# mauruszach/multimodal_diffusion

Hardware: AMD Instinct MI355X
Metric: denoising steps/sec @256x256 multimodal-cond batch=32 (higher is better)
Workload: dtype f32 via 3xbf16 split operands (6-term products, f32 accumulate; fp32-level error); 1 GPU; C3: 256x256 audio->video CFG denoising step (cond+null MMDiT d512 L8 H8 + noise head + DDIM), 384+37 tokens, batch 32 per GPU, DDIM 50 steps, guidance 3.5; global_batch=32, sampler_steps=50, parallelism=dp1, launch=eager, matmul=bf16x3, attn=default, cfg_halves=one stacked 2B batch, one stream

## Files before the change

include/avdiff_hip.h:

```cpp
#ifndef AVDIFF_HIP_H
#define AVDIFF_HIP_H

#include <stdint.h>

#ifdef __cplusplus
extern "C" {
#endif

#define AVD_ABI_VERSION 7

#define AVD_OK            0
#define AVD_EINVAL       -1
#define AVD_EUNSUPPORTED -2
#define AVD_ELAUNCH      -3
#define AVD_EWORKSPACE   -4

#define AVD_ACT_NONE 0
#define AVD_ACT_GELU 1
#define AVD_ACT_SILU 2
#define AVD_ACT_TANH 3
#define AVD_ACT_RELU 4
#define AVD_ACT_LEAKY_RELU 5

typedef void* avd_stream_t;

int         avd_abi_version(void);
const char* avd_last_error(void);
int         avd_device_arch(char* buf, int buflen);
int         avd_tune_set(const char* key, int64_t value);
int         avd_cfg_dedup_set(int on);

int avd_rmsnorm_f32(const float* x, const float* scale, float* y, int64_t rows, int d, float eps,
                    avd_stream_t stream);

int avd_gemm_bias_act_f32(const float* A, int64_t lda, const float* W, const float* bias,
                          const float* residual, int64_t ldr, float* C, int64_t ldc,
                          int64_t M, int N, int K, int act, avd_stream_t stream);

int avd_gemm_rmsfold_f32(const float* A, const float* W, const float* bias, const float* residual, float* C, int64_t M,
                         int N, int K, int act, const float* ss_in, int ss_in_cols, float eps, float* ss_out,
                         avd_stream_t stream);

int avd_attn_fwd_f32(const float* qkv, float* out, int B, int N, int H, int Dh, float scale,
                     int n_query, const uint8_t* key_padding_mask, avd_stream_t stream);

int avd_layernorm_act_f32(const float* x, const float* gamma, const float* beta, float* y,
                          int64_t rows, int d, float eps, int act, avd_stream_t stream);

int avd_timestep_embedding_f32(const int64_t* t, const float* freqs, float* out, int B, int dim, float max_period,
                               avd_stream_t stream);

int avd_tube_patch_f32(const float* z, float* tok, int B, int C, int T, int H, int W, int t, int h, int w,
                       avd_stream_t stream);
int avd_tube_unpatch_f32(const float* tok, float* z, int B, int C, int T, int H, int W, int t, int h, int w,
                         avd_stream_t stream);

int avd_audio_tokens_f32(const float* z, float* tok, int B, int Ca, int F, int len, int stride,
                         avd_stream_t stream);
int avd_audio_untokens_f32(const float* tok, const float* window, float* z, int B, int Ca, int F, int len, int stride,
                           avd_stream_t stream);

int avd_ddim_step_f32(const float* x_t, const float* eps_hat, const int64_t* t_now, const int64_t* t_prev,
                      const float* alpha_bar, int T_train, float eta, const float* noise,
                      float* x_prev, int B, int64_t per_sample, avd_stream_t stream);

int avd_dpmpp_2m_step_f32(const float* x_t, const float* eps_hat, float* x0_hist, const int64_t* t_last, const int64_t* t_now,
                          const int64_t* t_prev, const float* alpha_bar, int T_train, float* x_out, int B, int64_t per_sample,
                          avd_stream_t stream);

int avd_dpmpp_2m_sde_step_f32(const float* x_t, const float* eps_hat, float* x0_hist, const int64_t* t_last, const int64_t* t_now,
                              const int64_t* t_prev, const float* alpha_bar, int T_train, float eta, const float* noise, float* x_out,
                              int B, int64_t per_sample, avd_stream_t stream);

typedef struct {
    uint64_t seed;
    int64_t sample_offset;
} avd_noise_key;
int avd_gaussian_noise_f32(const avd_noise_key* key, const int64_t* t_now, float* out, int B, int64_t per_sample,
                           avd_stream_t stream);

int avd_canvas_noise_f32(const avd_noise_key* key, const int64_t* t_now, float* out, int N, int64_t outer, int L, int hop,
                         int64_t inner, avd_stream_t stream);

int avd_cfg_unpatch_ddim_slots_f32(const float* eps2, const float* z, const int64_t* t_now, const int64_t* t_prev,
                                   const float* alpha_bar, int T_train, float guidance, int slots, float* z_out,
                                   int B, int C, int T, int H, int W, int t, int h, int w, avd_stream_t stream);
int avd_cfg_untoken_ddim_audio_slots_f32(const float* eps2, const float* z, const int64_t* t_now, const int64_t* t_prev,
                                         const float* alpha_bar, int T_train, float guidance, int slots, float* z_out,
                                         int B, int Ca, int F, int len, int stride, avd_stream_t stream);
int avd_cfg_unpatch_dpmpp_2m_slots_f32(const float* eps2, const float* z, const int64_t* t_last, const int64_t* t_now,
                                       const int64_t* t_prev, const float* alpha_bar, int T_train, float guidance, int slots,
                                       float* x0_hist, float* z_out, int B, int C, int T, int H, int W, int t, int h, int w,
                                       avd_stream_t stream);
int avd_cfg_untoken_dpmpp_2m_audio_slots_f32(const float* eps2, const float* z, const int64_t* t_last, const int64_t* t_now,
                                             const int64_t* t_prev, const float* alpha_bar, int T_train, float guidance, int slots,
                                             float* x0_hist, float* z_out, int B, int Ca, int F, int len, int stride,
                                             avd_stream_t stream);

int avd_fifo_shift_f32(const avd_noise_key* key, int64_t t, int64_t c, const float* z_in, float* z_out, float* popped,
                       int B, int64_t outer, int slots, int slot_len, int64_t inner, avd_stream_t stream);
int avd_fifo_shift_hist_f32(const avd_noise_key* key, int64_t t, int64_t c, const float* z_in, float* z_out, float* popped,
                            const float* hist_in, float* hist_out, int B, int64_t outer, int slots, int slot_len, int64_t inner,
                            avd_stream_t stream);

int avd_fifo_lookahead_f32(const avd_noise_key* key, int64_t t, int64_t c, int shift, const float* z_in, float* z_out, float* popped,
                           int B, int64_t outer, int slots, int ctx, int slot_len, int64_t inner, avd_stream_t stream);
int avd_fifo_lookahead_hist_f32(const avd_noise_key* key, int64_t t, int64_t c, int shift, const float* z_in, float* z_out,
                                float* popped, const float* hist_in, float* hist_out, int B, int64_t outer, int slots, int ctx,
                                int slot_len, int64_t inner, avd_stream_t stream);

int avd_cursor_add(int32_t* cursor, int delta, avd_stream_t stream);
int avd_slot_tables_select(const int64_t* tab0, const int64_t* tab1, const int64_t* tab2, int n_rows, int n, const int32_t* cursor,
                           int64_t* out0, int64_t* out1, int64_t* out2, avd_stream_t stream);
int avd_fifo_prompt_gather_f32(const float* canvas, const int32_t* cursor, float* out, int B, int slots, int prompt_hop, int64_t outer,
                               int64_t P, int64_t prompt_len, int64_t inner, avd_stream_t stream);
int avd_fifo_shift_cursor_f32(const avd_noise_key* key, int64_t t, int64_t c0, const int32_t* cursor, int64_t n_out, const float* z_in,
                              float* z_out, float* clip, int B, int64_t outer, int slots, int slot_len, int64_t inner, avd_stream_t stream);
int avd_fifo_shift_cursor_hist_f32(const avd_noise_key* key, int64_t t, int64_t c0, const int32_t* cursor, int64_t n_out,
                                   const float* z_in, float* z_out, float* clip, const float* hist_in, float* hist_out, int B,
                                   int64_t outer, int slots, int slot_len, int64_t inner, avd_stream_t stream);

typedef struct {
    const float* known;
    const float* mask;
    int64_t mask_batch_stride;
    avd_noise_key key;
} avd_latent_guide;
int avd_latent_guide_f32(const avd_latent_guide* g, const int64_t* tau, const float* alpha_bar, int T_train,
                         const float* z, float* out, int B, int64_t per_sample, avd_stream_t stream);

int avd_latent_guide_canvas_f32(const avd_latent_guide* g, const int64_t* tau, const float* alpha_bar, int T_train,
                                const float* z, float* out, int N, int64_t outer, int L, int hop, int64_t inner, avd_stream_t stream);

int avd_renoise_f32(const avd_noise_key* key, uint32_t visit, const avd_latent_guide* g, const int64_t* t_from, const int64_t* t_to,
                    const float* alpha_bar, int T_train, const float* z, float* out, int B, int64_t per_sample, avd_stream_t stream);
int avd_renoise_canvas_f32(const avd_noise_key* key, uint32_t visit, const avd_latent_guide* g, const int64_t* t_from,
                           const int64_t* t_to, const float* alpha_bar, int T_train, const float* z, float* out, int N, int64_t outer,
                           int L, int hop, int64_t inner, avd_stream_t stream);

typedef struct {
    const float* guidance;
    const float* rescale;
    void* stats;
    int64_t stats_bytes;
} avd_cfg_control;
int64_t avd_cfg_stats_bytes(int B, int64_t per_sample);
int avd_cfg_rescale_f32(const float* e_cond, const float* e_cfg, const float* phi, void* stats, int64_t stats_bytes, float* out,
                        int B, int64_t per_sample, avd_stream_t stream);

typedef struct {
    float norm_threshold;
    float eta_parallel;
    float momentum;
    float* momentum_buf;
    void* stats;
    int64_t stats_bytes;
} avd_apg_control;
int64_t avd_apg_stats_bytes(int B, int64_t per_sample);
int avd_apg_guidance_f32(const float* e_cond, const float* e_null, const float* guidance, float guidance_scalar,
                         const avd_apg_control* apg, float* out, int B, int64_t per_sample, avd_stream_t stream);

int avd_cfg_unpatch_ddim_f32(const float* eps2, const float* z, const int64_t* t_now, const int64_t* t_prev,
                             const float* alpha_bar, int T_train, float guidance, float eta,
                             const float* noise, float* z_out,
                             int B, int C, int T, int H, int W, int t, int h, int w, avd_stream_t stream);

int avd_cfg_untoken_ddim_audio_f32(const float* eps2, const float* z, const int64_t* t_now,
                                   const int64_t* t_prev, const float* alpha_bar, int T_train,
                                   float guidance, float eta, const float* noise, float* z_out,
                                   int B, int Ca, int F, int len, int stride, avd_stream_t stream);

int avd_eps_unpatch_ddim_f32(const float* eps, const float* z, const int64_t* t_now, const int64_t* t_prev,
                             const float* alpha_bar, int T_train, float eta, const float* noise, float* z_out,
                             int B, int C, int T, int H, int W, int t, int h, int w, const avd_noise_key* key,
                             const int64_t* t_last, float* x0_hist, const avd_latent_guide* guide, avd_stream_t stream);
int avd_eps_untoken_ddim_audio_f32(const float* eps, const float* z, const int64_t* t_now, const int64_t* t_prev,
                                   const float* alpha_bar, int T_train, float eta, const float* noise, float* z_out,
                                   int B, int Ca, int F, int len, int stride, const avd_noise_key* key,
                                   const int64_t* t_last, float* x0_hist, const avd_latent_guide* guide, avd_stream_t stream);

typedef struct {
    int target_kind;
    int target_first;
    int B, d, tdim;
    int C, T, H, W;
    int p0, p1, p2;
// ... 244 lines not shown
```

multimodal_diffusion_amd/_lib.py:

```python
from __future__ import annotations

import ctypes as C
import os
from pathlib import Path
from typing import Optional

import torch

_HERE = Path(__file__).resolve().parent
LIB_PATH = Path(os.environ.get("AVDIFF_HIP_LIB", _HERE / "csrc" / "libavdiff_hip.so"))

ACT_NONE, ACT_GELU, ACT_SILU, ACT_TANH, ACT_RELU, ACT_LEAKY_RELU = 0, 1, 2, 3, 4, 5
EINVAL, EUNSUPPORTED, ELAUNCH, EWORKSPACE = -1, -2, -3, -4


class AvdError(RuntimeError):
    """A HIP-side failure (launch error, unsupported shape, workspace)."""


class EmbedDesc(C.Structure):
    _fields_ = [("target_kind", C.c_int), ("target_first", C.c_int), ("B", C.c_int), ("d", C.c_int),
                ("tdim", C.c_int), ("C", C.c_int), ("T", C.c_int), ("H", C.c_int), ("W", C.c_int),
                ("p0", C.c_int), ("p1", C.c_int), ("p2", C.c_int), ("Nt", C.c_int), ("Np", C.c_int),
                ("temb_freqs", C.c_void_p), ("temb_add", C.c_int)]


class BlockWeights(C.Structure):
    _fields_ = [(n, C.c_void_p) for n in (
        "norm1_scale", "in_proj_weight", "in_proj_bias", "out_proj_weight", "out_proj_bias",
        "norm2_scale", "fc1_weight", "fc1_bias", "fc2_weight", "fc2_bias",
        "in_proj_weight_n", "fc1_weight_n",
        "in_proj_weight3", "out_proj_weight3", "fc1_weight3", "fc2_weight3",
        "norm1_bias", "norm2_bias")] + [("f16x2_scale", C.c_float * 8), ("in_proj_weight3n", C.c_void_p), ("fc1_weight3n", C.c_void_p)]


class CoreWeights(C.Structure):
    _fields_ = [("d", C.c_int), ("n_layers", C.c_int), ("n_heads", C.c_int), ("mlp_hidden", C.c_int),
                ("norm_eps", C.c_float), ("blocks", C.POINTER(BlockWeights)), ("final_norm_scale", C.c_void_p),
                ("norm_kind", C.c_int), ("final_norm_bias", C.c_void_p), ("split_terms", C.c_int), ("attn_mode", C.c_int)]


class HeadWeights(C.Structure):
    _fields_ = [("d_in", C.c_int), ("hidden", C.c_int), ("d_out", C.c_int), ("n_shared", C.c_int),
                ("ln_eps", C.c_float), ("act", C.c_int),
                ("input_proj_weight", C.c_void_p), ("input_proj_bias", C.c_void_p),
                ("shared_lin_weight", C.POINTER(C.c_void_p)), ("shared_lin_bias", C.POINTER(C.c_void_p)),
                ("shared_ln_weight", C.POINTER(C.c_void_p)), ("shared_ln_bias", C.POINTER(C.c_void_p)),
                ("out_proj_weight", C.c_void_p), ("out_proj_bias", C.c_void_p),
                ("split_terms", C.c_int), ("input_proj_weight3", C.c_void_p), ("shared_lin_weight3", C.POINTER(C.c_void_p)),
                ("out_proj_weight3", C.c_void_p), ("f16x2_scale", C.POINTER(C.c_float))]


class StepDesc(C.Structure):
    _fields_ = [("embed", EmbedDesc), ("core", C.POINTER(CoreWeights)), ("head", C.POINTER(HeadWeights)),
                ("adapt_w", C.c_void_p), ("adapt_b", C.c_void_p), ("alpha_bar", C.c_void_p), ("T_train", C.c_int),
                ("guidance", C.c_float), ("eta", C.c_float), ("split_streams", C.c_int)]


class NoiseKey(C.Structure):
    _fields_ = [("seed", C.c_uint64), ("sample_offset", C.c_int64)]


class LatentGuide(C.Structure):
    _fields_ = [("known", C.c_void_p), ("mask", C.c_void_p), ("mask_batch_stride", C.c_int64), ("key", NoiseKey)]


class CfgControl(C.Structure):
    _fields_ = [("guidance", C.c_void_p), ("rescale", C.c_void_p), ("stats", C.c_void_p), ("stats_bytes", C.c_int64)]


class ApgControl(C.Structure):
    _fields_ = [("norm_threshold", C.c_float), ("eta_parallel", C.c_float), ("momentum", C.c_float), ("momentum_buf", C.c_void_p),
                ("stats", C.c_void_p), ("stats_bytes", C.c_int64)]


class VaeDecodeDesc(C.Structure):
    _fields_ = [("B", C.c_int), ("Cv", C.c_int), ("Tp", C.c_int), ("Hp", C.c_int), ("Wp", C.c_int),
                ("T", C.c_int), ("H", C.c_int), ("W", C.c_int),
                ("base", C.c_int), ("n_blocks", C.c_int), ("out_ch", C.c_int), ("out_tanh", C.c_int),
                ("gn_eps", C.c_float),
                ("from_lat_w", C.c_void_p), ("from_lat_b", C.c_void_p),
                ("conv_w", C.POINTER(C.c_void_p)), ("conv_b", C.POINTER(C.c_void_p)),
                ("gn_w", C.POINTER(C.c_void_p)), ("gn_b", C.POINTER(C.c_void_p)),
                ("to_img_w", C.c_void_p), ("to_img_b", C.c_void_p),
                ("conv_w3", C.POINTER(C.c_void_p)), ("conv_terms", C.c_int),
                ("conv_w_scale", C.POINTER(C.c_float)), ("conv_a_scale", C.POINTER(C.c_float)),
                ("conv0_lat_w3", C.c_void_p), ("conv0_lat_btab", C.c_void_p), ("conv0_lat_w_scale", C.c_float),
                ("conv0_lat_packed", C.c_int)]


class VaeEncodeDesc(C.Structure):
    _fields_ = [("B", C.c_int), ("in_ch", C.c_int), ("T", C.c_int), ("H", C.c_int), ("W", C.c_int),
                ("t_down", C.c_int), ("s_down", C.c_int),
                ("base", C.c_int), ("n_blocks", C.c_int), ("lat_ch", C.c_int), ("gn_eps", C.c_float),
                ("conv_w", C.POINTER(C.c_void_p)), ("conv_b", C.POINTER(C.c_void_p)),
                ("gn_w", C.POINTER(C.c_void_p)), ("gn_b", C.POINTER(C.c_void_p)),
                ("to_lat_w", C.c_void_p), ("to_lat_b", C.c_void_p),
                ("conv_w3", C.POINTER(C.c_void_p)), ("conv_terms", C.c_int),
                ("conv_w_scale", C.POINTER(C.c_float)), ("conv_a_scale", C.POINTER(C.c_float)),
                ("conv0_pk_w3", C.c_void_p)]


ABI_VERSION = 7
_P, _I, _L, _F = C.c_void_p, C.c_int, C.c_int64, C.c_float

SIGNATURES = {
    "avd_abi_version": (_I, []),
    "avd_last_error": (C.c_char_p, []),
    "avd_device_arch": (_I, [C.c_char_p, _I]),
    "avd_rmsnorm_f32": (_I, [_P, _P, _P, _L, _I, _F, _P]),
    "avd_gemm_bias_act_f32": (_I, [_P, _L, _P, _P, _P, _L, _P, _L, _L, _I, _I, _I, _P]),
    "avd_gemm_rmsfold_f32": (_I, [_P, _P, _P, _P, _P, _L, _I, _I, _I, _P, _I, _F, _P, _P]),
    "avd_tune_set": (_I, [C.c_char_p, _L]),
    "avd_cfg_dedup_set": (_I, [_I]),
    "avd_attn_fwd_f32": (_I, [_P, _P, _I, _I, _I, _I, _F, _I, _P, _P]),
    "avd_layernorm_act_f32": (_I, [_P, _P, _P, _P, _L, _I, _F, _I, _P]),
    "avd_timestep_embedding_f32": (_I, [_P, _P, _P, _I, _I, _F, _P]),
    "avd_tube_patch_f32": (_I, [_P, _P] + [_I] * 8 + [_P]),
    "avd_tube_unpatch_f32": (_I, [_P, _P] + [_I] * 8 + [_P]),
    "avd_audio_tokens_f32": (_I, [_P, _P] + [_I] * 5 + [_P]),
    "avd_audio_untokens_f32": (_I, [_P, _P, _P] + [_I] * 5 + [_P]),
    "avd_ddim_step_f32": (_I, [_P, _P, _P, _P, _P, _I, _F, _P, _P, _I, _L, _P]),
    "avd_cfg_unpatch_ddim_f32": (_I, [_P, _P, _P, _P, _P, _I, _F, _F, _P, _P] + [_I] * 8 + [_P]),
    "avd_cfg_untoken_ddim_audio_f32": (_I, [_P, _P, _P, _P, _P, _I, _F, _F, _P, _P] + [_I] * 5 + [_P]),
    "avd_embed_workspace_floats": (_L, [C.POINTER(EmbedDesc)]),
    "avd_embed_cfg_pair_f32": (_I, [C.POINTER(EmbedDesc), _P, _P, _P, _P, _P, _P, _P, _P]),
    "avd_core_workspace_bytes": (_L, [C.POINTER(CoreWeights), _I, _I]),
    "avd_core_forward_f32": (_I, [C.POINTER(CoreWeights), _P, _P, _I, _I, _I, _I, _P, _P, _L, _P]),
    "avd_head_workspace_bytes": (_L, [C.POINTER(HeadWeights), _L]),
    "avd_head_forward_f32": (_I, [C.POINTER(HeadWeights), _P, _L, _L, _L, _L, _P, _P, _L, _P]),
    "avd_step_workspace_bytes": (_L, [C.POINTER(StepDesc)]),
    "avd_denoise_step_f32": (_I, [C.POINTER(StepDesc), _P, _P, _P, _P, _P, _P, _P, _L, _P]),
    "avd_denoise_step_seeded_f32": (_I, [C.POINTER(StepDesc), C.POINTER(NoiseKey), _P, _P, _P, _P, _P, _P, _L, _P]),
    "avd_gaussian_noise_f32": (_I, [C.POINTER(NoiseKey), _P, _P, _I, _L, _P]),
    "avd_canvas_noise_f32": (_I, [C.POINTER(NoiseKey), _P, _P, _I, _L, _I, _I, _L, _P]),
    "avd_denoise_step_canvas_f32": (_I, [C.POINTER(StepDesc), C.POINTER(NoiseKey), _I, C.POINTER(CfgControl), C.POINTER(LatentGuide), _I,
                                         _P, _P, _P, _P, _P, _P, _L, _P]),
    "avd_cfg_unpatch_ddim_slots_f32": (_I, [_P, _P, _P, _P, _P, _I, _F, _I, _P] + [_I] * 8 + [_P]),
    "avd_cfg_untoken_ddim_audio_slots_f32": (_I, [_P, _P, _P, _P, _P, _I, _F, _I, _P] + [_I] * 5 + [_P]),
    "avd_embed_cfg_pair_slots_f32": (_I, [C.POINTER(EmbedDesc), _P, _P, _P, _P, _I, _P, _P, _P, _P]),
    "avd_denoise_step_slots_f32": (_I, [C.POINTER(StepDesc), _P, _P, _P, _P, _I, _P, _P, _L, _P]),
    "avd_fifo_shift_f32": (_I, [C.POINTER(NoiseKey), _L, _L, _P, _P, _P, _I, _L, _I, _I, _L, _P]),
    "avd_cfg_unpatch_dpmpp_2m_slots_f32": (_I, [_P, _P, _P, _P, _P, _P, _I, _F, _I, _P, _P] + [_I] * 8 + [_P]),
    "avd_cfg_untoken_dpmpp_2m_audio_slots_f32": (_I, [_P, _P, _P, _P, _P, _P, _I, _F, _I, _P, _P] + [_I] * 5 + [_P]),
    "avd_denoise_step_slots_dpmpp_2m_f32": (_I, [C.POINTER(StepDesc), _P, _P, _P, _P, _P, _I, _P, _P, _P, _L, _P]),
    "avd_fifo_shift_hist_f32": (_I, [C.POINTER(NoiseKey), _L, _L, _P, _P, _P, _P, _P, _I, _L, _I, _I, _L, _P]),
    "avd_fifo_lookahead_f32": (_I, [C.POINTER(NoiseKey), _L, _L, _I, _P, _P, _P, _I, _L, _I, _I, _I, _L, _P]),
    "avd_fifo_lookahead_hist_f32": (_I, [C.POINTER(NoiseKey), _L, _L, _I, _P, _P, _P, _P, _P, _I, _L, _I, _I, _I, _L, _P]),
    "avd_cursor_add": (_I, [_P, _I, _P]),
    "avd_slot_tables_select": (_I, [_P, _P, _P, _I, _I, _P, _P, _P, _P, _P]),
    "avd_fifo_prompt_gather_f32": (_I, [_P, _P, _P, _I, _I, _I, _L, _L, _L, _L, _P]),
    "avd_fifo_shift_cursor_f32": (_I, [C.POINTER(NoiseKey), _L, _L, _P, _L, _P, _P, _P, _I, _L, _I, _I, _L, _P]),
    "avd_fifo_shift_cursor_hist_f32": (_I, [C.POINTER(NoiseKey), _L, _L, _P, _L, _P, _P, _P, _P, _P, _I, _L, _I, _I, _L, _P]),
    "avd_sched_advance": (_I, [_P, _I, _P, _P, _P, _I, _P]),
    "avd_sched_advance_ms": (_I, [_P, _I, _P, _P, _P, _P, _I, _P]),
    "avd_dpmpp_2m_step_f32": (_I, [_P, _P, _P, _P, _P, _P, _P, _I, _P, _I, _L, _P]),
    "avd_denoise_step_dpmpp_2m_f32": (_I, [C.POINTER(StepDesc), _P, _P, _P, _P, _P, _P, _P, _P, _L, _P]),
    "avd_dpmpp_2m_sde_step_f32": (_I, [_P, _P, _P, _P, _P, _P, _P, _I, _F, _P, _P, _I, _L, _P]),
    "avd_denoise_step_dpmpp_2m_sde_f32": (_I, [C.POINTER(StepDesc), C.POINTER(NoiseKey), _I, C.POINTER(CfgControl), C.POINTER(LatentGuide),
                                               _I, _P, _P, _P, _P, _P, _P, _P, _P, _L, _P]),
    "avd_latent_guide_f32": (_I, [C.POINTER(LatentGuide), _P, _P, _I, _P, _P, _I, _L, _P]),
    "avd_latent_guide_canvas_f32": (_I, [C.POINTER(LatentGuide), _P, _P, _I, _P, _P, _I, _L, _I, _I, _L, _P]),
    "avd_renoise_f32": (_I, [C.POINTER(NoiseKey), C.c_uint32, C.POINTER(LatentGuide), _P, _P, _P, _I, _P, _P, _I, _L, _P]),
    "avd_renoise_canvas_f32": (_I, [C.POINTER(NoiseKey), C.c_uint32, C.POINTER(LatentGuide), _P, _P, _P, _I, _P, _P, _I, _L, _I, _I, _L,
                                    _P]),
    "avd_denoise_step_canvas_guided_f32": (_I, [C.POINTER(StepDesc), C.POINTER(LatentGuide), _I, C.POINTER(NoiseKey), C.POINTER(CfgControl),
                                                _I, _P, _P, _P, _P, _P, _P, _P, _P, _L, _P]),
    "avd_denoise_step_guided_f32": (_I, [C.POINTER(StepDesc), C.POINTER(LatentGuide), C.POINTER(NoiseKey), _P, _P, _P, _P, _P, _P, _P,
                                         _P, _L, _P]),
    "avd_cfg_stats_bytes": (_L, [_I, _L]),
    "avd_cfg_rescale_f32": (_I, [_P, _P, _P, _P, _L, _P, _I, _L, _P]),
    "avd_denoise_step_cfg_f32": (_I, [C.POINTER(StepDesc), C.POINTER(CfgControl), C.POINTER(LatentGuide), C.POINTER(NoiseKey), _P, _P, _P,
                                      _P, _P, _P, _P, _P, _L, _P]),
    "avd_apg_stats_bytes": (_L, [_I, _L]),
    "avd_apg_guidance_f32": (_I, [_P, _P, _P, _F, C.POINTER(ApgControl), _P, _I, _L, _P]),
    "avd_denoise_step_apg_f32": (_I, [C.POINTER(StepDesc), C.POINTER(ApgControl), C.POINTER(CfgControl), C.POINTER(LatentGuide),
                                      C.POINTER(NoiseKey), _I, _I, _P, _P, _P, _P, _P, _P, _P, _P, _L, _P]),
    "avd_eps_unpatch_ddim_f32": (_I, [_P, _P, _P, _P, _P, _I, _F, _P, _P] + [_I] * 8 + [C.POINTER(NoiseKey), _P, _P, C.POINTER(LatentGuide), _P]),
    "avd_eps_untoken_ddim_audio_f32": (_I, [_P, _P, _P, _P, _P, _I, _F, _P, _P] + [_I] * 5 + [C.POINTER(NoiseKey), _P, _P,
                                                                                               C.POINTER(LatentGuide), _P]),
    "avd_embed_cond_f32": (_I, [C.POINTER(EmbedDesc), _P, _P, _P, _P, _P, _P, _P, _P, _P]),
    "avd_denoise_step_cond_f32": (_I, [C.POINTER(StepDesc), C.POINTER(LatentGuide), C.POINTER(NoiseKey), _P, _P, _P, _P, _P, _P, _P, _P,
                                       _P, _L, _P]),
    "avd_split3_bytes": (_L, [_L, _I]),
    "avd_split3_f32": (_I, [_P, _P, _L, _I, _P]),
    "avd_rmsnorm_split3_f32": (_I, [_P, _P, _P, _L, _I, _F, _P]),
    "avd_attn_fwd_split3_f32": (_I, [_P, _P, _I, _I, _I, _I, _F, _I, _P]),
    "avd_qkv3_bytes": (_L, [_I, _I, _I]),
    "avd_gemm_bf16x3_qkv3_f32": (_I, [_P, _P, _P, _P, _L, _I, _I, _I, _F, _I, _P]),
    "avd_attn_fwd_qkv3_f32": (_I, [_P, _P, _P, _I, _I, _I, _I, _I, _P]),
    "avd_attn_fp8_workspace_bytes": (_L, [_I, _I, _I]),
    "avd_attn_fwd_fp8_f32": (_I, [_P, _P, _L, _P, _P, _I, _I, _I, _I, _P]),
    "avd_attn_fwd_fp8_f16x2_f32": (_I, [_P, _P, _L, _P, _P, _I, _I, _I, _I, _F, _F, _P]),
    "avd_gemm_bf16x3_f32": (_I, [_P, _P, _P, _P, _P, _P, _L, _I, _I, _I, _I, _P]),
    "avd_weight_bounds_f32": (_I, [_P, _L, _I, _P, _P]),
    "avd_split_f16x2_f32": (_I, [_P, _P, _L, _I, _F, _P]),
    "avd_rmsnorm_split_f16x2_f32": (_I, [_P, _P, _P, _L, _I, _F, _F, _P]),
    "avd_gemm_f16x2_f32": (_I, [_P, _P, _P, _P, _P, _P, _L, _I, _I, _I, _F, _F, _P]),
    "avd_gemm_f16x2_qkv_f32": (_I, [_P, _P, _P, _P, _L, _I, _I, _I, _F, _F, _F, _P]),
    "avd_attn_fwd_qkv_f16x2_f32": (_I, [_P, _P, _P, _I, _I, _I, _I, _F, _F, _P]),
    "avd_conv3_weight_bytes": (_L, []),
    "avd_conv3_weight_f32": (_I, [_P, _P, _P]),
    "avd_conv3_weight_f16x2_f32": (_I, [_P, _P, _F, _P]),
    "avd_vae_decode_workspace_bytes": (_L, [C.POINTER(VaeDecodeDesc)]),
    "avd_vae_decode_f32": (_I, [C.POINTER(VaeDecodeDesc), _P, _P, _P, _L, _P]),
    "avd_vae_encode_workspace_bytes": (_L, [C.POINTER(VaeEncodeDesc)]),
    "avd_vae_encode_f32": (_I, [C.POINTER(VaeEncodeDesc), _P, _P, _P, _L, _P]),
    "avd_conv1d_act_f32": (_I, [_P, _P, _P, _P, _I, _I, _I, _I, _I, _I, _I, _P]),
    "avd_avgpool_frames_f32": (_I, [_P, _P, _I, _I, _I, _I, _P]),
    "avd_crossfade_f32": (_I, [_P, _P, _P, _I, _I, _I, _L, _P]),
    "avd_crossfade_u8": (_I, [_P, _P, _P, _I, _I, _I, _L, _P]),
    "avd_window_consensus_f32": (_I, [_P, _P, _I, _L, _I, _I, _L, _P]),
    "avd_prof_enable": (_I, [_I]),
    "avd_prof_num_tags": (_I, []),
    "avd_prof_tag_name": (C.c_char_p, [_I]),
    "avd_prof_report": (_I, [C.POINTER(C.c_int64), C.POINTER(C.c_double), C.POINTER(C.c_double), _I]),
}

def prof_enable(on: bool) -> None:
    check(lib().avd_prof_enable(1 if on else 0))


def prof_report():
    n = lib().avd_prof_num_tags()
    cnt, ms, work = (C.c_int64 * max(n, 1))(), (C.c_double * max(n, 1))(), (C.c_double * max(n, 1))()
    check(lib().avd_prof_report(cnt, ms, work, n))
    return {lib().avd_prof_tag_name(i).decode(): (int(cnt[i]), float(ms[i]), float(work[i])) for i in range(n)}


_lib: Optional[C.CDLL] = None


def lib() -> C.CDLL:
    global _lib
    if _lib is None:
        if not LIB_PATH.exists():
            raise AvdError(
                f"{LIB_PATH} not found: build it with `make -C multimodal_diffusion_amd/csrc` "
                "(or __graft_entry__.build()); this package has no CPU/PyTorch fallback")
        handle = C.CDLL(str(LIB_PATH))
        for name, (res, args) in SIGNATURES.items():
            fn = getattr(handle, name)
            fn.restype, fn.argtypes = res, args
        if handle.avd_abi_version() != ABI_VERSION:
            raise AvdError(f"ABI version mismatch: library {handle.avd_abi_version()}, binding {ABI_VERSION}")
        _lib = handle
    return _lib


def check(rc: int) -> None:
    if rc == 0:
        return
    msg = lib().avd_last_error().decode("utf-8", "replace")
    if rc == EINVAL:
        raise ValueError(msg)
    raise AvdError(f"[avd {rc}] {msg}")


def stream_ptr(device: torch.device) -> int:
    idx = device.index if device.index is not None else torch.cuda.current_device()
    if idx != torch.cuda.current_device():
        raise AvdError(f"tensors are on cuda:{idx} but the current device is cuda:{torch.cuda.current_device()}: "
                       "call torch.cuda.set_device / use torch.cuda.device(...) around the call")
    return torch.cuda.current_stream(device).cuda_stream


MATMUL_TERMS = {"auto": 6, "f32": 0, "bf16x3": 6, "bf16x3_strict": 9, "bf16": 1, "f16x2": 3}
# ... 21 lines not shown
```

multimodal_diffusion_amd/csrc/avd_common.h:

```cpp
#pragma once
#include <hip/hip_runtime.h>
#include <stdint.h>
#include <stdio.h>
#include <stdarg.h>
#include <atomic>

#include "../../include/avdiff_hip.h"

namespace avd {

int set_error(int code, const char* fmt, ...);

#define AVD_REQUIRE(cond, code, ...)                       \
    do {                                                   \
        if (!(cond)) return avd::set_error((code), __VA_ARGS__); \
    } while (0)

#define AVD_CHECK_LAUNCH(name)                                                          \
    do {                                                                                \
        hipError_t e__ = hipGetLastError();                                             \
        if (e__ != hipSuccess)                                                          \
            return avd::set_error(AVD_ELAUNCH, "%s: %s", (name), hipGetErrorString(e__)); \
    } while (0)

// ... 66 lines not shown
    }
};

struct TubeGather {
    int T, H, W, t, h, w, Ht, Wt, Nt;
    int64_t per;
    __host__ __device__ __forceinline__ int64_t row_off(int64_t row) const {
        const int64_t b = row / Nt;
        const int n = (int)(row - b * Nt);
        const int nx = n % Wt, ny = (n / Wt) % Ht, nt = n / (Wt * Ht);
        return b * per + ((int64_t)(nt * t) * H + ny * h) * W + nx * w;
    }
    __host__ __device__ __forceinline__ int64_t k_off(int k) const {
        const int dx = k % w, dy = (k / w) % h, dt = (k / (w * h)) % t, c = k / (w * h * t);
        return (((int64_t)c * T + dt) * H + dy) * W + dx;
    }
};

typedef __bf16 bf16x8 __attribute__((ext_vector_type(8)));
typedef unsigned int u32x4 __attribute__((ext_vector_type(4)));

constexpr int S3_CHUNK = 128 * 96;
constexpr int S3_PLANE = 128 * 32;

typedef __bf16 bf16x2 __attribute__((ext_vector_type(2)));
typedef float f32x2 __attribute__((ext_vector_type(2)));

__device__ __forceinline__ unsigned int pk_bf16(float a, float b) {
    const f32x2 v = {a, b};
    return __builtin_bit_cast(unsigned int, __builtin_convertvector(v, bf16x2));
}
__device__ __forceinline__ float bf16_lo(unsigned int p) { return __uint_as_float(p << 16); }
__device__ __forceinline__ float bf16_hi(unsigned int p) { return __uint_as_float(p & 0xffff0000u); }

template <bool RANGE_CHECK = true>
__device__ __forceinline__ void split8(const float* v, u32x4& H, u32x4& Mi, u32x4& Lo) {
#pragma clang fp contract(off)
    bool edge = false;
    if constexpr (RANGE_CHECK) {
        float amax = fabsf(v[0]);
#pragma unroll
        for (int e = 1; e < 8; ++e) amax = fmaxf(amax, fabsf(v[e]));
        edge = __any(amax > 3.3895313892515355e38f);
    }
#pragma unroll
    for (int e = 0; e < 4; ++e) {
        const float a = v[2 * e], b = v[2 * e + 1];
        unsigned int h = pk_bf16(a, b);
        float ra = a - bf16_lo(h), rb = b - bf16_hi(h);
        if (edge) {
            if ((h & 0x7fffu) == 0x7f80u) {
                if (fabsf(a) < __builtin_inff()) { h = (h & 0xffff8000u) | 0x7f7fu; ra = a - bf16_lo(h); } else ra = 0.f;
            }
            if ((h & 0x7fff0000u) == 0x7f800000u) {
                if (fabsf(b) < __builtin_inff()) { h = (h & 0x8000ffffu) | 0x7f7f0000u; rb = b - bf16_hi(h); } else rb = 0.f;
            }
        }
        const unsigned int m = pk_bf16(ra, rb);
        const float sa = ra - bf16_lo(m), sb = rb - bf16_hi(m);
        H[e] = h;
        Mi[e] = m;
        Lo[e] = pk_bf16(sa, sb);
    }
}

template <bool RANGE_CHECK = true>
__device__ __forceinline__ void store_split8(unsigned char* img, int64_t r, int k, int K, const float* v) {
    u32x4 H, Mi, Lo;
    split8<RANGE_CHECK>(v, H, Mi, Lo);
    const int rr = (int)(r & 127), half = (k >> 3) & 1;
    unsigned char* dst = img + ((r >> 7) * (K >> 4) + (k >> 4)) * (int64_t)S3_CHUNK + rr * 32 + ((half ^ ((rr >> 4) & 1)) << 4);
    *reinterpret_cast<u32x4*>(dst) = H;
    *reinterpret_cast<u32x4*>(dst + S3_PLANE) = Mi;
    *reinterpret_cast<u32x4*>(dst + 2 * S3_PLANE) = Lo;
}

typedef _Float16 f16x8 __attribute__((ext_vector_type(8)));
typedef _Float16 f16x2 __attribute__((ext_vector_type(2)));

__device__ __forceinline__ unsigned int pk_f16(float a, float b) {
    const f32x2 v = {a, b};
    return __builtin_bit_cast(unsigned int, __builtin_convertvector(v, f16x2));
}
__device__ __forceinline__ f32x2 unpk_f16(unsigned int p) { return __builtin_convertvector(__builtin_bit_cast(f16x2, p), f32x2); }

__device__ __forceinline__ void split8_h2(const float* v, float s, u32x4& H, u32x4& L) {
#pragma unroll
    for (int e = 0; e < 4; ++e) {
        const float a = v[2 * e] * s, b = v[2 * e + 1] * s;
        const unsigned int h = pk_f16(a, b);
        const f32x2 u = unpk_f16(h);
        H[e] = h;
        L[e] = pk_f16(a - u[0], b - u[1]);
    }
}
__device__ __forceinline__ void store_split8_h2(unsigned char* img, int64_t r, int k, int K, const float* v, float s) {
    u32x4 H, L;
    split8_h2(v, s, H, L);
    const int rr = (int)(r & 127), half = (k >> 3) & 1;
    unsigned char* dst = img + ((r >> 7) * (K >> 4) + (k >> 4)) * (int64_t)S3_CHUNK + rr * 32 + ((half ^ ((rr >> 4) & 1)) << 4);
    *reinterpret_cast<u32x4*>(dst) = H;
    *reinterpret_cast<u32x4*>(dst + S3_PLANE) = L;
}

template <bool F16>
__device__ __forceinline__ f32x16 mma16(bf16x8 a, bf16x8 b, f32x16 c) {
    if constexpr (F16)
        return __builtin_amdgcn_mfma_f32_32x32x16_f16(__builtin_bit_cast(f16x8, a), __builtin_bit_cast(f16x8, b), c, 0, 0, 0);
    else
        return __builtin_amdgcn_mfma_f32_32x32x16_bf16(a, b, c, 0, 0, 0);
}
__host__ __device__ constexpr int s3_planes(int terms) { return terms == 1 ? 1 : terms == 3 ? 2 : 3; }

constexpr int QKV3_ROWB = 384;
__host__ __device__ __forceinline__ int qkv3_npad(int n) { return (n + 63) / 64 * 64; }
__host__ __device__ __forceinline__ int qkv3_swizzle(int part, int n) {
    return part == 0 ? 0 : part == 1 ? (n >> 1) & 7 : (((n >> 1) & 1) << 2) | (((n >> 2) & 1) << 1);
}

extern bool g_prof_on;
void prof_mark(int tag, double work, hipStream_t st, bool begin);
int prof_tag_id(const char* fmt, ...);
struct ProfScope {
    int tag; hipStream_t st; bool on;
    ProfScope(int t, double work, hipStream_t s) : tag(t), st(s), on(g_prof_on) { if (on) prof_mark(tag, work, st, true); }
    ~ProfScope() { if (on) prof_mark(tag, 0.0, st, false); }
};

int gemm_f32(const float* A, RowMap am, const float* W, const float* bias, const float* R, RowMap rm,
             float* C, RowMap cm, int64_t M, int N, int K, int act, hipStream_t st);
int gemm_f32_tube(const float* z, const TubeGather& tg, const float* W, const float* bias, float* C, RowMap cm, int64_t M, int N, int K,
                  hipStream_t st);

extern int g_gemm_stages;
extern int g_gemm_force_tile;
bool gemm_f32_fold_supported(int N, int K);
int gemm_f32_fold(const float* A, RowMap am, const float* W, const float* bias, const float* R, RowMap rm, float* C, RowMap cm,
                  int64_t M, int N, int K, int act, const float* ss_in, int ss_in_cols, float sqrt_d, float eps, float* ss_out,
                  hipStream_t st);
int rowss_f32(const float* x, float* ss, int64_t rows, int d, hipStream_t st);
constexpr int kGemmSplitKMax = 4;
extern int g_gemm_splitk;
int gemm_f32_splitk_slices(int64_t M, int N, int K);
int64_t gemm_f32_splitk_ws_max_floats(int64_t M, int N, int K);
int gemm_f32_splitk(const float* A, RowMap am, const float* W, const float* bias, const float* R, RowMap rm, float* C, RowMap cm, int64_t M,
                    int N, int K, int ns, float* part, float* ss_out, hipStream_t st);

int attn_f32(const float* qkv, float* out, int B, int N, int H, int Dh, float scale, int n_query, const unsigned char* key_padding_mask,
             hipStream_t st);
int rmsnorm_f32(const float* x, RowMap xm, const float* scale, float* y, RowMap ym, int64_t rows, int d, float eps,
                hipStream_t st);
int layernorm_act_f32(const float* x, const float* gamma, const float* beta, float* y, int64_t rows, int d, float eps,
                      int act, hipStream_t st);
int weight_bounds_f32(const float* x, int64_t rows, int d, float* out2, hipStream_t st);

int64_t split3_bytes(int64_t rows, int K);
int split3_f32(const float* x, int64_t ld, void* out, int64_t rows, int K, hipStream_t st, float h2_scale = 0.f);
int split3_rows_f32(const float* x, RowMap xm, void* out, int64_t rows, int K, hipStream_t st, float h2_scale = 0.f, float* ss = nullptr);
int rmsnorm_split3_f32(const float* x, const float* scale, void* out, int64_t rows, int d, float eps, hipStream_t st, float h2_scale = 0.f);
int layernorm_act_split3_f32(const float* x, const float* gamma, const float* beta, void* out, int64_t rows, int d, float eps, int act,
                             hipStream_t st, float h2_scale = 0.f);
bool gemm_bf16x3_supported(int64_t M, int N, int K);
int attn_f32_split3(const float* qkv, void* out3, int B, int N, int H, int Dh, float scale, int n_query, hipStream_t st);
extern int g_s3_stagger;
extern int g_mlp_fused;
bool mlp_bf16x3_supported(int d, int hidden, int terms);
int mlp_bf16x3(const void* X3, const void* W1n3, const float* b1, const void* W23, const float* b2, const float* ss_in, float eps,
               const float* R, float* C, void* C3, float* ss_out, int64_t M, int d, int hidden, hipStream_t st);
extern int g_attn_m16;
extern int g_attn_pipe;
extern int g_s3_m16;
extern int g_s3_w128;
extern int g_s3_rt4;
extern int g_s3_deep4;
extern int g_s3_rt;
extern int g_vae_lat;
extern int g_vae_fold;
extern int g_codec_mfma;
extern int g_cfg_rows;
extern int g_s3_sn, g_s3_super4, g_s3_super8;
extern int g_s3_tile;
extern thread_local bool t_s3_two_streams;
int gemm_bf16x3_qkv3(const void* A3, const void* W3, const float* bias, void* img, const RowSegs& seg, int heads, int K, float qscale,
                     int terms, hipStream_t st, float ab_scale = 1.f, float c_scale = 1.f, const float* ss_in = nullptr, float eps = 0.f,
                     int64_t plan_rows = 0);
int64_t qkv3_bytes(int B, int N, int H);
int64_t attn_fp8_ws_bytes(int B, int N, int H);
int attn_fp8(const void* qkv3, void* ws, int64_t ws_bytes, float* out, void* out3, int B, int N, int H, int n_query, hipStream_t st,
             int img_terms = 6, float img_scale = 1.f, float out_scale = 1.f);
int attn_bf16x3(const void* qkv3, float* out, void* out3, int B, int N, int H, int n_query, int terms, hipStream_t st,
                float img_scale = 1.f, float out_scale = 1.f, int out_tokens = 0, const RowSegs* out_rows = nullptr);
int gemm_bf16x3(const void* A3, const void* W3, const float* bias, const float* R, float* C, void* C3, int64_t M, int N, int K,
                int act, int terms, hipStream_t st, float ab_scale = 1.f, float c_scale = 1.f, const float* ss_in = nullptr, float eps = 0.f,
                float* ss_out = nullptr, const float* gamma = nullptr, int r_seg = 0, const RowSegs* r_map = nullptr, int64_t plan_rows = 0);
bool gemm_bf16x3_resmap_supported(int terms);
bool gemm_bf16x3_rownorm_supported(int N, int terms);
extern int g_s3_splitk;
int gemm_bf16x3_splitk_slices(int64_t M, int N, int K, int terms);
int64_t gemm_bf16x3_splitk_ws_floats(int64_t M, int N, int ns);
constexpr int kS3SplitKMax = 4;
int64_t gemm_bf16x3_splitk_ws_max_floats(int64_t M, int N, int K);
int gemm_bf16x3_splitk(const void* A3, const void* W3, const float* bias, const float* R, float* C, void* C3, float* ss, int64_t M, int N,
                       int K, int terms, int ns, float* part, hipStream_t st);

}
```

multimodal_diffusion_amd/csrc/composite.hip:

```cpp
#include "avd_common.h"

#include <limits.h>
#include <stdlib.h>

#include <string.h>
#include <map>
#include <mutex>
#include <string>
#include <utility>
#include <vector>

namespace avd {

static thread_local char g_err[512] = "";

int set_error(int code, const char* fmt, ...) {
    va_list ap;
    va_start(ap, fmt);
    vsnprintf(g_err, sizeof(g_err), fmt, ap);
    va_end(ap);
    return code;
}

int LdsAttr::ensure(const void* kern, int lds_bytes, const char* what) {
// ... 4 lines not shown
    if (bit && (done.load(std::memory_order_acquire) & bit)) return AVD_OK;
    e = hipFuncSetAttribute(kern, hipFuncAttributeMaxDynamicSharedMemorySize, lds_bytes);
    if (e != hipSuccess) return set_error(AVD_ELAUNCH, "%s: hipFuncSetAttribute: %s", what, hipGetErrorString(e));
    done.fetch_or(bit, std::memory_order_release);
    return AVD_OK;
}

bool g_prof_on = false;
namespace {
struct ProfRec { hipEvent_t a, b; int tag; double work; };
std::vector<ProfRec> g_recs;
std::vector<hipEvent_t> g_pool;
std::vector<std::string> g_tags;
hipEvent_t take_event() {
    if (!g_pool.empty()) { hipEvent_t e = g_pool.back(); g_pool.pop_back(); return e; }
    hipEvent_t e; (void)hipEventCreate(&e); return e;
}
}
int prof_tag_id(const char* fmt, ...) {
    char buf[160];
    va_list ap;
    va_start(ap, fmt);
    vsnprintf(buf, sizeof(buf), fmt, ap);
    va_end(ap);
    for (size_t i = 0; i < g_tags.size(); ++i)
        if (g_tags[i] == buf) return (int)i;
    g_tags.emplace_back(buf);
    return (int)g_tags.size() - 1;
}
void prof_mark(int tag, double work, hipStream_t st, bool begin) {
    if (begin) {
        ProfRec r{take_event(), take_event(), tag, work};
        (void)hipEventRecord(r.a, st);
        g_recs.push_back(r);
    } else if (!g_recs.empty()) {
        (void)hipEventRecord(g_recs.back().b, st);
    }
}

int temb_f32(const int64_t* t, const float* freqs, float* out, int B, int dim, float max_period, hipStream_t st);
int tube_patch_f32(const float* z, float* tok, int B, int C, int T, int H, int W, int t, int h, int w, hipStream_t st);
int audio_tokens_f32(const float* z, float* tok, int B, int Ca, int F, int len, int stride, hipStream_t st);
int assemble_f32(float* X2, const float* temb, const float* Xp, int B, int N, int d, int tdim, int Nt, int Np,
                 int target_first, hipStream_t st);
int assemble_rows_f32(float* X2, const int64_t* t_now, const float* freqs, const float* Xp, float* ss, int B, int N, int d, int tdim,
                      int Nt, int Np, int target_first, float max_period, hipStream_t st, const RowSegs* short_null = nullptr, int slots = 0,
                      int slot_tok = 0);
int qkv3_replicate(void* img, int img_samples, int H, int n_keys, int first_sample, int n_samples, int src, hipStream_t st);
int cfg_unpatch_ddim_f32(const float* eps2, const float* z, const int64_t* t_now, const int64_t* t_prev,
                         const float* abar, int T_train, float guidance, float eta, const float* noise, float* z_out,
                         int B, int C, int T, int H, int W, int t, int h, int w, hipStream_t st, const avd_noise_key* key = nullptr,
                         const int64_t* t_last = nullptr, float* x0_hist = nullptr, const avd_latent_guide* guide = nullptr,
                         const avd_cfg_control* ctl = nullptr, int canvas_hop = 0, int guide_hop = 0, int slots = 0,
                         const avd_apg_control* apg = nullptr);
int cfg_untoken_ddim_audio_f32(const float* eps2, const float* z, const int64_t* t_now, const int64_t* t_prev,
                               const float* abar, int T_train, float guidance, float eta, const float* noise,
                               float* z_out, int B, int Ca, int F, int len, int stride, hipStream_t st,
                               const avd_noise_key* key = nullptr, const int64_t* t_last = nullptr, float* x0_hist = nullptr,
                               const avd_latent_guide* guide = nullptr, const avd_cfg_control* ctl = nullptr, int canvas_hop = 0, int guide_hop = 0,
                               int slots = 0, const avd_apg_control* apg = nullptr);
int assemble_cond_f32(float* X1, const float* temb, const float* Xp, int B, int N, int d, int tdim, int Nt, int Np, int target_first,
                      hipStream_t st);
int assemble_rows_cond_f32(float* X1, const int64_t* t_now, const float* freqs, const float* Xp, float* ss, int B, int N, int d,
                           int tdim, int Nt, int Np, int target_first, float max_period, hipStream_t st);
int eps_unpatch_ddim_f32(const float* eps1, const float* z, const int64_t* t_now, const int64_t* t_prev, const float* abar, int T_train,
                         float eta, const float* noise, float* z_out, int B, int C, int T, int H, int W, int t, int h, int w,
                         hipStream_t st, const avd_noise_key* key, const int64_t* t_last, float* x0_hist, const avd_latent_guide* guide,
                         int canvas_hop = 0, int guide_hop = 0);
int eps_untoken_ddim_audio_f32(const float* eps1, const float* z, const int64_t* t_now, const int64_t* t_prev, const float* abar,
                               int T_train, float eta, const float* noise, float* z_out, int B, int Ca, int F, int len, int stride,
                               hipStream_t st, const avd_noise_key* key, const int64_t* t_last, float* x0_hist,
                               const avd_latent_guide* guide, int canvas_hop = 0, int guide_hop = 0);
int check_canvas_key(const avd_noise_key* key, int N, int64_t outer, int L, int hop, int64_t inner);
int check_canvas_guide(const avd_latent_guide* g, int N, int64_t outer, int L, int hop, int64_t inner, const float* out,
                       const float* x0_hist);
int check_latent_guide(const avd_latent_guide* g, int B, int64_t per, const float* out, const float* x0_hist);
int check_cfg_control(const avd_cfg_control* ctl, int B, int64_t per, const float* out, const float* x0_hist);
int check_apg_control(const avd_apg_control* apg, const avd_cfg_control* ctl, int B, int64_t per, const float* z, const float* out,
                      const float* x0_hist, const void* eps, int64_t eps_bytes);
bool overlaps(const float* a, const float* b, int64_t n);

static inline int64_t align_up(int64_t x) { return (x + 255) & ~(int64_t)255; }

struct Carver {
    char* base;
    int64_t used, cap;
    bool ok = true;
    float* take(int64_t floats) {
        float* p = reinterpret_cast<float*>(base + used);
        used += align_up(floats * (int64_t)sizeof(float));
        if (used > cap) ok = false;
        return p;
    }
};

constexpr int64_t kSplitMinRows = 6144;
constexpr int64_t kSplitMinRowsM16 = 2048;
static int g_s3_min_rows = -1;
static int g_no_fold = 0;
static int64_t split_min_rows(int terms = 3) {
    if (g_s3_min_rows >= 0) return g_s3_min_rows;
    return (terms == 0 || terms == 6) && g_s3_m16 ? kSplitMinRowsM16 : kSplitMinRows;
}
static bool core_split_capable(const avd_core_weights* w, int64_t M) {
    if (w->norm_kind != 0) return false;
    if (!gemm_bf16x3_supported(M, 3 * w->d, w->d) || !gemm_bf16x3_supported(M, w->d, w->d) ||
        !gemm_bf16x3_supported(M, w->mlp_hidden, w->d) || !gemm_bf16x3_supported(M, w->d, w->mlp_hidden))
        return false;
    for (int l = 0; l < w->n_layers; ++l) {
        const avd_block_weights& b = w->blocks[l];
        if (!b.in_proj_weight3 || !b.out_proj_weight3 || !b.fc1_weight3 || !b.fc2_weight3) return false;
    }
    return true;
}
static thread_local int64_t t_step_rows = 0;
static bool core_use_split(const avd_core_weights* w, int64_t M) {
    const int64_t Mt = t_step_rows > M ? t_step_rows : M;
    if (Mt < split_min_rows(w->split_terms) && w->split_terms != 1 && w->attn_mode != 1) return false;
    return core_split_capable(w, M);
}

static bool core_split_fold_capable(const avd_core_weights* w) {
    if (w->norm_kind != 0 || w->split_terms == 3 || w->d % 64 != 0) return false;
    for (int l = 0; l < w->n_layers; ++l)
        if (!w->blocks[l].in_proj_weight3n || !w->blocks[l].fc1_weight3n) return false;
    return true;
}
static bool core_use_split_fold(const avd_core_weights* w) { return !g_no_fold && core_split_fold_capable(w); }

static bool core_split_rownorm_capable(const avd_core_weights* w) {
    return w->norm_kind == 0 && w->split_terms == 3 && gemm_bf16x3_rownorm_supported(w->d, 3);
}
static bool core_use_split_rownorm(const avd_core_weights* w) { return !g_no_fold && core_split_rownorm_capable(w); }

static bool core_use_fold(const avd_core_weights* w) {
    if (g_no_fold || w->norm_kind != 0) return false;
    if (!gemm_f32_fold_supported(3 * w->d, w->d) || !gemm_f32_fold_supported(w->d, w->d) ||
        !gemm_f32_fold_supported(w->mlp_hidden, w->d) || !gemm_f32_fold_supported(w->d, w->mlp_hidden))
        return false;
    for (int l = 0; l < w->n_layers; ++l)
        if (!w->blocks[l].in_proj_weight_n || !w->blocks[l].fc1_weight_n) return false;
    return true;
}

static int g_core_trim = 1;
static int64_t core_trim_floats(const avd_core_weights* w, int B, int N) { return (int64_t)B * N * w->d; }

static int g_cfg_dedup = 1;
[[maybe_unused]] static const bool g_cfg_dedup_env_applied = [] {
    if (const char* e = getenv("AVD_CFG_DEDUP")) g_cfg_dedup = atoll(e) != 0;
    return true;
}();

static int64_t core_split_wide_bytes(const avd_core_weights* w, int B, int N) {
    const int64_t qkv3 = qkv3_bytes(B, N, w->n_heads), fc1 = split3_bytes((int64_t)B * N, w->mlp_hidden);
    return qkv3 > fc1 ? qkv3 : fc1;
}

static int64_t core_ws_bytes(const avd_core_weights* w, int B, int N) {
    const int64_t M = (int64_t)B * N;
    const int wide = 3 * w->d > w->mlp_hidden ? 3 * w->d : w->mlp_hidden;
    int64_t fp32_path = align_up(M * w->d * 4) + align_up(M * wide * 4) + 2 * align_up(M * (w->d / 32 + 1) * 4) +
                        align_up(gemm_f32_splitk_ws_max_floats(M, w->d, w->mlp_hidden) * 4);
    if (!core_split_capable(w, M)) return fp32_path;
    const int64_t wide_b = core_split_wide_bytes(w, B, N);
    const int64_t f8_b = w->attn_mode == 1 ? attn_fp8_ws_bytes(B, N, w->n_heads) : 0;
    const int64_t fold_b = core_split_fold_capable(w) ? align_up(split3_bytes(M, w->d)) + align_up(M * (w->d / 64) * 4)
                         : core_split_rownorm_capable(w) ? align_up(split3_bytes(M, w->d)) : 0;
    const int64_t sk_b = core_split_fold_capable(w) ? align_up(gemm_bf16x3_splitk_ws_max_floats(M, w->d, w->mlp_hidden) * 4) : 0;
    const int64_t trim_b = core_split_fold_capable(w) ? align_up(core_trim_floats(w, B, N) * 4) : 0;
    const int64_t split_path = align_up(wide_b) + align_up(split3_bytes(M, w->d)) + align_up(f8_b) + fold_b + sk_b + trim_b;
    return split_path > fp32_path ? split_path : fp32_path;
}

static int check_core(const avd_core_weights* w) {
    AVD_REQUIRE(w && w->blocks && w->final_norm_scale, AVD_EINVAL, "core: null weight table");
    AVD_REQUIRE(w->d > 0 && w->n_layers > 0 && w->n_heads > 0 && w->mlp_hidden > 0, AVD_EINVAL, "core: bad dims");
    AVD_REQUIRE(w->d % w->n_heads == 0, AVD_EINVAL, "core: d_model %d not divisible by n_heads %d", w->d, w->n_heads);
    AVD_REQUIRE(w->attn_mode == 0 || w->attn_mode == 1, AVD_EINVAL, "core: attn_mode must be 0 (follow the matmul mode) or 1 (fp8)");
    AVD_REQUIRE(w->norm_kind == 0 || w->norm_kind == 1, AVD_EINVAL, "core: norm_kind must be 0 (RMSNorm) or 1 (LayerNorm)");
    AVD_REQUIRE(w->d / w->n_heads == 64, AVD_EUNSUPPORTED, "core: head_dim %d unsupported (64 only)", w->d / w->n_heads);
    AVD_REQUIRE(w->d % 4 == 0 && w->mlp_hidden % 4 == 0, AVD_EUNSUPPORTED, "core: widths must be multiples of 4");
    AVD_REQUIRE(w->split_terms == 0 || w->split_terms == 6 || w->split_terms == 9 || w->split_terms == 1 || w->split_terms == 3, AVD_EINVAL,
                "core: split_terms must be 0/6 (default), 9 (strict), 1 (plain bf16) or 3 (f16x2), got %d", w->split_terms);
    if (w->split_terms == 3) {
        for (int l = 0; l < w->n_layers; ++l)
            for (int i = 0; i < 8; ++i) {
                const float s = w->blocks[l].f16x2_scale[i];
                AVD_REQUIRE(s > 0.f && s < __builtin_inff(), AVD_EINVAL, "core: blocks[%d].f16x2_scale[%d] must be positive and finite", l, i);
            }
    }
    return AVD_OK;
}

static int core_norm(const avd_core_weights* w, const float* x, const float* scale, const float* bias, float* y, int64_t M, hipStream_t st) {
    const RowMap rd{w->d, 0, 0};
    if (w->norm_kind == 0) return rmsnorm_f32(x, rd, scale, y, rd, M, w->d, w->norm_eps, st);
    AVD_REQUIRE(bias, AVD_EINVAL, "core: norm_kind 1 (LayerNorm) needs the bias vectors");
    return layernorm_act_f32(x, scale, bias, y, M, w->d, w->norm_eps, AVD_ACT_NONE, st);
}

static bool core_dedup_ok(const avd_core_weights* w, int B2, int N, int n_out) {
    const int terms = w->split_terms;
    return B2 % 2 == 0 && n_out > 0 && n_out + 2 <= N && w->attn_mode == 0 && (terms == 0 || terms == 6 || terms == 9) && g_core_trim &&
           !g_mlp_fused && gemm_bf16x3_resmap_supported(terms) && core_use_split(w, (int64_t)B2 * N) && core_use_split_fold(w);
}

static int core_forward(const avd_core_weights* w, const float* x, float* y, int B, int N, int out_row0,
                        int n_out_rows, const unsigned char* kpm, void* ws, int64_t ws_bytes, hipStream_t st,
                        const float* ss_first = nullptr, const RowSegs* segs = nullptr) {
    if (int rc = check_core(w)) return rc;
    AVD_REQUIRE(x && y && B > 0 && N > 0, AVD_EINVAL, "core: bad input");
    AVD_REQUIRE(out_row0 >= 0 && n_out_rows > 0 && out_row0 + n_out_rows <= N, AVD_EINVAL, "core: bad output row window");
    const int64_t M = (int64_t)B * N;
    AVD_REQUIRE(ws && ws_bytes >= core_ws_bytes(w, B, N), AVD_EWORKSPACE, "core: workspace %lld < %lld bytes",
                (long long)ws_bytes, (long long)core_ws_bytes(w, B, N));
    const int d = w->d, hid = w->mlp_hidden, H = w->n_heads;
    Carver cv{static_cast<char*>(ws), 0, ws_bytes};
    float* hbuf = cv.take(M * d);
    float* wide = cv.take(M * (3 * d > hid ? 3 * d : hid));
    const RowMap rd{d, 0, 0}, r3{3 * d, 0, 0}, rh{hid, 0, 0};
    const float scale = 1.0f / sqrtf((float)(d / H));
    const float* cur = x;
    AVD_REQUIRE(!(w->attn_mode == 1 && (kpm || w->norm_kind != 0)), AVD_EUNSUPPORTED,
                "core: attn_mode 1 (fp8 attention) cannot be combined with a key_padding_mask or norm_kind 1 (LayerNorm)");
    const int null_from = segs ? segs->samples[0] : 0;
    AVD_REQUIRE(!segs || (null_from > 0 && segs->n_samples() == B && segs->tok[0] == N && segs->tok[1] == n_out_rows + 1 &&
                          segs->m0 == (int64_t)null_from * N && out_row0 == 0 && !kpm && core_dedup_ok(w, B, N, n_out_rows)), AVD_EUNSUPPORTED,
                "core: the two-segment row layout needs the folded six-term split path with the trimmed last block");
    AVD_REQUIRE(!(w->attn_mode == 1 && !core_use_split(w, M)), AVD_EUNSUPPORTED,
                "core: attn_mode 1 (fp8 attention) reads the q|k|v image of the split-operand projections, which these weights / shapes "
                "do not take (every block needs its *_weight3 images; 3 d, d and mlp_hidden must be multiples of 256, d of 16)");
    if (!kpm && core_use_split(w, M)) {
        const int terms = w->split_terms;
        Carver cs{static_cast<char*>(ws), 0, ws_bytes};
        const int64_t wide_b = core_split_wide_bytes(w, B, N);
        float* qkv = cs.take((wide_b + 3) / 4);
        void* wide3 = qkv;
        void* hs = cs.take((split3_bytes(M, d) + 3) / 4);
        const int64_t f8_b = w->attn_mode == 1 ? attn_fp8_ws_bytes(B, N, H) : 0;
        float* f8w = cs.take((f8_b + 3) / 4);
        if (core_use_split_fold(w)) {
            void* hx = cs.take((split3_bytes(M, d) + 3) / 4);
            float* ss = cs.take(M * (d / 64));
            const int ns = gemm_bf16x3_splitk_slices(M, d, hid, terms);
            float* part = ns ? cs.take(gemm_bf16x3_splitk_ws_floats(M, d, ns)) : nullptr;
            const bool trim = g_core_trim && out_row0 == 0 && n_out_rows < N && w->attn_mode == 0 && gemm_bf16x3_resmap_supported(terms);
            float* yc = cs.take(core_trim_floats(w, B, N));
            const bool fused = g_mlp_fused && !ns && mlp_bf16x3_supported(d, hid, terms) && gemm_bf16x3_resmap_supported(terms);
            AVD_REQUIRE(cs.ok, AVD_EWORKSPACE, "core: workspace carve %lld > %lld bytes", (long long)cs.used, (long long)cs.cap);
            const RowSegs seg = segs ? *segs : RowSegs::uniform(B, N);
            const int64_t Mr = seg.rows();
            const float qscale = scale * 1.4426950408889634f;
            auto in_proj = [&](const avd_block_weights& b) {
                if (int rc = gemm_bf16x3_qkv3(hx, b.in_proj_weight3n, b.in_proj_bias, qkv, seg, H, d, qscale, terms, st, 1.f, 1.f, ss, w->norm_eps, M))
                    return rc;
                return null_from ? qkv3_replicate(qkv, B, H, N, null_from, B - null_from, n_out_rows, st) : (int)AVD_OK;
            };
            if (int rc = split3_rows_f32(cur, rd, hx, Mr, d, st, 0.f, ss)) return rc;
            for (int l = 0; l < w->n_layers; ++l) {
                const avd_block_weights& b = w->blocks[l];
                const bool last = l == w->n_layers - 1;
                const int nq = (last && out_row0 == 0) ? n_out_rows : N;
                if (last && trim) {
                    const int64_t Mc = (int64_t)B * nq;
                    if (int rc = in_proj(b)) return rc;
                    if (int rc = attn_bf16x3(qkv, nullptr, hs, B, N, H, nq, terms, st, 1.f, 1.f, nq)) return rc;
                    if (int rc = gemm_bf16x3(hs, b.out_proj_weight3, b.out_proj_bias, cur, yc, hx, Mc, d, d, AVD_ACT_NONE, terms, st, 1.f, 1.f,
                                             nullptr, 0.f, ss, nullptr, nq, &seg)) return rc;
                    if (fused) {
                        if (int rc = mlp_bf16x3(hx, b.fc1_weight3n, b.fc1_bias, b.fc2_weight3, b.fc2_bias, ss, w->norm_eps, yc, yc, nullptr, nullptr, Mc,
                                                d, hid, st)) return rc;
                    } else {
                        if (int rc = gemm_bf16x3(hx, b.fc1_weight3n, b.fc1_bias, nullptr, nullptr, wide3, Mc, hid, d, AVD_ACT_GELU, terms, st, 1.f, 1.f,
                                                 ss, w->norm_eps)) return rc;
                        if (ns) {
                            if (int rc = gemm_bf16x3_splitk(wide3, b.fc2_weight3, b.fc2_bias, yc, yc, nullptr, nullptr, Mc, d, hid, terms, ns, part,
                                                            st)) return rc;
                        } else {
                            if (int rc = gemm_bf16x3(wide3, b.fc2_weight3, b.fc2_bias, yc, yc, nullptr, Mc, d, hid, AVD_ACT_NONE, terms, st)) return rc;
                        }
                    }
                    return rmsnorm_f32(yc, rd, w->final_norm_scale, y, null_from ? rd : RowMap{d, nq, (int64_t)N * d}, Mc, d, w->norm_eps, st);
                }
                if (int rc = in_proj(b)) return rc;
                if (w->attn_mode == 1) {
                    if (int rc = attn_fp8(qkv, f8w, f8_b, nullptr, hs, B, N, H, nq, st, terms, 1.f, 1.f)) return rc;
                } else if (null_from) {
                    if (int rc = attn_bf16x3(qkv, nullptr, hs, B, N, H, N, terms, st, 1.f, 1.f, 0, &seg)) return rc;
                } else {
                    if (int rc = attn_bf16x3(qkv, nullptr, hs, B, N, H, nq, terms, st, 1.f, 1.f)) return rc;
                }
                if (int rc = gemm_bf16x3(hs, b.out_proj_weight3, b.out_proj_bias, cur, y, hx, Mr, d, d, AVD_ACT_NONE, terms, st, 1.f, 1.f, nullptr,
                                         0.f, ss, nullptr, 0, nullptr, M)) return rc;
                cur = y;
                if (fused) {
                    if (int rc = mlp_bf16x3(hx, b.fc1_weight3n, b.fc1_bias, b.fc2_weight3, b.fc2_bias, ss, w->norm_eps, y, y, last ? nullptr : hx,
                                            last ? nullptr : ss, Mr, d, hid, st)) return rc;
                    continue;
                }
                if (int rc = gemm_bf16x3(hx, b.fc1_weight3n, b.fc1_bias, nullptr, nullptr, wide3, Mr, hid, d, AVD_ACT_GELU, terms, st, 1.f, 1.f, ss,
                                         w->norm_eps, nullptr, nullptr, 0, nullptr, M)) return rc;
                if (ns) {
                    if (int rc = gemm_bf16x3_splitk(wide3, b.fc2_weight3, b.fc2_bias, y, y, last ? nullptr : hx, last ? nullptr : ss, Mr, d, hid,
                                                    terms, ns, part, st)) return rc;
                } else if (last) {
                    if (int rc = gemm_bf16x3(wide3, b.fc2_weight3, b.fc2_bias, y, y, nullptr, Mr, d, hid, AVD_ACT_NONE, terms, st)) return rc;
                } else {
                    if (int rc = gemm_bf16x3(wide3, b.fc2_weight3, b.fc2_bias, y, y, hx, Mr, d, hid, AVD_ACT_NONE, terms, st, 1.f, 1.f, nullptr, 0.f,
                                             ss, nullptr, 0, nullptr, M)) return rc;
                }
            }
            return rmsnorm_f32(y, rd, w->final_norm_scale, y, rd, Mr, d, w->norm_eps, st);
        }
        const bool rown = core_use_split_rownorm(w);
        void* hn = rown ? cs.take((split3_bytes(M, d) + 3) / 4) : hs;
        AVD_REQUIRE(cs.ok, AVD_EWORKSPACE, "core: workspace carve %lld > %lld bytes", (long long)cs.used, (long long)cs.cap);
        for (int l = 0; l < w->n_layers; ++l) {
            const avd_block_weights& b = w->blocks[l];
            const bool last = l == w->n_layers - 1;
            const int nq = (last && out_row0 == 0) ? n_out_rows : N;
            const bool h2 = terms == 3;
            const float* fs = b.f16x2_scale;
            const float s_n1 = h2 ? fs[4] : 0.f, s_qkv = h2 ? fs[5] : 1.f, s_n2 = h2 ? fs[6] : 0.f, s_fc1 = h2 ? fs[7] : 1.f;
            const float w_in = h2 ? fs[0] : 1.f, w_out = h2 ? fs[1] : 1.f, w_fc1 = h2 ? fs[2] : 1.f, w_fc2 = h2 ? fs[3] : 1.f;
            if (!rown || l == 0)
                if (int rc = rmsnorm_split3_f32(cur, b.norm1_scale, hn, M, d, w->norm_eps, st, s_n1)) return rc;
            if (int rc = gemm_bf16x3_qkv3(hn, b.in_proj_weight3, b.in_proj_bias, qkv, RowSegs::uniform(B, N), H, d, scale * 1.4426950408889634f, terms, st,
                                          h2 ? s_n1 * w_in : 1.f, s_qkv)) return rc;
            if (w->attn_mode == 1) {
                if (int rc = attn_fp8(qkv, f8w, f8_b, nullptr, hs, B, N, H, nq, st, terms, s_qkv, s_qkv)) return rc;
            } else {
                if (int rc = attn_bf16x3(qkv, nullptr, hs, B, N, H, nq, terms, st, s_qkv, s_qkv)) return rc;
            }
            if (rown) {
                if (int rc = gemm_bf16x3(hs, b.out_proj_weight3, b.out_proj_bias, cur, y, hn, M, d, d, AVD_ACT_NONE, terms, st, s_qkv * w_out, s_n2,
                                         nullptr, w->norm_eps, nullptr, b.norm2_scale)) return rc;
                cur = y;
            } else {
                if (int rc = gemm_bf16x3(hs, b.out_proj_weight3, b.out_proj_bias, cur, y, nullptr, M, d, d, AVD_ACT_NONE, terms, st,
                                         h2 ? s_qkv * w_out : 1.f, 1.f)) return rc;
                cur = y;
                if (int rc = rmsnorm_split3_f32(y, b.norm2_scale, hn, M, d, w->norm_eps, st, s_n2)) return rc;
            }
            if (int rc = gemm_bf16x3(hn, b.fc1_weight3, b.fc1_bias, nullptr, nullptr, wide3, M, hid, d, AVD_ACT_GELU, terms, st,
                                     h2 ? s_n2 * w_fc1 : 1.f, s_fc1)) return rc;
            if (rown && !last) {
                const avd_block_weights& nb = w->blocks[l + 1];
                if (int rc = gemm_bf16x3(wide3, b.fc2_weight3, b.fc2_bias, y, y, hn, M, d, hid, AVD_ACT_NONE, terms, st, s_fc1 * w_fc2,
                                         nb.f16x2_scale[4], nullptr, w->norm_eps, nullptr, nb.norm1_scale)) return rc;
            } else {
                if (int rc = gemm_bf16x3(wide3, b.fc2_weight3, b.fc2_bias, y, y, nullptr, M, d, hid, AVD_ACT_NONE, terms, st,
                                         h2 ? s_fc1 * w_fc2 : 1.f, 1.f)) return rc;
            }
        }
        return rmsnorm_f32(y, rd, w->final_norm_scale, y, rd, M, d, w->norm_eps, st);
    }
    if (core_use_fold(w)) {
        float* ssA = cv.take(M * (d / 32 + 1));
        float* ssB = cv.take(M * (d / 32 + 1));
        const int nsf = gemm_f32_splitk_slices(M, d, hid);
        float* partf = nsf ? cv.take((int64_t)nsf * M * d) : nullptr;
        AVD_REQUIRE(cv.ok, AVD_EWORKSPACE, "core: workspace carve %lld > %lld bytes", (long long)cv.used, (long long)cv.cap);
        const float sqrt_d = (float)sqrt((double)d);
        const float* ssA_in = ss_first;
        if (!ssA_in) {
            if (int rc = rowss_f32(cur, ssA, M, d, st)) return rc;
            ssA_in = ssA;
        }
        int colsA = 1;
        for (int l = 0; l < w->n_layers; ++l) {
            const avd_block_weights& b = w->blocks[l];
            const bool last = l == w->n_layers - 1;
            const int nq = (last && out_row0 == 0) ? n_out_rows : N;
            if (int rc = gemm_f32_fold(cur, rd, b.in_proj_weight_n, b.in_proj_bias, nullptr, rd, wide, r3, M, 3 * d, d, AVD_ACT_NONE,
                                       l == 0 ? ssA_in : ssA, colsA, sqrt_d, w->norm_eps, nullptr, st)) return rc;
            if (int rc = attn_f32(wide, hbuf, B, N, H, d / H, scale, nq, kpm, st)) return rc;
            if (int rc = gemm_f32_fold(hbuf, rd, b.out_proj_weight, b.out_proj_bias, cur, rd, y, rd, M, d, d, AVD_ACT_NONE, nullptr, 0,
                                       1.f, 0.f, ssB, st)) return rc;
            cur = y;
            if (int rc = gemm_f32_fold(y, rd, b.fc1_weight_n, b.fc1_bias, nullptr, rd, wide, rh, M, hid, d, AVD_ACT_GELU, ssB, d / 32,
                                       sqrt_d, w->norm_eps, nullptr, st)) return rc;
            if (nsf) {
                if (int rc = gemm_f32_splitk(wide, rh, b.fc2_weight, b.fc2_bias, y, rd, y, rd, M, d, hid, nsf, partf, ssA, st)) return rc;
            } else {
                if (int rc = gemm_f32_fold(wide, rh, b.fc2_weight, b.fc2_bias, y, rd, y, rd, M, d, hid, AVD_ACT_NONE, nullptr, 0, 1.f, 0.f,
                                           ssA, st)) return rc;
            }
            colsA = d / 32;
        }
        return rmsnorm_f32(y, rd, w->final_norm_scale, y, rd, M, d, w->norm_eps, st);
    }
    for (int l = 0; l < w->n_layers; ++l) {
        const avd_block_weights& b = w->blocks[l];
        const bool last = l == w->n_layers - 1;
        const int nq = (last && out_row0 == 0) ? n_out_rows : N;
        if (int rc = core_norm(w, cur, b.norm1_scale, b.norm1_bias, hbuf, M, st)) return rc;
        if (int rc = gemm_f32(hbuf, rd, b.in_proj_weight, b.in_proj_bias, nullptr, rd, wide, r3, M, 3 * d, d, AVD_ACT_NONE, st)) return rc;
        if (int rc = attn_f32(wide, hbuf, B, N, H, d / H, scale, nq, kpm, st)) return rc;
        if (int rc = gemm_f32(hbuf, rd, b.out_proj_weight, b.out_proj_bias, cur, rd, y, rd, M, d, d, AVD_ACT_NONE, st)) return rc;
        cur = y;
        if (int rc = core_norm(w, y, b.norm2_scale, b.norm2_bias, hbuf, M, st)) return rc;
        if (int rc = gemm_f32(hbuf, rd, b.fc1_weight, b.fc1_bias, nullptr, rd, wide, rh, M, hid, d, AVD_ACT_GELU, st)) return rc;
        if (int rc = gemm_f32(wide, rh, b.fc2_weight, b.fc2_bias, y, rd, y, rd, M, d, hid, AVD_ACT_NONE, st)) return rc;
    }
    return core_norm(w, y, w->final_norm_scale, w->final_norm_bias, y, M, st);
}

static bool head_split_capable(const avd_head_weights* w, int64_t rows) {
    if (w->split_terms == 0) return false;
    if (!w->input_proj_weight3 || !w->out_proj_weight3 || (w->n_shared > 0 && !w->shared_lin_weight3)) return false;
    for (int j = 0; j < w->n_shared; ++j)
        if (!w->shared_lin_weight3[j]) return false;
    if (w->split_terms == 3 && !w->f16x2_scale) return false;
    return gemm_bf16x3_supported(rows, w->hidden, w->d_in) && gemm_bf16x3_supported(rows, w->hidden, w->hidden) &&
           gemm_bf16x3_supported(rows, w->d_out, w->hidden);
}
static thread_local int64_t t_step_head_rows = 0;
static bool head_use_split(const avd_head_weights* w, int64_t rows) {
    return (t_step_head_rows > rows ? t_step_head_rows : rows) >= split_min_rows() && head_split_capable(w, rows);
}

static int64_t head_ws_bytes(const avd_head_weights* w, int64_t rows) {
    const int64_t fp32_path = 2 * align_up(rows * w->hidden * 4);
    if (!head_split_capable(w, rows)) return fp32_path;
    const int wide = w->d_in > w->hidden ? w->d_in : w->hidden;
    const int64_t split_path = 2 * align_up(split3_bytes(rows, wide)) + align_up(rows * w->hidden * 4);
    return split_path > fp32_path ? split_path : fp32_path;
}

static int head_forward(const avd_head_weights* w, const float* h, RowMap hm, int64_t rows, float* out, void* ws,
                        int64_t ws_bytes, hipStream_t st) {
    AVD_REQUIRE(w && h && out, AVD_EINVAL, "head: null pointer");
    AVD_REQUIRE(w->d_in > 0 && w->hidden > 0 && w->d_out > 0 && w->n_shared >= 0, AVD_EINVAL, "head: bad dims");
    AVD_REQUIRE(w->input_proj_weight && w->out_proj_weight, AVD_EINVAL, "head: null weights");
    AVD_REQUIRE(w->n_shared == 0 || (w->shared_lin_weight && w->shared_lin_bias && w->shared_ln_weight && w->shared_ln_bias),
                AVD_EINVAL, "head: null shared-trunk tables");
    AVD_REQUIRE(w->split_terms == 0 || w->split_terms == 6 || w->split_terms == 9 || w->split_terms == 1 || w->split_terms == 3, AVD_EINVAL,
                "head: split_terms must be 0 (fp32), 6, 9, 1 or 3, got %d", w->split_terms);
    AVD_REQUIRE(ws && ws_bytes >= head_ws_bytes(w, rows), AVD_EWORKSPACE, "head: workspace too small");
    Carver cv{static_cast<char*>(ws), 0, ws_bytes};
    const RowMap rh{w->hidden, 0, 0}, ro{w->d_out, 0, 0};
    if (head_use_split(w, rows)) {
        const int terms = w->split_terms, n = w->n_shared;
        const bool h2 = terms == 3;
        const float* fs = w->f16x2_scale;
        if (h2)
            for (int i = 0; i < 2 * (n + 2); ++i)
                AVD_REQUIRE(fs[i] > 0.f && fs[i] < __builtin_inff(), AVD_EINVAL, "head: f16x2_scale[%d] must be positive and finite", i);
        auto wsc = [&](int i) { return h2 ? fs[i] : 1.f; };
        auto asc = [&](int i) { return h2 ? fs[n + 2 + i] : 0.f; };
        const int wide = w->d_in > w->hidden ? w->d_in : w->hidden;
        void* imgA = cv.take((split3_bytes(rows, wide) + 3) / 4);
        void* imgB = cv.take((split3_bytes(rows, wide) + 3) / 4);
        float* t2 = cv.take(rows * w->hidden);
        if (int rc = split3_rows_f32(h, hm, imgA, rows, w->d_in, st, asc(0))) return rc;
        if (int rc = gemm_bf16x3(imgA, w->input_proj_weight3, w->input_proj_bias, nullptr, nullptr, imgB, rows, w->hidden, w->d_in, AVD_ACT_NONE,
                                 terms, st, h2 ? asc(0) * wsc(0) : 1.f, h2 ? asc(1) : 1.f)) return rc;
        void* cur = imgB;
        void* nxt = imgA;
        for (int j = 0; j < n; ++j) {
            if (int rc = gemm_bf16x3(cur, w->shared_lin_weight3[j], w->shared_lin_bias[j], nullptr, t2, nullptr, rows, w->hidden, w->hidden,
                                     AVD_ACT_NONE, terms, st, h2 ? asc(1 + j) * wsc(1 + j) : 1.f, 1.f)) return rc;
            if (int rc = layernorm_act_split3_f32(t2, w->shared_ln_weight[j], w->shared_ln_bias[j], nxt, rows, w->hidden, w->ln_eps, w->act, st,
                                                  asc(2 + j))) return rc;
            void* t = cur; cur = nxt; nxt = t;
        }
        return gemm_bf16x3(cur, w->out_proj_weight3, w->out_proj_bias, nullptr, out, nullptr, rows, w->d_out, w->hidden, AVD_ACT_NONE, terms, st,
                           h2 ? asc(1 + n) * wsc(1 + n) : 1.f, 1.f);
    }
    float* t1 = cv.take(rows * w->hidden);
    float* t2 = cv.take(rows * w->hidden);
    if (int rc = gemm_f32(h, hm, w->input_proj_weight, w->input_proj_bias, nullptr, rh, t1, rh, rows, w->hidden, w->d_in, AVD_ACT_NONE, st)) return rc;
    for (int j = 0; j < w->n_shared; ++j) {
        if (int rc = gemm_f32(t1, rh, w->shared_lin_weight[j], w->shared_lin_bias[j], nullptr, rh, t2, rh, rows, w->hidden, w->hidden, AVD_ACT_NONE, st)) return rc;
        if (int rc = layernorm_act_f32(t2, w->shared_ln_weight[j], w->shared_ln_bias[j], t1, rows, w->hidden, w->ln_eps, w->act, st)) return rc;
    }
    return gemm_f32(t1, rh, w->out_proj_weight, w->out_proj_bias, nullptr, ro, out, ro, rows, w->d_out, w->hidden, AVD_ACT_NONE, st);
}

static int check_embed(const avd_embed_desc* e) {
    AVD_REQUIRE(e, AVD_EINVAL, "embed: null descriptor");
    AVD_REQUIRE(e->B > 0 && e->d > 0 && e->tdim >= 0, AVD_EINVAL, "embed: bad widths");
    AVD_REQUIRE(e->temb_add ? e->tdim == e->d : e->tdim < e->d, AVD_EINVAL,
                "embed: timestep width %d does not fit token width %d in %s mode", e->tdim, e->d, e->temb_add ? "add" : "concat");
    AVD_REQUIRE(e->d % 4 == 0 && e->tdim % 4 == 0, AVD_EUNSUPPORTED, "embed: d and tdim must be multiples of 4");
    AVD_REQUIRE(e->Nt > 0 && e->Np >= 0, AVD_EINVAL, "embed: bad token counts");
    if (e->target_kind == 0) {
        AVD_REQUIRE(e->p0 > 0 && e->p1 > 0 && e->p2 > 0 && e->T % e->p0 == 0 && e->H % e->p1 == 0 && e->W % e->p2 == 0,
                    AVD_EINVAL, "tube sizes must divide latent dims");
        AVD_REQUIRE(e->Nt == (e->T / e->p0) * (e->H / e->p1) * (e->W / e->p2), AVD_EINVAL, "embed: token count mismatch");
    } else if (e->target_kind == 1) {
        AVD_REQUIRE(e->p0 > 0 && e->p1 > 0 && e->T >= e->p0, AVD_EINVAL, "embed: bad audio chunking");
        AVD_REQUIRE(e->Nt == (e->T - e->p0) / e->p1 + 1, AVD_EINVAL, "embed: token count mismatch");
    } else {
        return set_error(AVD_EINVAL, "embed: unknown target_kind %d", e->target_kind);
    }
    return AVD_OK;
}
static int embed_tok_dim(const avd_embed_desc* e) {
    return e->target_kind == 0 ? e->C * e->p0 * e->p1 * e->p2 : e->C * e->p0;
}
static int64_t embed_ws_floats(const avd_embed_desc* e) {
    return align_up((int64_t)e->B * e->Nt * embed_tok_dim(e) * 4) / 4 + align_up((int64_t)e->B * (e->tdim > 0 ? e->tdim : 1) * 4) / 4;
}

static int embed_slots(const avd_embed_desc* e, int& S, int& tok) {
    if (e->target_kind == 0) {
        S = e->T / e->p0;
        tok = (e->H / e->p1) * (e->W / e->p2);
    } else {
        AVD_REQUIRE(e->p1 == e->p0, AVD_EUNSUPPORTED, "slot timesteps need non-overlapping audio chunks (stride %d == len %d)", e->p1, e->p0);
        S = e->Nt;
        tok = 1;
    }
    return AVD_OK;
}

static int embed_cfg_pair(const avd_embed_desc* e, const float* z, const float* Wt, const float* bt,
                          const int64_t* t_now, const float* Xp, float* tok_ws, float* X2, hipStream_t st, float* ss_out = nullptr,
                          bool cond_only = false, const RowSegs* short_null = nullptr, int slots = 0) {
    if (int rc = check_embed(e)) return rc;
    int slot_tok = 0;
    if (slots) {
        int S = 0;
        if (int rc = embed_slots(e, S, slot_tok)) return rc;
        AVD_REQUIRE(slots == S, AVD_EINVAL, "embed: slots %d must equal the geometry's %d slots along the sliding axis", slots, S);
        AVD_REQUIRE(!e->temb_add && !cond_only, AVD_EINVAL, "embed: slot timesteps take the concat embedding of the CFG pair (temb_add == 0)");
    }
    AVD_REQUIRE(z && Wt && t_now && tok_ws && X2 && (e->Np == 0 || Xp), AVD_EINVAL, "embed: null pointer");
    AVD_REQUIRE(!short_null || (!cond_only && !e->temb_add && e->target_first && e->Np >= 1), AVD_EINVAL,
                "embed: the short null half is the concat-mode CFG pair with the target rows first");
    const int B = e->B, d = e->d, N = e->Nt + e->Np, D = embed_tok_dim(e);
    float* tok = tok_ws;
    float* temb = tok_ws + align_up((int64_t)B * e->Nt * D * 4) / 4;
    const bool fuse_patch = e->target_kind == 0 && !e->temb_add && e->p2 % 4 == 0 && e->W % 4 == 0 && D % 4 == 0 && aligned16(z);
    if (e->target_kind == 0) {
        if (!fuse_patch)
            if (int rc = tube_patch_f32(z, tok, B, e->C, e->T, e->H, e->W, e->p0, e->p1, e->p2, st)) return rc;
    } else {
        if (int rc = audio_tokens_f32(z, tok, B, e->C, e->T, e->p0, e->p1, st)) return rc;
    }
    if (e->tdim > 0 && e->temb_add)
        if (int rc = temb_f32(t_now, e->temb_freqs, temb, B, e->tdim, 10000.f, st)) return rc;
    float* c0 = X2 + (e->target_first ? 0 : (int64_t)e->Np * d);
    const RowMap cm{d, e->Nt, (int64_t)N * d};
    if (e->temb_add) {
        const RowMap rm{0, e->Nt, (int64_t)e->tdim};
        if (int rc = gemm_f32(tok, RowMap{D, 0, 0}, Wt, bt, temb, rm, c0, cm, (int64_t)B * e->Nt, d, D, AVD_ACT_NONE, st)) return rc;
        if (cond_only) return assemble_cond_f32(X2, temb, Xp, B, N, d, 0, e->Nt, e->Np, e->target_first, st);
        return assemble_f32(X2, temb, Xp, B, N, d, 0, e->Nt, e->Np, e->target_first, st);
    }
    if (fuse_patch) {
        const TubeGather tg{e->T, e->H, e->W, e->p0, e->p1, e->p2, e->H / e->p1, e->W / e->p2, e->Nt, (int64_t)e->C * e->T * e->H * e->W};
        if (int rc = gemm_f32_tube(z, tg, Wt, bt, c0, cm, (int64_t)B * e->Nt, d - e->tdim, D, st)) return rc;
    } else {
        if (int rc = gemm_f32(tok, RowMap{D, 0, 0}, Wt, bt, nullptr, cm, c0, cm, (int64_t)B * e->Nt, d - e->tdim, D, AVD_ACT_NONE, st)) return rc;
    }
    if (cond_only)
        return assemble_rows_cond_f32(X2, t_now, e->temb_freqs, Xp, ss_out, B, N, d, e->tdim, e->Nt, e->Np, e->target_first, 10000.f, st);
    return assemble_rows_f32(X2, t_now, e->temb_freqs, Xp, ss_out, B, N, d, e->tdim, e->Nt, e->Np, e->target_first, 10000.f, st,
                             short_null, slots, slot_tok);
}

#define AVD_HIP(call)                                                                        \
    do {                                                                                     \
        hipError_t e__ = (call);                                                             \
        if (e__ != hipSuccess) return set_error(AVD_ELAUNCH, "%s: %s", #call, hipGetErrorString(e__)); \
    } while (0)

struct AuxState { hipStream_t aux = nullptr; hipEvent_t fork = nullptr, join = nullptr; };
static std::mutex g_aux_mu;
static std::map<std::pair<int, hipStream_t>, AuxState> g_aux_map;
static int ensure_aux(hipStream_t st, AuxState& out) {
    int dev = 0;
    AVD_HIP(hipGetDevice(&dev));
    std::lock_guard<std::mutex> lk(g_aux_mu);
    AuxState& a = g_aux_map[{dev, st}];
    if (!a.aux) {
        AVD_HIP(hipStreamCreateWithFlags(&a.aux, hipStreamNonBlocking));
        AVD_HIP(hipEventCreateWithFlags(&a.fork, hipEventDisableTiming));
        AVD_HIP(hipEventCreateWithFlags(&a.join, hipEventDisableTiming));
    }
    out = a;
    return AVD_OK;
}

struct StepPlan {
    int64_t x2, tok, core, head, eps, ss, total;
    int N, D;
    int64_t rows;
};
static int plan_step(const avd_step_desc* s, StepPlan& p) {
    AVD_REQUIRE(s && s->core && s->head, AVD_EINVAL, "step: null descriptor");
    if (int rc = check_embed(&s->embed)) return rc;
    if (int rc = check_core(s->core)) return rc;
    const avd_embed_desc& e = s->embed;
    AVD_REQUIRE(e.d == s->core->d && s->head->d_in == e.d, AVD_EINVAL, "step: width mismatch between embed/core/head");
    p.N = e.Nt + e.Np;
    p.D = embed_tok_dim(&e);
    AVD_REQUIRE(s->head->d_out == p.D, AVD_EINVAL, "step: head d_out %d != token dim %d", s->head->d_out, p.D);
    p.rows = (int64_t)2 * e.B * e.Nt;
    p.x2 = align_up((int64_t)2 * e.B * p.N * e.d * 4);
    p.tok = align_up(embed_ws_floats(&e) * 4);
    const int64_t halves = 2 * core_ws_bytes(s->core, e.B, p.N), whole = core_ws_bytes(s->core, 2 * e.B, p.N);
    p.core = halves > whole ? halves : whole;
    const int64_t head_halves = 2 * head_ws_bytes(s->head, p.rows / 2), head_whole = head_ws_bytes(s->head, p.rows);
    p.head = head_halves > head_whole ? head_halves : head_whole;
    p.eps = align_up(p.rows * p.D * 4);
    p.ss = align_up((int64_t)2 * e.B * p.N * 4);
    p.total = p.x2 + p.tok + p.core + p.head + p.ss + p.eps;
    return AVD_OK;
}

struct StepWs {
    StepPlan p;
    float *X, *tok;
    void *core_ws, *head_ws;
    float *ssx, *eps;
};
static int open_step(const avd_step_desc* s, const float* z, const float* z_out, const int64_t* t_now, const int64_t* t_prev,
                     void* workspace, int64_t workspace_bytes, StepWs& ws) {
    StepPlan& p = ws.p;
    if (int rc = plan_step(s, p)) return rc;
    AVD_REQUIRE(z && z_out && t_now && t_prev && s->alpha_bar && s->adapt_w, AVD_EINVAL, "step: null pointer");
    AVD_REQUIRE(z != z_out, AVD_EINVAL, "step: z_out must not alias z");
    AVD_REQUIRE(workspace && workspace_bytes >= p.total, AVD_EWORKSPACE, "step: workspace %lld < %lld bytes",
                (long long)workspace_bytes, (long long)p.total);
    char* w = static_cast<char*>(workspace);
    ws.X = reinterpret_cast<float*>(w);
    ws.tok = reinterpret_cast<float*>(w + p.x2);
    ws.core_ws = w + p.x2 + p.tok;
    ws.head_ws = w + p.x2 + p.tok + p.core;
    ws.ssx = reinterpret_cast<float*>(w + p.x2 + p.tok + p.core + p.head);
    ws.eps = reinterpret_cast<float*>(w + p.x2 + p.tok + p.core + p.head + p.ss);
    return AVD_OK;
}

}

using namespace avd;

extern "C" int avd_abi_version(void) { return AVD_ABI_VERSION; }
extern "C" const char* avd_last_error(void) { return g_err; }

constexpr int kNoExcept = INT_MIN;
struct TuneKey { const char* key; const char* env; int* var; int lo, hi; bool boolean; int except = kNoExcept; };
static const TuneKey kTuneKeys[] = {
    {"s3_tile", "AVD_S3_TILE", &g_s3_tile, INT_MIN, INT_MAX, false},
    {"s3_m16", "AVD_S3_M16", &g_s3_m16, INT_MIN, INT_MAX, false},
    {"s3_rt", "AVD_S3_RT", &g_s3_rt, INT_MIN, INT_MAX, false},
    {"s3_rt4", "AVD_S3_RT4", &g_s3_rt4, 0, 8, false, 1},
    {"s3_deep4", "AVD_S3_DEEP4", &g_s3_deep4, INT_MIN, INT_MAX, true},
    {"s3_w128", "AVD_S3_W128", &g_s3_w128, INT_MIN, INT_MAX, false},
    {"s3_splitk", "AVD_S3_SPLITK", &g_s3_splitk, 0, kS3SplitKMax, false},
    {"s3_stagger", "AVD_S3_STAGGER", &g_s3_stagger, INT_MIN, INT_MAX, false},
    {"cfg_rows", "AVD_CFG_ROWS", &g_cfg_rows, INT_MIN, INT_MAX, true},
    {"vae_lat", "AVD_VAE_LAT", &g_vae_lat, INT_MIN, INT_MAX, true},
    {"vae_fold", "AVD_VAE_FOLD", &g_vae_fold, INT_MIN, INT_MAX, true},
    {"codec_mfma", "AVD_CODEC_MFMA", &g_codec_mfma, INT_MIN, INT_MAX, true},
    {"s3_sn", "AVD_S3_SN", &g_s3_sn, INT_MIN, INT_MAX, false},
    {"s3_super4", "AVD_S3_SUPER4", &g_s3_super4, INT_MIN, INT_MAX, false},
    {"s3_super8", "AVD_S3_SUPER8", &g_s3_super8, INT_MIN, INT_MAX, false},
    {"attn_pipe", "AVD_ATTN_PIPE", &g_attn_pipe, INT_MIN, INT_MAX, false},
    {"attn_m16", "AVD_ATTN_M16", &g_attn_m16, INT_MIN, INT_MAX, false},
    {"core_trim", "AVD_CORE_TRIM", &g_core_trim, INT_MIN, INT_MAX, true},
    {"mlp_fused", "AVD_MLP_FUSED", &g_mlp_fused, INT_MIN, INT_MAX, false},
    {"gemm_tile", "AVD_GEMM_TILE", &g_gemm_force_tile, INT_MIN, INT_MAX, false},
    {"gemm_stages", "AVD_GEMM_STAGES", &g_gemm_stages, INT_MIN, INT_MAX, false},
    {"gemm_splitk", "AVD_GEMM_SPLITK", &g_gemm_splitk, 0, kGemmSplitKMax, false},
    {"s3_min_rows", "AVD_S3_MIN_ROWS", &g_s3_min_rows, INT_MIN, INT_MAX, false},
    {"no_fold", "AVD_NO_FOLD", &g_no_fold, INT_MIN, INT_MAX, true},
};
static void tune_store(const TuneKey& t, int64_t value) { *t.var = t.boolean ? value != 0 : (int)value; }
[[maybe_unused]] static const bool g_tune_env_applied = [] {
    for (const TuneKey& t : kTuneKeys)
        if (const char* e = getenv(t.env)) {
            const long long v = atoll(e);
            tune_store(t, v < t.lo ? t.lo : v > t.hi ? t.hi : v);
        }
    return true;
}();

extern "C" int avd_tune_set(const char* key, int64_t value) {
    AVD_REQUIRE(key, AVD_EINVAL, "tune_set: null key");
    for (const TuneKey& t : kTuneKeys) {
        if (strcmp(key, t.key)) continue;
        AVD_REQUIRE(value >= t.lo && value <= t.hi && value != t.except, AVD_EINVAL, "tune_set: %s does not take %lld", key, (long long)value);
        tune_store(t, value);
        return AVD_OK;
    }
    return set_error(AVD_EINVAL, "tune_set: unknown key '%s'", key);
}

extern "C" int avd_cfg_dedup_set(int on) {
    const int prev = g_cfg_dedup;
    g_cfg_dedup = on != 0;
    return prev;
}

extern "C" int avd_device_arch(char* buf, int buflen) {
    AVD_REQUIRE(buf && buflen > 0, AVD_EINVAL, "device_arch: bad buffer");
    hipDeviceProp_t prop;
    int dev = 0;
    hipError_t e = hipGetDevice(&dev);
    if (e != hipSuccess) return set_error(AVD_ELAUNCH, "hipGetDevice: %s", hipGetErrorString(e));
    e = hipGetDeviceProperties(&prop, dev);
    if (e != hipSuccess) return set_error(AVD_ELAUNCH, "hipGetDeviceProperties: %s", hipGetErrorString(e));
    strncpy(buf, prop.gcnArchName, buflen - 1);
    buf[buflen - 1] = 0;
    return AVD_OK;
}

extern "C" int64_t avd_core_workspace_bytes(const avd_core_weights* w, int B, int N) {
    if (!w || B <= 0 || N <= 0) return -1;
    return core_ws_bytes(w, B, N);
}
extern "C" int avd_core_forward_f32(const avd_core_weights* w, const float* x, float* y, int B, int N, int out_row0,
                                    int n_out_rows, const uint8_t* key_padding_mask, void* workspace, int64_t workspace_bytes,
                                    avd_stream_t stream) {
    return core_forward(w, x, y, B, N, out_row0, n_out_rows, key_padding_mask, workspace, workspace_bytes,
                        static_cast<hipStream_t>(stream));
}

extern "C" int64_t avd_head_workspace_bytes(const avd_head_weights* w, int64_t rows) {
    if (!w || rows < 0) return -1;
    return head_ws_bytes(w, rows);
}
extern "C" int avd_head_forward_f32(const avd_head_weights* w, const float* h, int64_t ldh, int64_t seg_rows,
                                    int64_t seg_stride, int64_t rows, float* out, void* workspace,
                                    int64_t workspace_bytes, avd_stream_t stream) {
    return head_forward(w, h, RowMap{ldh, seg_rows, seg_stride}, rows, out, workspace, workspace_bytes,
                        static_cast<hipStream_t>(stream));
}

extern "C" int64_t avd_embed_workspace_floats(const avd_embed_desc* e) {
    if (check_embed(e)) return -1;
    return embed_ws_floats(e);
}
extern "C" int avd_embed_cfg_pair_f32(const avd_embed_desc* desc, const float* z_target, const float* Wt,
                                      const float* bt, const int64_t* t_now, const float* Xp, float* tok_ws, float* X2,
                                      avd_stream_t stream) {
    return embed_cfg_pair(desc, z_target, Wt, bt, t_now, Xp, tok_ws, X2, static_cast<hipStream_t>(stream));
}

extern "C" int avd_embed_cfg_pair_slots_f32(const avd_embed_desc* desc, const float* z_target, const float* Wt, const float* bt,
                                            const int64_t* t_now, int slots, const float* Xp, float* tok_ws, float* X2,
                                            avd_stream_t stream) {
    AVD_REQUIRE(slots > 0, AVD_EINVAL, "embed_cfg_pair_slots: slots must be > 0 (got %d)", slots);
    return embed_cfg_pair(desc, z_target, Wt, bt, t_now, Xp, tok_ws, X2, static_cast<hipStream_t>(stream), nullptr, false, nullptr, slots);
}

extern "C" int avd_embed_cond_f32(const avd_embed_desc* desc, const float* z_target, const float* Wt, const float* bt,
                                  const int64_t* t_now, const float* Xp, float* tok_ws, float* X1, float* ss, avd_stream_t stream) {
    return embed_cfg_pair(desc, z_target, Wt, bt, t_now, Xp, tok_ws, X1, static_cast<hipStream_t>(stream), ss, true);
}

extern "C" int64_t avd_step_workspace_bytes(const avd_step_desc* s) {
    StepPlan p;
    if (plan_step(s, p)) return -1;
    return p.total;
}

static int denoise_step(const avd_step_desc* s, const avd_noise_key* key, const float* z, const float* Xp, const int64_t* t_now,
                        const int64_t* t_prev, const float* noise, float* z_out, void* workspace, int64_t workspace_bytes,
                        avd_stream_t stream, const int64_t* t_last = nullptr, float* x0_hist = nullptr,
                        const avd_latent_guide* guide = nullptr, const avd_cfg_control* ctl = nullptr, int canvas_hop = 0,
                        int guide_hop = 0, int slots = 0, const avd_apg_control* apg = nullptr) {
    StepWs ws;
    if (int rc = open_step(s, z, z_out, t_now, t_prev, workspace, workspace_bytes, ws)) return rc;
    auto& [p, X2, tok, core_ws, head_ws, ssx, eps2] = ws;
    hipStream_t st = static_cast<hipStream_t>(stream);
    const avd_embed_desc& e = s->embed;
    const bool have_ss = !e.temb_add;

    const bool dedup = g_cfg_dedup && !s->split_streams && !e.temb_add && e.target_first && e.Np >= 2 && core_dedup_ok(s->core, 2 * e.B, p.N, e.Nt);
    const RowSegs seg{(int64_t)e.B * p.N, {p.N, e.Nt + 1}, {e.B, e.B}};
    if (int rc = embed_cfg_pair(&e, z, s->adapt_w, s->adapt_b, t_now, Xp, tok, X2, st, ssx, false, dedup ? &seg : nullptr, slots)) return rc;
    const int row0 = e.target_first ? 0 : e.Np;
    const RowMap hm{e.d, e.Nt, (int64_t)p.N * e.d};
    if (dedup) {
        if (int rc = core_forward(s->core, X2, X2, 2 * e.B, p.N, 0, e.Nt, nullptr, core_ws, p.core, st, nullptr, &seg)) return rc;
        if (int rc = head_forward(s->head, X2, RowMap{e.d, 0, 0}, p.rows, eps2, head_ws, p.head, st)) return rc;
    } else if (!s->split_streams) {
        if (int rc = core_forward(s->core, X2, X2, 2 * e.B, p.N, row0, e.Nt, nullptr, core_ws, p.core, st, have_ss ? ssx : nullptr)) return rc;
        if (int rc = head_forward(s->head, X2 + (int64_t)row0 * e.d, hm, p.rows, eps2, head_ws, p.head, st)) return rc;
    } else {
        AuxState ax;
        if (int rc = ensure_aux(st, ax)) return rc;
        hipStream_t g_aux = ax.aux;
        hipEvent_t g_fork = ax.fork, g_join = ax.join;
        const int64_t half_rows = (int64_t)e.B * p.N * e.d;
        const int64_t hc = p.core / 2, hh = p.head / 2;
        AVD_HIP(hipEventRecord(g_fork, st));
        AVD_HIP(hipStreamWaitEvent(g_aux, g_fork, 0));
        struct TwoStreams {
            TwoStreams(int64_t rows, int64_t head_rows) { t_s3_two_streams = true; t_step_rows = rows; t_step_head_rows = head_rows; }
            ~TwoStreams() { t_s3_two_streams = false; t_step_rows = 0; t_step_head_rows = 0; }
        } two_streams_scope((int64_t)2 * e.B * p.N, p.rows);
        for (int half = 0; half < 2; ++half) {
            hipStream_t hs = half ? g_aux : st;
            float* xh = X2 + half * half_rows;
            if (int rc = core_forward(s->core, xh, xh, e.B, p.N, row0, e.Nt, nullptr, static_cast<char*>(core_ws) + half * hc, hc, hs,
                                      have_ss ? ssx + (int64_t)half * e.B * p.N : nullptr)) return rc;
            if (int rc = head_forward(s->head, xh + (int64_t)row0 * e.d, hm, p.rows / 2, eps2 + half * (p.rows / 2) * p.D,
                                      static_cast<char*>(head_ws) + half * hh, hh, hs)) return rc;
        }
        AVD_HIP(hipEventRecord(g_join, g_aux));
        AVD_HIP(hipStreamWaitEvent(st, g_join, 0));
    }
    if (e.target_kind == 0)
        return cfg_unpatch_ddim_f32(eps2, z, t_now, t_prev, s->alpha_bar, s->T_train, s->guidance, s->eta, noise, z_out,
                                    e.B, e.C, e.T, e.H, e.W, e.p0, e.p1, e.p2, st, key, t_last, x0_hist, guide, ctl, canvas_hop,
                                    guide_hop, slots, apg);
    return cfg_untoken_ddim_audio_f32(eps2, z, t_now, t_prev, s->alpha_bar, s->T_train, s->guidance, s->eta, noise, z_out,
                                      e.B, e.C, e.T, e.p0, e.p1, st, key, t_last, x0_hist, guide, ctl, canvas_hop, guide_hop, slots, apg);
}

static int denoise_step_cond(const avd_step_desc* s, const avd_noise_key* key, const float* z, const float* Xp, const int64_t* t_now,
                             const int64_t* t_prev, const float* noise, float* z_out, void* workspace, int64_t workspace_bytes,
                             avd_stream_t stream, const int64_t* t_last, float* x0_hist, const avd_latent_guide* guide,
                             int canvas_hop = 0, int guide_hop = 0) {
    StepWs ws;
    if (int rc = open_step(s, z, z_out, t_now, t_prev, workspace, workspace_bytes, ws)) return rc;
    auto& [p, X1, tok, core_ws, head_ws, ssx, eps1] = ws;
    hipStream_t st = static_cast<hipStream_t>(stream);
    const avd_embed_desc& e = s->embed;
    const bool have_ss = !e.temb_add;

    if (int rc = embed_cfg_pair(&e, z, s->adapt_w, s->adapt_b, t_now, Xp, tok, X1, st, ssx, true)) return rc;
    const int row0 = e.target_first ? 0 : e.Np;
    const RowMap hm{e.d, e.Nt, (int64_t)p.N * e.d};
    if (int rc = core_forward(s->core, X1, X1, e.B, p.N, row0, e.Nt, nullptr, core_ws, p.core / 2, st, have_ss ? ssx : nullptr)) return rc;
    if (int rc = head_forward(s->head, X1 + (int64_t)row0 * e.d, hm, p.rows / 2, eps1, head_ws, p.head / 2, st)) return rc;
    if (e.target_kind == 0)
        return eps_unpatch_ddim_f32(eps1, z, t_now, t_prev, s->alpha_bar, s->T_train, s->eta, noise, z_out, e.B, e.C, e.T, e.H, e.W, e.p0,
                                    e.p1, e.p2, st, key, t_last, x0_hist, guide, canvas_hop, guide_hop);
    return eps_untoken_ddim_audio_f32(eps1, z, t_now, t_prev, s->alpha_bar, s->T_train, s->eta, noise, z_out, e.B, e.C, e.T, e.p0, e.p1, st,
                                      key, t_last, x0_hist, guide, canvas_hop, guide_hop);
}

enum { NEED_KEY = 1, NEED_HIST = 2, NEED_GUIDE = 4, NEED_CTL = 8, TAKES_SDE = 16 };
static int check_step_options(const char* what, int need, const avd_step_desc* s, const avd_noise_key* key, const int64_t* t_last,
                              const float* x0_hist, const float* z, const float* z_out, const avd_latent_guide* g,
                              const avd_cfg_control* ctl, const float* noise, bool takes_noise = false) {
    AVD_REQUIRE(s, AVD_EINVAL, "step: null descriptor");
    const int B = s->embed.B;
    const int64_t n = (int64_t)B * s->embed.C * s->embed.T * s->embed.H * s->embed.W, per = B > 0 ? n / B : 0;
    if (ctl || (need & NEED_CTL))
        if (int rc = check_cfg_control(ctl, B, per, z_out, x0_hist)) return rc;
    if (g || (need & NEED_GUIDE))
        if (int rc = check_latent_guide(g, B, per, z_out, x0_hist)) return rc;
    AVD_REQUIRE(!(need & NEED_HIST) || (t_last && x0_hist), AVD_EINVAL, "%s: null t_last or x0_hist", what);
    AVD_REQUIRE(!t_last == !x0_hist, AVD_EINVAL, "%s: t_last and x0_hist go together (the DPM-Solver++(2M) update)", what);
    if (x0_hist) {
        AVD_REQUIRE(s->eta == 0.f || (need & TAKES_SDE), AVD_EINVAL,
                    "%s: DPM-Solver++(2M) needs eta == 0 here (eta > 0 is avd_denoise_step_dpmpp_2m_sde_f32)", what);
        AVD_REQUIRE(!(z && overlaps(x0_hist, z, n)) && !(z_out && overlaps(x0_hist, z_out, n)), AVD_EINVAL,
                    "%s: x0_hist must not alias z or z_out", what);
    }
    AVD_REQUIRE(key || !(need & NEED_KEY), AVD_EINVAL, "%s: null noise key", what);
    AVD_REQUIRE(!(noise && key), AVD_EINVAL, "%s: pass a noise tensor or a noise key, not both", what);
    AVD_REQUIRE(!(noise && g), AVD_EINVAL, "%s: unseeded noise is not supported with a latent guide (pass a noise key)", what);
    AVD_REQUIRE(s->eta == 0.f || key || noise, AVD_EINVAL, "%s: eta > 0 needs a noise key%s", what,
                takes_noise && !g ? " or a noise tensor" : " (unseeded noise is not supported here)");
    if (key)
        AVD_REQUIRE(key->sample_offset >= 0 && key->sample_offset + (int64_t)B <= ((int64_t)1 << 32), AVD_EINVAL,
                    "%s: sample_offset %lld + B %d must lie in [0, 2^32]", what, (long long)key->sample_offset, B);
    return AVD_OK;
}

extern "C" int avd_denoise_step_cond_f32(const avd_step_desc* s, const avd_latent_guide* g, const avd_noise_key* key,
                                         const int64_t* t_last, float* x0_hist, const float* z, const float* Xp, const int64_t* t_now,
                                         const int64_t* t_prev, const float* noise, float* z_out, void* workspace,
                                         int64_t workspace_bytes, avd_stream_t stream) {
    if (int rc = check_step_options("denoise_step_cond", 0, s, key, t_last, x0_hist, z, z_out, g, nullptr, noise, true)) return rc;
    return denoise_step_cond(s, key, z, Xp, t_now, t_prev, noise, z_out, workspace, workspace_bytes, stream, t_last, x0_hist, g);
}

extern "C" int avd_denoise_step_f32(const avd_step_desc* s, const float* z, const float* Xp, const int64_t* t_now,
                                    const int64_t* t_prev, const float* noise, float* z_out, void* workspace,
                                    int64_t workspace_bytes, avd_stream_t stream) {
    return denoise_step(s, nullptr, z, Xp, t_now, t_prev, noise, z_out, workspace, workspace_bytes, stream);
}

extern "C" int avd_denoise_step_slots_f32(const avd_step_desc* s, const float* z, const float* Xp, const int64_t* t_now,
                                          const int64_t* t_prev, int slots, float* z_out, void* workspace, int64_t workspace_bytes,
                                          avd_stream_t stream) {
    AVD_REQUIRE(s, AVD_EINVAL, "denoise_step_slots: null descriptor");
    AVD_REQUIRE(s->eta == 0.f, AVD_EINVAL, "denoise_step_slots: slot timesteps take the DDIM update at eta == 0 (eta is %g)", (double)s->eta);
    AVD_REQUIRE(!s->embed.temb_add, AVD_EINVAL, "denoise_step_slots: slot timesteps take the concat embedding (temb_add == 0)");
    if (int rc = check_embed(&s->embed)) return rc;
    int S = 0, tok = 0;
    if (int rc = embed_slots(&s->embed, S, tok)) return rc;
    AVD_REQUIRE(slots == S, AVD_EINVAL, "denoise_step_slots: slots %d must equal the geometry's %d slots along the sliding axis", slots, S);
    return denoise_step(s, nullptr, z, Xp, t_now, t_prev, nullptr, z_out, workspace, workspace_bytes, stream, nullptr, nullptr, nullptr,
                        nullptr, 0, 0, slots);
}

extern "C" int avd_denoise_step_slots_dpmpp_2m_f32(const avd_step_desc* s, const float* z, const float* Xp, const int64_t* t_last,
                                                   const int64_t* t_now, const int64_t* t_prev, int slots, float* x0_hist, float* z_out,
                                                   void* workspace, int64_t workspace_bytes, avd_stream_t stream) {
    AVD_REQUIRE(s, AVD_EINVAL, "denoise_step_slots_dpmpp_2m: null descriptor");
    AVD_REQUIRE(s->eta == 0.f, AVD_EINVAL, "denoise_step_slots_dpmpp_2m: slot timesteps take the ODE update at eta == 0 (eta is %g)",
                (double)s->eta);
    AVD_REQUIRE(!s->embed.temb_add, AVD_EINVAL, "denoise_step_slots_dpmpp_2m: slot timesteps take the concat embedding (temb_add == 0)");
    if (int rc = check_embed(&s->embed)) return rc;
    int S = 0, tok = 0;
    if (int rc = embed_slots(&s->embed, S, tok)) return rc;
    AVD_REQUIRE(slots == S, AVD_EINVAL, "denoise_step_slots_dpmpp_2m: slots %d must equal the geometry's %d slots along the sliding axis",
                slots, S);
    if (int rc = check_step_options("denoise_step_slots_dpmpp_2m", NEED_HIST, s, nullptr, t_last, x0_hist, z, z_out, nullptr, nullptr, nullptr))
        return rc;
    AVD_REQUIRE(aligned16(x0_hist), AVD_EUNSUPPORTED, "denoise_step_slots_dpmpp_2m: x0_hist must be 16-byte aligned");
    return denoise_step(s, nullptr, z, Xp, t_now, t_prev, nullptr, z_out, workspace, workspace_bytes, stream, t_last, x0_hist, nullptr,
                        nullptr, 0, 0, slots);
}

extern "C" int avd_denoise_step_seeded_f32(const avd_step_desc* s, const avd_noise_key* key, const float* z, const float* Xp,
                                           const int64_t* t_now, const int64_t* t_prev, float* z_out, void* workspace,
                                           int64_t workspace_bytes, avd_stream_t stream) {
    if (int rc = check_step_options("denoise_step_seeded", NEED_KEY, s, key, nullptr, nullptr, z, z_out, nullptr, nullptr, nullptr)) return rc;
    return denoise_step(s, key, z, Xp, t_now, t_prev, nullptr, z_out, workspace, workspace_bytes, stream);
}

extern "C" int avd_denoise_step_dpmpp_2m_f32(const avd_step_desc* s, const float* z, const float* Xp, const int64_t* t_last,
                                             const int64_t* t_now, const int64_t* t_prev, float* x0_hist, float* z_out, void* workspace,
                                             int64_t workspace_bytes, avd_stream_t stream) {
    if (int rc = check_step_options("denoise_step_dpmpp_2m", NEED_HIST, s, nullptr, t_last, x0_hist, z, z_out, nullptr, nullptr, nullptr))
        return rc;
    return denoise_step(s, nullptr, z, Xp, t_now, t_prev, nullptr, z_out, workspace, workspace_bytes, stream, t_last, x0_hist);
}

extern "C" int avd_denoise_step_guided_f32(const avd_step_desc* s, const avd_latent_guide* g, const avd_noise_key* key,
                                           const int64_t* t_last, float* x0_hist, const float* z, const float* Xp, const int64_t* t_now,
                                           const int64_t* t_prev, float* z_out, void* workspace, int64_t workspace_bytes,
                                           avd_stream_t stream) {
    if (int rc = check_step_options("denoise_step_guided", NEED_GUIDE, s, key, t_last, x0_hist, z, z_out, g, nullptr, nullptr)) return rc;
    return denoise_step(s, key, z, Xp, t_now, t_prev, nullptr, z_out, workspace, workspace_bytes, stream, t_last, x0_hist, g);
}

extern "C" int avd_denoise_step_cfg_f32(const avd_step_desc* s, const avd_cfg_control* ctl, const avd_latent_guide* g,
                                        const avd_noise_key* key, const int64_t* t_last, float* x0_hist, const float* z, const float* Xp,
                                        const int64_t* t_now, const int64_t* t_prev, float* z_out, void* workspace,
                                        int64_t workspace_bytes, avd_stream_t stream) {
    if (int rc = check_step_options("denoise_step_cfg", NEED_CTL, s, key, t_last, x0_hist, z, z_out, g, ctl, nullptr)) return rc;
    return denoise_step(s, key, z, Xp, t_now, t_prev, nullptr, z_out, workspace, workspace_bytes, stream, t_last, x0_hist, g, ctl);
}

extern "C" int avd_denoise_step_canvas_f32(const avd_step_desc* s, const avd_noise_key* key, int hop, const avd_cfg_control* ctl,
                                           const avd_latent_guide* g, int cond_only, const float* z, const float* Xp,
                                           const int64_t* t_now, const int64_t* t_prev, float* z_out, void* workspace,
                                           int64_t workspace_bytes, avd_stream_t stream) {
    AVD_REQUIRE(s, AVD_EINVAL, "denoise_step_canvas: null descriptor");
    AVD_REQUIRE(key, AVD_EINVAL, "denoise_step_canvas: null noise key");
    AVD_REQUIRE(s->eta > 0.f, AVD_EINVAL, "denoise_step_canvas: canvas keying is the seeded eta > 0 DDIM step (eta is %g)", (double)s->eta);
    AVD_REQUIRE(!(cond_only && ctl), AVD_EINVAL, "denoise_step_canvas: a cond-only step takes no CFG control");
    const avd_embed_desc& e = s->embed;
    if (int rc = check_canvas_key(key, e.B, e.C, e.T, hop, (int64_t)e.H * e.W)) return rc;
    if (int rc = check_step_options("denoise_step_canvas", NEED_KEY, s, key, nullptr, nullptr, z, z_out, g, ctl, nullptr)) return rc;
    if (cond_only)
        return denoise_step_cond(s, key, z, Xp, t_now, t_prev, nullptr, z_out, workspace, workspace_bytes, stream, nullptr, nullptr, g, hop);
    return denoise_step(s, key, z, Xp, t_now, t_prev, nullptr, z_out, workspace, workspace_bytes, stream, nullptr, nullptr, g, ctl, hop);
}

extern "C" int avd_denoise_step_dpmpp_2m_sde_f32(const avd_step_desc* s, const avd_noise_key* key, int canvas_hop,
                                                 const avd_cfg_control* ctl, const avd_latent_guide* g, int cond_only,
                                                 const int64_t* t_last, float* x0_hist, const float* z, const float* Xp,
                                                 const int64_t* t_now, const int64_t* t_prev, float* z_out, void* workspace,
                                                 int64_t workspace_bytes, avd_stream_t stream) {
    AVD_REQUIRE(s, AVD_EINVAL, "denoise_step_dpmpp_2m_sde: null descriptor");
    AVD_REQUIRE(s->eta > 0.f, AVD_EINVAL, "denoise_step_dpmpp_2m_sde: the SDE form needs eta > 0 (eta is %g: avd_denoise_step_dpmpp_2m_f32)",
                (double)s->eta);
    AVD_REQUIRE(key, AVD_EINVAL, "denoise_step_dpmpp_2m_sde: null noise key (the SDE form draws seeded noise only)");
    AVD_REQUIRE(t_last && x0_hist, AVD_EINVAL, "denoise_step_dpmpp_2m_sde: null t_last or x0_hist");
    AVD_REQUIRE(!(cond_only && ctl), AVD_EINVAL, "denoise_step_dpmpp_2m_sde: a cond-only step takes no CFG control");
    AVD_REQUIRE(canvas_hop >= 0, AVD_EINVAL, "denoise_step_dpmpp_2m_sde: canvas_hop must be >= 0 (0: per-sample keying), got %d", canvas_hop);
    const avd_embed_desc& e = s->embed;
    if (canvas_hop)
        if (int rc = check_canvas_key(key, e.B, e.C, e.T, canvas_hop, (int64_t)e.H * e.W)) return rc;
    if (int rc = check_step_options("denoise_step_dpmpp_2m_sde", NEED_KEY | NEED_HIST | TAKES_SDE, s, key, t_last, x0_hist, z, z_out, g, ctl,
                                    nullptr)) return rc;
    if (cond_only)
        return denoise_step_cond(s, key, z, Xp, t_now, t_prev, nullptr, z_out, workspace, workspace_bytes, stream, t_last, x0_hist, g,
                                 canvas_hop);
    return denoise_step(s, key, z, Xp, t_now, t_prev, nullptr, z_out, workspace, workspace_bytes, stream, t_last, x0_hist, g, ctl, canvas_hop);
}
// ... 84 lines not shown
```

multimodal_diffusion_amd/csrc/rowops.hip:

```cpp
#include "avd_common.h"

namespace avd {

constexpr int ROW_MAXV = 8;

template <int NV>
__global__ __launch_bounds__(256) void rmsnorm_kernel(const float* x, RowMap xm,
                                                      const float* __restrict__ scale, float* y,
                                                      RowMap ym, int64_t rows, int d, float eps, float sqrt_d) {
    const int lane = threadIdx.x & 63;
    const int64_t row = (int64_t)blockIdx.x * 4 + (threadIdx.x >> 6);
    if (row >= rows) return;
    const float* xr = x + xm.off(row);
    f32x4 v[NV];
    float ss = 0.f;
#pragma unroll
    for (int i = 0; i < NV; ++i) {
        const int c = (lane + 64 * i) * 4;
        if (c < d) {
            v[i] = *reinterpret_cast<const f32x4*>(xr + c);
            ss += v[i][0] * v[i][0] + v[i][1] * v[i][1] + v[i][2] * v[i][2] + v[i][3] * v[i][3];
        }
    }
    ss = wave_sum(ss);
    const float den = sqrtf(ss) / sqrt_d + eps;
    float* yr = y + ym.off(row);
#pragma unroll
    for (int i = 0; i < NV; ++i) {
        const int c = (lane + 64 * i) * 4;
        if (c < d) {
            const f32x4 s = *reinterpret_cast<const f32x4*>(scale + c);
            f32x4 o = {s[0] * v[i][0] / den, s[1] * v[i][1] / den, s[2] * v[i][2] / den, s[3] * v[i][3] / den};
            *reinterpret_cast<f32x4*>(yr + c) = o;
        }
    }
}

template <int NV>
__global__ __launch_bounds__(256) void layernorm_act_kernel(const float* x,
                                                            const float* __restrict__ gamma,
                                                            const float* __restrict__ beta, float* y,
                                                            int64_t rows, int d, float eps, int act) {
    const int lane = threadIdx.x & 63;
    const int64_t row = (int64_t)blockIdx.x * 4 + (threadIdx.x >> 6);
    if (row >= rows) return;
    const float* xr = x + row * d;
    f32x4 v[NV];
    float s = 0.f;
#pragma unroll
    for (int i = 0; i < NV; ++i) {
        const int c = (lane + 64 * i) * 4;
        if (c < d) {
            v[i] = *reinterpret_cast<const f32x4*>(xr + c);
            s += v[i][0] + v[i][1] + v[i][2] + v[i][3];
        }
    }
    const float mean = wave_sum(s) / (float)d;
    float q = 0.f;
#pragma unroll
    for (int i = 0; i < NV; ++i) {
        const int c = (lane + 64 * i) * 4;
        if (c < d) {
#pragma unroll
            for (int e = 0; e < 4; ++e) {
                const float t = v[i][e] - mean;
                q += t * t;
            }
        }
    }
    const float var = wave_sum(q) / (float)d;
    const float rstd = 1.0f / sqrtf(var + eps);
    float* yr = y + row * d;
#pragma unroll
    for (int i = 0; i < NV; ++i) {
        const int c = (lane + 64 * i) * 4;
        if (c < d) {
            const f32x4 gm = *reinterpret_cast<const f32x4*>(gamma + c);
            const f32x4 bt = *reinterpret_cast<const f32x4*>(beta + c);
            f32x4 o;
#pragma unroll
            for (int e = 0; e < 4; ++e) {
                float t = (v[i][e] - mean) * rstd * gm[e] + bt[e];
                if (act == AVD_ACT_GELU) t = gelu_erf(t);
                else if (act == AVD_ACT_SILU) t = silu(t);
                else if (act == AVD_ACT_RELU) t = fmaxf(t, 0.f);
                else if (act == AVD_ACT_LEAKY_RELU) t = t > 0.f ? t : 0.1f * t;
                o[e] = t;
            }
            *reinterpret_cast<f32x4*>(yr + c) = o;
        }
    }
}

static int nv_for(int d) { return (d + 255) / 256; }

int rmsnorm_f32(const float* x, RowMap xm, const float* scale, float* y, RowMap ym, int64_t rows, int d, float eps,
                hipStream_t st) {
    AVD_REQUIRE(x && scale && y, AVD_EINVAL, "rmsnorm: null pointer");
    AVD_REQUIRE(rows >= 0 && d > 0, AVD_EINVAL, "rmsnorm: bad dims");
    AVD_REQUIRE(d % 4 == 0 && d <= 256 * ROW_MAXV, AVD_EUNSUPPORTED, "rmsnorm: d=%d must be a multiple of 4, <= %d", d,
                256 * ROW_MAXV);
    AVD_REQUIRE(xm.ld % 4 == 0 && ym.ld % 4 == 0 && aligned16(x) && aligned16(y) && aligned16(scale), AVD_EUNSUPPORTED,
                "rmsnorm: rows must be 16-byte aligned");
    if (rows == 0) return AVD_OK;
    const int tag = prof_tag_id("rmsnorm_kernel<%d>", nv_for(d));
    ProfScope prof(tag, 8.0 * (double)rows * d, st);
    const unsigned grid = (unsigned)((rows + 3) / 4);
    const float isd = (float)sqrt((double)d);
    switch (nv_for(d)) {
#define AVD_CASE(NV) case NV: hipLaunchKernelGGL(rmsnorm_kernel<NV>, dim3(grid), dim3(256), 0, st, x, xm, scale, y, ym, rows, d, eps, isd); break;
        AVD_CASE(1) AVD_CASE(2) AVD_CASE(3) AVD_CASE(4) AVD_CASE(5) AVD_CASE(6) AVD_CASE(7) AVD_CASE(8)
#undef AVD_CASE
    }
    AVD_CHECK_LAUNCH("rmsnorm");
    return AVD_OK;
}

__global__ __launch_bounds__(256) void rowss_kernel(const float* __restrict__ x, float* __restrict__ ss, int64_t rows, int d) {
    const int lane = threadIdx.x & 63;
    const int64_t row = (int64_t)blockIdx.x * 4 + (threadIdx.x >> 6);
    if (row >= rows) return;
    const float* xr = x + row * d;
    float s = 0.f;
    for (int c = lane * 4; c < d; c += 256) {
        const f32x4 v = *reinterpret_cast<const f32x4*>(xr + c);
        s += v[0] * v[0] + v[1] * v[1] + v[2] * v[2] + v[3] * v[3];
    }
    s = wave_sum(s);
    if (lane == 0) ss[row] = s;
}

int rowss_f32(const float* x, float* ss, int64_t rows, int d, hipStream_t st) {
    AVD_REQUIRE(x && ss && rows > 0 && d > 0 && d % 4 == 0 && aligned16(x), AVD_EINVAL, "rowss: bad arguments");
    static const int tag = prof_tag_id("rowss_kernel");
    ProfScope prof(tag, 4.0 * (double)rows * d, st);
    hipLaunchKernelGGL(rowss_kernel, dim3((unsigned)((rows + 3) / 4)), dim3(256), 0, st, x, ss, rows, d);
    AVD_CHECK_LAUNCH("rowss");
    return AVD_OK;
}

__global__ __launch_bounds__(256) void bounds_kernel(const float* __restrict__ x, float* __restrict__ out, int64_t rows, int d) {
    const int lane = threadIdx.x & 63;
    const int64_t row = (int64_t)blockIdx.x * 4 + (threadIdx.x >> 6);
    if (row >= rows) return;
    const float* xr = x + row * d;
    float s = 0.f, m = 0.f;
    bool bad = false;
    for (int c = lane; c < d; c += 64) {
        const float v = xr[c];
        s += v * v;
        m = fmaxf(m, fabsf(v));
        bad = bad || v != v;
    }
    s = wave_sum(s);
#pragma unroll
    for (int o = 32; o > 0; o >>= 1) m = fmaxf(m, __shfl_xor(m, o, 64));
    bad = __any(bad);
    if (lane == 0) {
        const float nrm = bad ? __builtin_nanf("") : sqrtf(s);
        const float mx = bad ? __builtin_nanf("") : m;
        atomicMax(reinterpret_cast<unsigned int*>(out), __float_as_uint(mx));
        atomicMax(reinterpret_cast<unsigned int*>(out) + 1, __float_as_uint(nrm));
    }
}
__global__ void bounds_init_kernel(float* out) { out[threadIdx.x] = 0.f; }

int weight_bounds_f32(const float* x, int64_t rows, int d, float* out2, hipStream_t st) {
    AVD_REQUIRE(x && out2 && rows > 0 && d > 0, AVD_EINVAL, "weight_bounds: bad arguments");
    hipLaunchKernelGGL(bounds_init_kernel, dim3(1), dim3(2), 0, st, out2);
    hipLaunchKernelGGL(bounds_kernel, dim3((unsigned)((rows + 3) / 4)), dim3(256), 0, st, x, out2, rows, d);
    AVD_CHECK_LAUNCH("weight_bounds");
    return AVD_OK;
}

int layernorm_act_f32(const float* x, const float* gamma, const float* beta, float* y, int64_t rows, int d, float eps,
                      int act, hipStream_t st) {
    AVD_REQUIRE(x && gamma && beta && y, AVD_EINVAL, "layernorm: null pointer");
    AVD_REQUIRE(rows >= 0 && d > 0, AVD_EINVAL, "layernorm: bad dims");
    AVD_REQUIRE(d % 4 == 0 && d <= 256 * ROW_MAXV, AVD_EUNSUPPORTED, "layernorm: d=%d must be a multiple of 4, <= %d",
                d, 256 * ROW_MAXV);
    AVD_REQUIRE(aligned16(x) && aligned16(y) && aligned16(gamma) && aligned16(beta), AVD_EUNSUPPORTED,
                "layernorm: pointers must be 16-byte aligned");
    if (rows == 0) return AVD_OK;
    const int tag = prof_tag_id("layernorm_act_kernel<%d>", nv_for(d));
    ProfScope prof(tag, 8.0 * (double)rows * d, st);
    const unsigned grid = (unsigned)((rows + 3) / 4);
    switch (nv_for(d)) {
#define AVD_CASE(NV) case NV: hipLaunchKernelGGL(layernorm_act_kernel<NV>, dim3(grid), dim3(256), 0, st, x, gamma, beta, y, rows, d, eps, act); break;
        AVD_CASE(1) AVD_CASE(2) AVD_CASE(3) AVD_CASE(4) AVD_CASE(5) AVD_CASE(6) AVD_CASE(7) AVD_CASE(8)
#undef AVD_CASE
    }
    AVD_CHECK_LAUNCH("layernorm_act");
    return AVD_OK;
}

}

extern "C" int avd_rmsnorm_f32(const float* x, const float* scale, float* y, int64_t rows, int d, float eps,
                               avd_stream_t stream) {
    return avd::rmsnorm_f32(x, avd::RowMap{d, 0, 0}, scale, y, avd::RowMap{d, 0, 0}, rows, d, eps,
                            static_cast<hipStream_t>(stream));
}

extern "C" int avd_weight_bounds_f32(const float* w, int64_t rows, int cols, float* out2, avd_stream_t stream) {
    return avd::weight_bounds_f32(w, rows, cols, out2, static_cast<hipStream_t>(stream));
}

extern "C" int avd_layernorm_act_f32(const float* x, const float* gamma, const float* beta, float* y, int64_t rows,
                                     int d, float eps, int act, avd_stream_t stream) {
    return avd::layernorm_act_f32(x, gamma, beta, y, rows, d, eps, act, static_cast<hipStream_t>(stream));
}
```

multimodal_diffusion_amd/functional.py:

```python
from __future__ import annotations

import ctypes as C
import math
import numbers
from typing import Optional

import torch

from . import _lib as L

Tensor = torch.Tensor


def _st(t: Tensor) -> int:
    return L.stream_ptr(t.device)


def rmsnorm(x: Tensor, scale: Tensor, eps: float = 1e-6) -> Tensor:
    x = L.dev_f32(x, "x")
    scale = L.dev_f32(scale, "scale")
    d = x.shape[-1]
    y = torch.empty_like(x)
    L.check(L.lib().avd_rmsnorm_f32(x.data_ptr(), scale.data_ptr(), y.data_ptr(), x.numel() // d, d, eps, _st(x)))
    return y


def linear(x: Tensor, weight: Tensor, bias: Optional[Tensor] = None, act: int = L.ACT_NONE,
           residual: Optional[Tensor] = None) -> Tensor:
    x = L.dev_f32(x, "x")
    weight = L.dev_f32(weight, "weight")
    n, k = weight.shape
    if x.shape[-1] != k:
        raise RuntimeError(f"mat1 and mat2 shapes cannot be multiplied ({tuple(x.shape)} x {k}->{n})")
    m = x.numel() // k
    out = torch.empty(*x.shape[:-1], n, device=x.device, dtype=torch.float32)
    b = None if bias is None else L.dev_f32(bias, "bias")
    r = None
    if residual is not None:
        r = L.dev_f32(residual, "residual")
        if r.shape != out.shape:
            raise RuntimeError("residual shape mismatch")
    L.check(L.lib().avd_gemm_bias_act_f32(x.data_ptr(), k, weight.data_ptr(), L.ptr(b), L.ptr(r), n, out.data_ptr(), n,
                                          m, n, k, act, _st(x)))
    return out


def linear_rmsfold(x: Tensor, weight_n: Tensor, bias: Optional[Tensor] = None, act: int = L.ACT_NONE,
                   residual: Optional[Tensor] = None, ss_in: Optional[Tensor] = None, eps: float = 1e-6, want_ss: bool = False):
    x = L.dev_f32(x, "x")
    weight_n = L.dev_f32(weight_n, "weight")
    n, k = weight_n.shape
    m = x.numel() // k
    y = torch.empty(*x.shape[:-1], n, device=x.device, dtype=torch.float32)
    ss_out = torch.empty(m, n // 32, device=x.device, dtype=torch.float32) if want_ss else None
    cols = 0 if ss_in is None else ss_in.shape[-1]
    L.check(L.lib().avd_gemm_rmsfold_f32(x.data_ptr(), weight_n.data_ptr(), L.ptr(bias), L.ptr(residual), y.data_ptr(), m, n, k,
                                         act, L.ptr(ss_in), cols, eps, L.ptr(ss_out), _st(x)))
    return y, ss_out


def key_padding_bytes(mask: Optional[Tensor], B: int, N: int, device: torch.device) -> Optional[Tensor]:
    if mask is None:
        return None
    if mask.is_floating_point():
        raise NotImplementedError("key_padding_mask must be boolean / integer (True = padding), as MMDiT.forward documents")
    if tuple(mask.shape) != (B, N):
        raise RuntimeError(f"key_padding_mask shape {tuple(mask.shape)} != {(B, N)}")
    if not mask.is_cuda:
        raise L.AvdError("key_padding_mask must be on the ROCm device (no CPU fallback)")
    return (mask != 0).to(torch.uint8).contiguous()


def attention(qkv: Tensor, n_heads: int, n_query: Optional[int] = None, key_padding_mask: Optional[Tensor] = None) -> Tensor:
    qkv = L.dev_f32(qkv, "qkv")
    B, N, d3 = qkv.shape
    kpm = key_padding_bytes(key_padding_mask, B, N, qkv.device)
    d = d3 // 3
    dh = d // n_heads
    out = torch.empty(B, N, d, device=qkv.device, dtype=torch.float32) if n_query in (None, N) else \
        torch.zeros(B, N, d, device=qkv.device, dtype=torch.float32)
    L.check(L.lib().avd_attn_fwd_f32(qkv.data_ptr(), out.data_ptr(), B, N, n_heads, dh, 1.0 / math.sqrt(dh),
                                     N if n_query is None else n_query, L.ptr(kpm), _st(qkv)))
    return out


def layernorm_act(x: Tensor, weight: Tensor, bias: Tensor, eps: float = 1e-5, act: int = L.ACT_NONE) -> Tensor:
    x = L.dev_f32(x, "x")
    d = x.shape[-1]
    y = torch.empty_like(x)
    L.check(L.lib().avd_layernorm_act_f32(x.data_ptr(), L.dev_f32(weight).data_ptr(), L.dev_f32(bias).data_ptr(),
                                          y.data_ptr(), x.numel() // d, d, eps, act, _st(x)))
    return y


_FREQS = {}


def temb_freqs(dim: int, max_period: int, device: torch.device) -> Tensor:
    key = (dim, max_period, str(device))
    if key not in _FREQS:
        half = dim // 2
        f = torch.exp(-math.log(max_period) * torch.arange(0, half, dtype=torch.float32) / half)
        _FREQS[key] = f.to(device)
    return _FREQS[key]


def timestep_embedding(t: Tensor, dim: int, max_period: int = 10000) -> Tensor:
    if not t.is_cuda:
        raise L.AvdError("timesteps must be on the ROCm device (no CPU fallback)")
    if t.is_floating_point():
        if not torch.equal(t, t.round()):
            raise L.AvdError("fractional timesteps are not supported by the HIP path")
    t = L.dev_i64(t, t.device)
    out = torch.empty(t.shape[0], dim, device=t.device, dtype=torch.float32)
    fr = temb_freqs(dim, max_period, t.device) if dim >= 2 else None
    L.check(L.lib().avd_timestep_embedding_f32(t.data_ptr(), L.ptr(fr), out.data_ptr(), t.shape[0], dim,
                                               float(max_period), _st(out)))
    return out


def tube_patch(z: Tensor, t: int, h: int, w: int) -> Tensor:
    z = L.dev_f32(z, "z")
    B, C_, T, H, W = z.shape
    assert T % t == 0 and H % h == 0 and W % w == 0, "tube sizes must divide latent dims"
    n = (T // t) * (H // h) * (W // w)
    tok = torch.empty(B, n, C_ * t * h * w, device=z.device, dtype=torch.float32)
    L.check(L.lib().avd_tube_patch_f32(z.data_ptr(), tok.data_ptr(), B, C_, T, H, W, t, h, w, _st(z)))
    return tok


def tube_unpatch(tokens: Tensor, C_: int, T: int, H: int, W: int, t: int, h: int, w: int) -> Tensor:
    tokens = L.dev_f32(tokens, "tokens")
    B, N, D = tokens.shape
    assert D == C_ * t * h * w, "token width mismatch"
    assert N == (T // t) * (H // h) * (W // w), "token count mismatch"
    z = torch.empty(B, C_, T, H, W, device=tokens.device, dtype=torch.float32)
    L.check(L.lib().avd_tube_unpatch_f32(tokens.data_ptr(), z.data_ptr(), B, C_, T, H, W, t, h, w, _st(z)))
    return z


def audio_tokens(z_a: Tensor, length: int, stride: int) -> Tensor:
    z_a = L.dev_f32(z_a, "z_a")
    B, Ca, F = z_a.shape
    if length <= 0 or stride <= 0 or F < length:
        raise L.AvdError(f"audio_tokens: need 0 < len <= F and stride > 0 (got F={F} len={length} stride={stride})")
    na = (F - length) // stride + 1
    tok = torch.empty(B, na, Ca * length, device=z_a.device, dtype=torch.float32)
    L.check(L.lib().avd_audio_tokens_f32(z_a.data_ptr(), tok.data_ptr(), B, Ca, F, length, stride, _st(z_a)))
    return tok


def audio_untokens(tokens: Tensor, Ca: int, length: int, frames: int, stride: int, window: Optional[Tensor] = None) -> Tensor:
    tokens = L.dev_f32(tokens, "tokens")
    if window is not None:
        window = L.dev_f32(window, "window")
        assert window.numel() == length
    B, na, D = tokens.shape
    assert D == Ca * length
# ... 438 lines not shown
    elif not (hist_out.is_cuda and hist_out.dtype == torch.float32 and hist_out.is_contiguous() and hist_out.shape == hist.shape and
              hist_out.device == hist.device):
        raise ValueError(f"hist_out must be a contiguous float32 tensor of hist's shape {tuple(hist.shape)} on its device")
    L.check(L.lib().avd_fifo_shift_hist_f32(C.byref(key), t, c, z.data_ptr(), out.data_ptr(), popped.data_ptr(), hist.data_ptr(),
                                            hist_out.data_ptr(), z.shape[0], outer, L_ // slot_len, slot_len, inner, _st(z)))
    return out, popped, hist_out


def fifo_lookahead(z: Tensor, ctx: int, shift: int, slot_len: int, c: Optional[int] = None, seed: Optional[int] = None,
                   t: Optional[int] = None, hist: Optional[Tensor] = None, hist_out: Optional[Tensor] = None):
    z = L.dev_f32(z, "z")
    if hist is None and hist_out is not None:
        raise ValueError("hist_out goes with hist")
    if hist is not None and not (hist.is_cuda and hist.dtype == torch.float32 and hist.is_contiguous() and hist.shape == z.shape and
                                 hist.device == z.device):
        raise ValueError(f"hist must be a contiguous float32 tensor of z's shape {tuple(z.shape)} on z's device")
    outer, L_, inner = window_dims(z.shape)
    if isinstance(slot_len, bool) or not isinstance(slot_len, int) or slot_len < 1 or L_ % slot_len:
        raise ValueError(f"slot_len must be an int >= 1 that divides the sliding length {L_}, got {slot_len!r}")
    S = L_ // slot_len
    if isinstance(ctx, bool) or not isinstance(ctx, int) or not 0 <= ctx < S:
        raise ValueError(f"the lookahead ctx must be an int in [0, S = {S}), got {ctx!r}")
    if isinstance(shift, bool) or shift not in (0, 1):
        raise ValueError(f"shift must be 0 or 1, got {shift!r}")
    popped, key = None, None
    if shift:
        for name, v in (("c", c), ("t", t)):
            if isinstance(v, bool) or not isinstance(v, int) or v < 0:
                raise ValueError(f"{name} must be an int >= 0 at shift=1, got {v!r}")
        if (c + 1) * slot_len > 2 ** 32:
            raise ValueError(f"(c {c} + 1) * slot_len {slot_len} exceeds the stream's 2**32 canvas positions")
        if seed is None:
            raise ValueError("shift=1 draws the entering slot's noise from a seed: pass one")
        key = C.byref(noise_key(seed, 0))
        popped = torch.empty((z.shape[1], slot_len) + tuple(z.shape[3:]), device=z.device, dtype=torch.float32)
    elif c is not None or seed is not None or t is not None:
        raise ValueError("shift=0 draws nothing: leave c, seed and t None")
    out = torch.empty_like(z)
    head = (key, t or 0, c or 0, shift, z.data_ptr(), out.data_ptr(), L.ptr(popped))
    tail = (z.shape[0], outer, S, ctx, slot_len, inner, _st(z))
    if hist is None:
        L.check(L.lib().avd_fifo_lookahead_f32(*head, *tail))
        return out, popped
    if hist_out is None:
        hist_out = torch.empty_like(hist)
    elif not (hist_out.is_cuda and hist_out.dtype == torch.float32 and hist_out.is_contiguous() and hist_out.shape == hist.shape and
              hist_out.device == hist.device):
        raise ValueError(f"hist_out must be a contiguous float32 tensor of hist's shape {tuple(hist.shape)} on its device")
    L.check(L.lib().avd_fifo_lookahead_hist_f32(*head, hist.data_ptr(), hist_out.data_ptr(), *tail))
    return out, popped, hist_out


def _cursor(cursor: Tensor, device: torch.device) -> Tensor:
    if not (isinstance(cursor, Tensor) and cursor.is_cuda and cursor.dtype == torch.int32 and cursor.numel() == 1 and
            cursor.device == device):
        raise ValueError("a cursor is one int32 in device memory (a 1-element int32 tensor on the buffers' device)")
    return cursor


def cursor_add(cursor: Tensor, delta: int = 1) -> None:
    L.check(L.lib().avd_cursor_add(_cursor(cursor, cursor.device).data_ptr(), int(delta), _st(cursor)))


def stack_slot_tables(rows: Tensor) -> Tensor:
    rows = torch.as_tensor(rows)
    if rows.dim() != 3 or rows.is_floating_point() or rows.dtype == torch.bool:
        raise ValueError(f"slot tables are integer [n_rows, B, S], got {rows.dtype} {tuple(rows.shape)}")
    return rows.to(torch.long).reshape(rows.shape[0], rows.shape[1] * rows.shape[2]).contiguous()


def slot_tables_select(tables, cursor: Tensor, outs) -> None:
    tables, outs = list(tables), list(outs)
    if len(tables) not in (2, 3) or len(outs) != len(tables):
        raise ValueError("slot_tables_select takes two or three tables and as many buffers")
    dev = tables[0].device
    n_rows, n = (int(v) for v in tables[0].shape) if tables[0].dim() == 2 else (0, 0)
    for t in tables:
        if not (t.is_cuda and t.dtype == torch.long and t.is_contiguous() and t.dim() == 2 and tuple(t.shape) == (n_rows, n) and t.device == dev):
            raise ValueError("tables must be contiguous int64 [n_rows, n] device tensors of one shape")
    for o in outs:
        if not (o.is_cuda and o.dtype == torch.long and o.is_contiguous() and o.numel() == n and o.device == dev):
            raise ValueError(f"every buffer must be a contiguous int64 device tensor of {n} elements")
    p = [t.data_ptr() for t in tables] + [None] * (3 - len(tables))
    q = [o.data_ptr() for o in outs] + [None] * (3 - len(outs))
    L.check(L.lib().avd_slot_tables_select(*p, n_rows, n, _cursor(cursor, dev).data_ptr(), *q, L.stream_ptr(dev)))


def fifo_prompt_gather(prompt_canvas: Tensor, cursor: Tensor, B: int, S: int, prompt_hop: int, prompt_len: int,
                       out: Optional[Tensor] = None) -> Tensor:
    pc = prompt_canvas
    if not (isinstance(pc, Tensor) and pc.is_cuda and pc.dtype == torch.float32 and pc.is_contiguous() and pc.dim() in (2, 4)):
        raise ValueError("a prompt canvas is a contiguous float32 device tensor [C, P, H, W] (video) or [Ca, P] (audio)")
    for name, v in (("B", B), ("S", S), ("prompt_hop", prompt_hop), ("prompt_len", prompt_len)):
        if isinstance(v, bool) or not isinstance(v, int) or not 1 <= v < 2 ** 31:
            raise ValueError(f"{name} must be an int in [1, 2**31), got {v!r}")
    shape = (B, pc.shape[0], prompt_len) + tuple(pc.shape[2:])
    if out is None:
        out = torch.empty(shape, device=pc.device, dtype=torch.float32)
    elif not (out.is_cuda and out.dtype == torch.float32 and out.is_contiguous() and tuple(out.shape) == shape and out.device == pc.device):
        raise ValueError(f"out must be a contiguous float32 tensor of shape {shape} on the canvas's device")
    inner = pc.shape[2] * pc.shape[3] if pc.dim() == 4 else 1
    L.check(L.lib().avd_fifo_prompt_gather_f32(pc.data_ptr(), _cursor(cursor, pc.device).data_ptr(), out.data_ptr(), B, S, prompt_hop,
                                               pc.shape[0], pc.shape[1], prompt_len, inner, _st(pc)))
    return out


def fifo_shift_cursor(z: Tensor, c0: int, cursor: Tensor, clip: Tensor, seed: int, t: int, slot_len: int, out: Optional[Tensor] = None,
                      hist: Optional[Tensor] = None, hist_out: Optional[Tensor] = None):
    z = L.dev_f32(z, "z")
    outer, L_, inner = window_dims(z.shape)
    if isinstance(slot_len, bool) or not isinstance(slot_len, int) or slot_len < 1 or L_ % slot_len:
        raise ValueError(f"slot_len must be an int >= 1 that divides the sliding length {L_}, got {slot_len!r}")
    for name, v in (("c0", c0), ("t", t)):
        if isinstance(v, bool) or not isinstance(v, int) or v < 0:
            raise ValueError(f"{name} must be an int >= 0, got {v!r}")
    if not (isinstance(clip, Tensor) and clip.is_cuda and clip.dtype == torch.float32 and clip.is_contiguous() and clip.device == z.device and
            clip.dim() == z.dim() - 1 and clip.shape[0] == z.shape[1] and tuple(clip.shape[2:]) == tuple(z.shape[3:]) and
            clip.shape[1] >= slot_len and clip.shape[1] % slot_len == 0):
        raise ValueError(f"clip must be a contiguous float32 canvas [{z.shape[1]}, n_out * {slot_len}, ...] of z's slice shape on z's device")
    n_out = clip.shape[1] // slot_len
    if (c0 + n_out) * slot_len > 2 ** 32:
        raise ValueError(f"(c0 {c0} + n_out {n_out}) * slot_len {slot_len} exceeds the stream's 2**32 canvas positions")
    if hist is None and hist_out is not None:
        raise ValueError("hist_out goes with hist")
    bufs = [("out", out)] + ([("hist", hist), ("hist_out", hist_out)] if hist is not None else [])
    for name, b in bufs:
        if b is not None and not (b.is_cuda and b.dtype == torch.float32 and b.is_contiguous() and b.shape == z.shape and b.device == z.device):
            raise ValueError(f"{name} must be a contiguous float32 tensor of z's shape {tuple(z.shape)} on z's device")
    key = noise_key(seed, 0)
    out = torch.empty_like(z) if out is None else out
    head = (C.byref(key), t, c0, _cursor(cursor, z.device).data_ptr(), n_out, z.data_ptr(), out.data_ptr(), clip.data_ptr())
    tail = (z.shape[0], outer, L_ // slot_len, slot_len, inner, _st(z))
    if hist is None:
        L.check(L.lib().avd_fifo_shift_cursor_f32(*head, *tail))
        return out
    hist_out = torch.empty_like(hist) if hist_out is None else hist_out
    L.check(L.lib().avd_fifo_shift_cursor_hist_f32(*head, hist.data_ptr(), hist_out.data_ptr(), *tail))
    return out, hist_out


def split3(x: Tensor, out: Optional[Tensor] = None) -> Tensor:
    x = L.dev_f32(x, "x")
    k = x.shape[-1]
    rows = x.numel() // k
    nbytes = L.lib().avd_split3_bytes(rows, k)
    if nbytes < 0:
        raise L.AvdError(f"split3: K={k} must be a multiple of 16")
    if out is None or out.numel() != nbytes or out.device != x.device:
        out = torch.empty(nbytes, dtype=torch.uint8, device=x.device)
    L.check(L.lib().avd_split3_f32(x.data_ptr(), out.data_ptr(), rows, k, _st(x)))
    return out


def rmsnorm_split3(x: Tensor, scale: Tensor, eps: float = 1e-6) -> Tensor:
    x = L.dev_f32(x, "x")
    scale = L.dev_f32(scale, "scale")
    d = x.shape[-1]
    rows = x.numel() // d
    out = torch.empty(L.lib().avd_split3_bytes(rows, d), dtype=torch.uint8, device=x.device)
    L.check(L.lib().avd_rmsnorm_split3_f32(x.data_ptr(), scale.data_ptr(), out.data_ptr(), rows, d, eps, _st(x)))
    return out


def linear_bf16x3(x3: Tensor, rows: int, w3: Tensor, n: int, k: int, bias: Optional[Tensor] = None,
                  residual: Optional[Tensor] = None, act: int = L.ACT_NONE, out_split3: bool = False, terms: int = 6) -> Tensor:
    b = None if bias is None else L.dev_f32(bias, "bias")
    r = None if residual is None else L.dev_f32(residual, "residual")
    if out_split3:
        out = torch.empty(L.lib().avd_split3_bytes(rows, n), dtype=torch.uint8, device=x3.device)
        c, c3 = None, out.data_ptr()
    else:
        out = torch.empty(rows, n, dtype=torch.float32, device=x3.device)
        c, c3 = out.data_ptr(), None
    L.check(L.lib().avd_gemm_bf16x3_f32(x3.data_ptr(), w3.data_ptr(), L.ptr(b), L.ptr(r), c, c3, rows, n, k, act, terms, _st(x3)))
    return out


def f16x2_scale(bound: float) -> float:
    import math
    bound = float(bound) * 1.01
    if not math.isfinite(bound):
        raise L.AvdError("f16x2: the bound on the operand's magnitude is not finite")
    if bound <= 0.0:
        return 1.0
    e = 15 - math.ceil(math.log2(bound))
    return float(2.0 ** max(-100, min(100, e)))


def weight_bounds(tensors) -> list:
    tensors = [L.dev_f32(t.detach(), "weight") for t in tensors]
    if not tensors:
        return []
    out = torch.empty(len(tensors), 2, dtype=torch.float32, device=tensors[0].device)
    for i, t in enumerate(tensors):
        cols = t.shape[-1]
        rows = t.numel() // cols
        L.check(L.lib().avd_weight_bounds_f32(t.data_ptr(), rows, cols, out[i].data_ptr(), _st(t)))
    return [(float(a), float(b)) for a, b in out.cpu().tolist()]


def split_f16x2(x: Tensor, scale: Optional[float] = None, out: Optional[Tensor] = None):
    x = L.dev_f32(x, "x")
    k = x.shape[-1]
    rows = x.numel() // k
    nbytes = L.lib().avd_split3_bytes(rows, k)
    if nbytes < 0:
        raise L.AvdError(f"split_f16x2: K={k} must be a multiple of 16")
    if scale is None:
        scale = f16x2_scale(weight_bounds([x.reshape(rows, k)])[0][0])
    if out is None or out.numel() != nbytes or out.device != x.device:
        out = torch.empty(nbytes, dtype=torch.uint8, device=x.device)
    L.check(L.lib().avd_split_f16x2_f32(x.data_ptr(), out.data_ptr(), rows, k, scale, _st(x)))
    return out, scale


def rmsnorm_split_f16x2(x: Tensor, gamma: Tensor, eps: float = 1e-6, scale: Optional[float] = None):
    x = L.dev_f32(x, "x")
    gamma = L.dev_f32(gamma, "scale")
    d = x.shape[-1]
    rows = x.numel() // d
    if scale is None:
        scale = f16x2_scale(weight_bounds([gamma])[0][0] * d ** 0.5)
    out = torch.empty(L.lib().avd_split3_bytes(rows, d), dtype=torch.uint8, device=x.device)
    L.check(L.lib().avd_rmsnorm_split_f16x2_f32(x.data_ptr(), gamma.data_ptr(), out.data_ptr(), rows, d, eps, scale, _st(x)))
    return out, scale


def linear_f16x2(x2: Tensor, rows: int, w2: Tensor, n: int, k: int, ab_scale: float, bias: Optional[Tensor] = None,
                 residual: Optional[Tensor] = None, act: int = L.ACT_NONE, out_scale: Optional[float] = None) -> Tensor:
    b = None if bias is None else L.dev_f32(bias, "bias")
    r = None if residual is None else L.dev_f32(residual, "residual")
    if out_scale is not None:
        out = torch.empty(L.lib().avd_split3_bytes(rows, n), dtype=torch.uint8, device=x2.device)
        c, c2 = None, out.data_ptr()
    else:
        out = torch.empty(rows, n, dtype=torch.float32, device=x2.device)
        c, c2 = out.data_ptr(), None
    L.check(L.lib().avd_gemm_f16x2_f32(x2.data_ptr(), w2.data_ptr(), L.ptr(b), L.ptr(r), c, c2, rows, n, k, act, ab_scale,
                                       1.0 if out_scale is None else out_scale, _st(x2)))
    return out
```

multimodal_diffusion_amd/noise_heads.py:

```python
from __future__ import annotations

import ctypes as C
from typing import Dict, List, Optional, Union

import torch
import torch.nn as nn

from . import _lib as L

__all__ = ["MultiModalNoiseHead"]

_ACTS = {"gelu": L.ACT_GELU, "relu": L.ACT_RELU, "leaky_relu": L.ACT_LEAKY_RELU}


def _act_code(name: str) -> int:
    name = (name or "gelu").lower()
    if name in _ACTS:
        return _ACTS[name]
    raise ValueError(f"Unsupported activation: {name}")


class _Marker(nn.Module):
    """Parameter-free placeholder keeping Sequential indices (activation / dropout slots) aligned."""


def _trunk_block(hidden: int) -> nn.Sequential:
    return nn.Sequential(nn.Linear(hidden, hidden), nn.LayerNorm(hidden), _Marker(), _Marker())


def _init_linear(m: nn.Module):
    if isinstance(m, nn.Linear):
        nn.init.xavier_uniform_(m.weight)
        if m.bias is not None:
            nn.init.zeros_(m.bias)


class MultiModalNoiseHead(nn.Module):
    def __init__(self, input_dims: Dict[str, int], output_dims: Dict[str, int], hidden_dim: int = 512,
                 num_shared_layers: int = 2, num_modality_specific_layers: int = 1, dropout: float = 0.1,
                 activation: str = "gelu", share_parameters: bool = False):
        super().__init__()
        self.modalities = list(input_dims.keys())
        self.input_dims = {k: int(v) for k, v in input_dims.items()}
        self.output_dims = {k: int(v) for k, v in output_dims.items()}
        self.hidden_dim = int(hidden_dim)
        self.share_parameters = bool(share_parameters)
        self.dropout = float(dropout)
        self._act = _act_code(activation)

        self.input_proj = nn.ModuleDict({m: nn.Linear(self.input_dims[m], self.hidden_dim) for m in self.modalities})
        self.shared = None if num_shared_layers <= 0 else \
            nn.Sequential(*[_trunk_block(self.hidden_dim) for _ in range(num_shared_layers)])
        n_spec = max(0, num_modality_specific_layers - 1)
        if num_modality_specific_layers <= 0 or self.share_parameters:
            if num_modality_specific_layers > 0:
                self.shared_specific_trunk = nn.Sequential(*[_trunk_block(self.hidden_dim) for _ in range(n_spec)]) \
                    if n_spec > 0 else nn.Identity()
            self.spec = nn.ModuleDict({m: nn.Identity() for m in self.modalities})
        else:
            self.spec = nn.ModuleDict({
                m: nn.Sequential(*[_trunk_block(self.hidden_dim) for _ in range(n_spec)]) if n_spec > 0 else nn.Identity()
                for m in self.modalities})
        self.out_proj = nn.ModuleDict({m: nn.Linear(self.hidden_dim, self.output_dims[m]) for m in self.modalities})
        self.apply(_init_linear)
        self._ws: Optional[torch.Tensor] = None
        self.matmul = "auto"
        self._images: dict = {}

    def get_output_dim(self, modality: str) -> int:
        return int(self.output_dims[modality])

    def _trunk(self, m: str) -> List[nn.Sequential]:
        blocks: List[nn.Sequential] = list(self.shared) if self.shared is not None else []
        if self.share_parameters and hasattr(self, "shared_specific_trunk"):
            if not isinstance(self.shared_specific_trunk, nn.Identity):
                blocks += list(self.shared_specific_trunk)
        elif not isinstance(self.spec[m], nn.Identity):
            blocks += list(self.spec[m])
        return blocks

    def _image(self, name: str, p: torch.Tensor, h2_scale: float) -> torch.Tensor:
        from . import functional as Fn
        key = (p.data_ptr(), p._version, tuple(p.shape), float(h2_scale))
        hit = self._images.get(name)
        if hit is None or hit[0] != key:
            old = hit[1] if hit is not None and hit[0][2] == key[2] and hit[1].device == p.device else None
            img = Fn.split_f16x2(p.detach(), h2_scale, out=old)[0] if h2_scale > 0 else Fn.split3(p.detach(), out=old)
            hit = (key, img)
            self._images[name] = hit
        return hit[1]

    def _f16x2_scales(self, m: str, blocks, in_bound: float, in_norm: float):
        from . import functional as Fn
        ps = [self.input_proj[m].weight, self.input_proj[m].bias] + [q for b in blocks for q in (b[0].weight, b[1].weight, b[1].bias)] + \
            [self.out_proj[m].weight]
        key = (tuple((q.data_ptr(), q._version) for q in ps), float(in_bound), float(in_norm))
        hit = self._images.get(f"{m}.f16x2")
        if hit is None or hit[0] != key:
            wi, bi = self.input_proj[m].weight, self.input_proj[m].bias
            ts = [wi, bi] + [t for b in blocks for t in (b[0].weight, b[1].weight, b[1].bias)] + [self.out_proj[m].weight]
            bd = Fn.weight_bounds(ts)
            q = [bd[0][0], bd[0][1], bd[1][0]] + [bd[2 + j][0] for j in range(3 * len(blocks))] + [bd[-1][0]]
            w_in, wn_in, b_in = q[0], q[1], q[2]
            w_sc = [Fn.f16x2_scale(w_in)] + [Fn.f16x2_scale(q[3 + 3 * j]) for j in range(len(blocks))] + [Fn.f16x2_scale(q[-1])]
            a_sc = [Fn.f16x2_scale(in_bound), Fn.f16x2_scale(in_norm * wn_in + b_in)]
            a_sc += [Fn.f16x2_scale(self.hidden_dim ** 0.5 * q[4 + 3 * j] + q[5 + 3 * j]) for j in range(len(blocks))]
            hit = (key, w_sc + a_sc)
            self._images[f"{m}.f16x2"] = hit
        return hit[1]

    def weight_table(self, m: str, matmul: Optional[str] = None, in_bound: Optional[float] = None, in_norm: Optional[float] = None):
        matmul = self.matmul if matmul is None else matmul
        if matmul not in L.MATMUL_TERMS:
            raise ValueError(f"matmul must be one of {sorted(L.MATMUL_TERMS)}, got {matmul!r}")
        blocks = self._trunk(m)
        n = len(blocks)
        keep = []

        def dp(p):
            t = L.dev_f32(p.detach(), "head parameter")
            keep.append(t)
            return t.data_ptr()

        arrs = [(C.c_void_p * max(n, 1))() for _ in range(5)]
        for j, blk in enumerate(blocks):
            arrs[0][j], arrs[1][j] = dp(blk[0].weight), dp(blk[0].bias)
            arrs[2][j], arrs[3][j] = dp(blk[1].weight), dp(blk[1].bias)
        eps = blocks[0][1].eps if n else 1e-5
        hw = L.HeadWeights(self.input_dims[m], self.hidden_dim, self.output_dims[m], n, eps, self._act,
                           dp(self.input_proj[m].weight), dp(self.input_proj[m].bias),
                           C.cast(arrs[0], C.POINTER(C.c_void_p)), C.cast(arrs[1], C.POINTER(C.c_void_p)),
                           C.cast(arrs[2], C.POINTER(C.c_void_p)), C.cast(arrs[3], C.POINTER(C.c_void_p)),
                           dp(self.out_proj[m].weight), dp(self.out_proj[m].bias))
        terms = L.MATMUL_TERMS[matmul]
        shapes_ok = self.input_dims[m] % 16 == 0 and self.hidden_dim % 256 == 0 and self.output_dims[m] % 256 == 0
        if terms and shapes_ok:
            sc = None
            if matmul == "f16x2":
                if in_bound is None or in_norm is None:
                    raise ValueError("matmul='f16x2' needs in_bound / in_norm (bounds on the head's input rows)")
                sc = self._f16x2_scales(m, blocks, in_bound, in_norm)
                scales = (C.c_float * len(sc))(*sc)
                arrs.append(scales)
                hw.f16x2_scale = C.cast(scales, C.POINTER(C.c_float))
            ws = [self.input_proj[m].weight] + [b[0].weight for b in blocks] + [self.out_proj[m].weight]
            imgs = [self._image(f"{m}.{i}", w, sc[i] if sc else 0.0) for i, w in enumerate(ws)]
            keep += imgs
            hw.split_terms = terms
            hw.input_proj_weight3 = imgs[0].data_ptr()
            for j in range(n):
                arrs[4][j] = imgs[1 + j].data_ptr()
            hw.shared_lin_weight3 = C.cast(arrs[4], C.POINTER(C.c_void_p))
            hw.out_proj_weight3 = imgs[-1].data_ptr()
        return hw, (arrs, keep)

    def forward(self, inputs: Dict[str, torch.Tensor], return_dict: bool = True
                ) -> Union[Dict[str, torch.Tensor], torch.Tensor]:
        if self.training and self.dropout > 0:
            raise NotImplementedError("HIP path is inference-only; call .eval()")
        outputs: Dict[str, torch.Tensor] = {}
        for m in self.modalities:
            if m not in inputs or inputs[m] is None:
                continue
            x = L.dev_f32(inputs[m], f"inputs[{m}]")
            d_in = x.shape[-1]
            if d_in != self.input_dims[m]:
                raise RuntimeError(f"{m}: expected last dim {self.input_dims[m]}, got {d_in}")
            rows = x.numel() // d_in
            if self.matmul == "f16x2":
                from . import functional as Fn
                amax = Fn.weight_bounds([x.reshape(rows, d_in)])[0][0]
                hw, keep = self.weight_table(m, in_bound=amax, in_norm=amax * d_in ** 0.5)
            else:
                hw, keep = self.weight_table(m)
            need = L.lib().avd_head_workspace_bytes(C.byref(hw), rows)
            if self._ws is None or self._ws.numel() < need or self._ws.device != x.device:
                self._ws = torch.empty(max(need, 1), dtype=torch.uint8, device=x.device)
            out = torch.empty(*x.shape[:-1], self.output_dims[m], device=x.device, dtype=torch.float32)
            L.check(L.lib().avd_head_forward_f32(C.byref(hw), x.data_ptr(), d_in, 0, 0, rows, out.data_ptr(),
                                                 self._ws.data_ptr(), self._ws.numel(), L.stream_ptr(x.device)))
            del keep
            outputs[m] = out
        if return_dict:
            return outputs
        for m in self.modalities:
            if m in outputs:
                return outputs[m]
        raise ValueError("No modalities found in inputs for MultiModalNoiseHead.forward")
```

multimodal_diffusion_amd/sampler.py:

```python
from __future__ import annotations

import ctypes as C
from typing import Dict, Optional, Tuple

import numpy as np
import torch
import torch.nn as nn

from . import _lib as L
from . import _pipeline as P
from . import functional as Fn
from . import ops
from . import schedule_utils as su
from ._pipeline import tube_from_config
from .mmdt import MMDiT
from .noise_heads import MultiModalNoiseHead


class LinearAdapter(nn.Module):

    def __init__(self, d_in: int, d_out: int):
        super().__init__()
        self.proj = nn.Linear(d_in, d_out)

    def forward(self, x: torch.Tensor) -> torch.Tensor:
        return Fn.linear(x, self.proj.weight, self.proj.bias)


def add_sinusoidal_timestep(tokens: torch.Tensor, t_scalar: torch.Tensor, dim: int) -> torch.Tensor:
    emb = su.timestep_embedding(L.dev_i64(t_scalar, tokens.device), dim)
    out = torch.empty(tokens.shape[0], tokens.shape[1], tokens.shape[2] + dim, device=tokens.device, dtype=tokens.dtype)
    out[..., :tokens.shape[2]] = tokens
    out[..., tokens.shape[2]:] = emb[:, None, :]
    return out


def build_components(cfg: Dict, device: torch.device, vid_vae: Optional[nn.Module] = None,
                     aud_codec: Optional[nn.Module] = None):
    matmul = str(cfg.get("runtime", {}).get("matmul", "auto"))
    if matmul not in L.MATMUL_TERMS:
        raise ValueError(f"runtime.matmul must be one of {sorted(L.MATMUL_TERMS)}, got {matmul!r}")
    if vid_vae is None and "video" in cfg:
        from .vae_video3d import VideoVAE
        vid_vae = VideoVAE.from_config(cfg["video"]).to(device).eval()
        vid_vae.matmul = matmul if matmul in ("auto", "f32", "bf16x3", "f16x2") else "bf16x3"
    if aud_codec is None and "audio" in cfg:
        from .audio_codec import AudioCodec
        aud_codec = AudioCodec.from_config(cfg["audio"]).to(device).eval()
    d = int(cfg["tokenizer"]["width"])
    out_v = int(cfg["model"]["heads"]["video"]["out_dim"])
    out_a = int(cfg["model"]["heads"]["audio"]["out_dim"])
    tstep_dim = int(cfg["embeddings"].get("timestep_dim", 256))
    adapt_v = LinearAdapter(out_v, d - tstep_dim).to(device)
    adapt_a = LinearAdapter(out_a, d - tstep_dim).to(device)
    core = MMDiT(**cfg["model"]["core"]).to(device).eval()
    core.matmul = matmul
    head = MultiModalNoiseHead(
        input_dims={"video": d, "audio": d}, output_dims={"video": out_v, "audio": out_a},
        hidden_dim=int(cfg["model"]["heads"]["video"]["hidden_dim"]), num_shared_layers=2,
        num_modality_specific_layers=1, dropout=float(cfg["model"]["core"].get("dropout", 0.1)),
        activation=cfg["model"]["heads"]["video"].get("activation", "gelu")).to(device).eval()
    head.matmul = matmul
    return vid_vae, aud_codec, adapt_v, adapt_a, core, head, tstep_dim


def latents_to_tokens_video(z_v: torch.Tensor, t_p: int, p: int) -> torch.Tensor:
    return ops.tube_patch_video(z_v, t=t_p, h=p, w=p)


def latents_to_tokens_audio(z_a: torch.Tensor, l_chunk: int, s_chunk: int) -> torch.Tensor:
    return Fn.audio_tokens(z_a, l_chunk, s_chunk)


def tokens_to_latents_audio(tokens: torch.Tensor, Ca: int, l_chunk: int, Fa: int, stride: int) -> torch.Tensor:
    return Fn.audio_untokens(tokens, Ca, l_chunk, Fa, stride)



class FifoQueue:
    """The state of one open FIFO queue (``DenoiseEngine.fifo_open``): the device cursors ``r`` (ramp iteration) and ``m`` (steady
    iteration), the uploaded tables (``ramp``: [n - 1, B*S] each; ``steady`` and the selected ``slot`` tables: [B, S] each; two, or
    three with t_last), the prompt canvas ``canvas_p`` and the prompt-latent buffer ``prompt``, the latent buffers ``z`` / ``other``,
    the clip canvas ``clip``, and what the launches take by value: ``seed``, ``s0``, ``n`` (= c0), ``n_slots``, ``hop``."""


class _CapturedPair:

    def __init__(self, engine: "DenoiseEngine", graph: "torch.cuda.CUDAGraph"):
        self.engine, self.graph, self.generation = engine, graph, engine._generation

    def replay(self) -> None:
        self.engine._sync_weights()
        if self.generation != self.engine._generation:
            raise L.AvdError(f"this captured graph is stale ({self.engine._stale_reason or 'the engine tables changed'} since "
                             "capture_pair()): replaying it would launch kernels that hold the old values; capture again")
        self.graph.replay()


class DenoiseEngine:

    SOLVERS = ("ddim", "dpmpp_2m")
    NOISE_KEYINGS = ("sample", "canvas")
    GUIDE_KEYINGS = ("sample", "canvas")

    def __init__(self, *, adapt_v: LinearAdapter, adapt_a: LinearAdapter, core: MMDiT, head: MultiModalNoiseHead,
                 tstep_dim: int, target: str, latent_shape: Tuple[int, ...], prompt_tokens: int, alpha_bar: torch.Tensor,
                 guidance: float, eta: float = 0.0, tube=(2, 4, 4), chunk=(4, 4), split_streams: Optional[bool] = None,
                 temb_mode: str = "concat", matmul: Optional[str] = None, attn: Optional[str] = None,
                 noise_seed: Optional[int] = None, sample_offset: int = 0, solver: str = "ddim", guidance_rescale=0.0,
                 guidance_interval=None, noise_keying: str = "sample", canvas_hop: Optional[int] = None, apg=None):
        if target not in ("video", "audio"):
            raise ValueError("target must be 'video' or 'audio'")
        if eta < 0:
            raise ValueError("eta must be >= 0")
        if solver not in self.SOLVERS:
            raise ValueError(f"solver must be one of {self.SOLVERS}, got {solver!r}")
        if solver == "dpmpp_2m" and eta > 0 and noise_seed is None:
            raise ValueError("solver 'dpmpp_2m' with eta > 0 (its SDE form) draws seeded noise only: pass noise_seed, or eta = 0 for the "
                             "deterministic (ODE) solver")
        self.solver = solver
        self.guidance_interval = su.check_guidance_interval(guidance_interval)
        self._last_cond_only = False
        if temb_mode not in ("concat", "add"):
            raise ValueError("temb_mode must be 'concat' (sampler, sample_clip.py:59-70) or 'add' (trainer, trainer.py:45-49)")
        self.temb_mode = temb_mode
        self.target = target
        self.core, self.head = core, head
        self.adapt_t = adapt_v if target == "video" else adapt_a
        self.adapt_p = adapt_a if target == "video" else adapt_v
        self.d = core.cfg.d_model
        self.tdim = self.d if temb_mode == "add" else int(tstep_dim)
        self.tube, self.chunk = tuple(tube), tuple(chunk)
        self.eta = float(eta)
        self.device = next(core.final_norm.parameters()).device
        if not self.device.type == "cuda":
            raise L.AvdError("DenoiseEngine needs its modules on a ROCm device (no CPU fallback)")
        self.latent_shape = tuple(int(s) for s in latent_shape)
        B = self.latent_shape[0]
        self._g_vals, self._g_per_sample = Fn.cfg_values(guidance, B, "guidance"), not _scalar_like(guidance)
        self._phi_vals = Fn.cfg_values(guidance_rescale, B, "guidance_rescale", 0.0, 1.0)
        self.guidance = float(self._g_vals[0])
        self._cfg_g = self._cfg_phi = self._cfg_stats = None
        self._ctl: Optional[L.CfgControl] = None
        self._cfg_sig = None
        self._apg_vals = self._check_apg(Fn.apg_from_dict(apg), self._phi_vals)
        self._apg: Optional[L.ApgControl] = None
        self._apg_stats: Optional[torch.Tensor] = None
        self.apg_momentum: Optional[torch.Tensor] = None
        self._apg_sig = None
        self.noise_seed, self.sample_offset = noise_seed, int(sample_offset)
        self._key = None if noise_seed is None else Fn.noise_key(noise_seed, sample_offset)
        if self._key is None and sample_offset != 0:
            raise ValueError("sample_offset keys the seeded noise: it needs noise_seed")
        if noise_keying not in self.NOISE_KEYINGS:
            raise ValueError(f"noise_keying must be one of {self.NOISE_KEYINGS}, got {noise_keying!r}")
        self.noise_keying, self.canvas_hop = noise_keying, None
        if noise_keying == "canvas":
            if self._key is None:
                raise ValueError("noise_keying='canvas' keys the seeded noise stream by canvas position: it needs noise_seed")
            if canvas_hop is None:
                raise ValueError("noise_keying='canvas' needs canvas_hop: the latent positions from one window of the batch to the next")
            self.canvas_hop = Fn.check_canvas_keying(self.latent_shape, canvas_hop, self.sample_offset)
        elif canvas_hop is not None:
            raise ValueError("canvas_hop belongs to noise_keying='canvas'")
        elif self._key is not None and sample_offset + B > 2 ** 32:
            raise ValueError(f"sample_offset {sample_offset} + batch {B} exceeds the stream's 2**32 sample indices")
        e = L.EmbedDesc()
        e.B, e.d, e.tdim = B, self.d, self.tdim
        if target == "video":
            _, Cc, T, H, W = self.latent_shape
            t, h, w = self.tube
            assert T % t == 0 and H % h == 0 and W % w == 0, "tube sizes must divide latent dims"
            e.target_kind, e.target_first = 0, 1
            e.C, e.T, e.H, e.W = Cc, T, H, W
            e.p0, e.p1, e.p2 = t, h, w
            e.Nt = (T // t) * (H // h) * (W // w)
        else:
            _, Ca, Fa = self.latent_shape
            ln, st = self.chunk
            e.target_kind, e.target_first = 1, 0
            e.C, e.T, e.H, e.W = Ca, Fa, 1, 1
            e.p0, e.p1, e.p2 = ln, st, 1
            e.Nt = (Fa - ln) // st + 1
        e.Np = int(prompt_tokens)
        self._freqs = Fn.temb_freqs(self.tdim, 10000, self.device) if self.tdim >= 2 else None
        e.temb_freqs = L.ptr(self._freqs)
        e.temb_add = 1 if temb_mode == "add" else 0
        w_out = self.adapt_t.proj.weight.shape[0]
        if w_out != (self.d if temb_mode == "add" else self.d - self.tdim):
            raise ValueError(f"adapter width {w_out} does not match temb_mode='{temb_mode}' (d={self.d}, tdim={self.tdim})")
        self.embed = e
        self.N = e.Nt + e.Np
        self.alpha_bar = alpha_bar.to(self.device, torch.float32).contiguous()

        self.matmul = core.matmul if matmul is None else matmul
        self.attn = core.attn if attn is None else attn
        if split_streams is None:
            split_streams = self.matmul == "f16x2" and B * self.N >= 6144
        self._split_streams = bool(split_streams)
        self._generation = 0
        self._stale_reason = ""
        self.workspace: Optional[torch.Tensor] = None
        self.Xp: Optional[torch.Tensor] = None
        self._prompt_latent: Optional[torch.Tensor] = None
        self.x0_hist: Optional[torch.Tensor] = None
        if solver == "dpmpp_2m":
            self.x0_hist = torch.zeros(self.latent_shape, device=self.device, dtype=torch.float32)
            self._no_hist = torch.full((B,), -1, dtype=torch.long, device=self.device)
        self._hist_other: Optional[torch.Tensor] = None
        self._known: Optional[torch.Tensor] = None
        self._mask: Optional[torch.Tensor] = None
        self._guide: Optional[L.LatentGuide] = None
        self._guide_sig = None
        self._guide_hop: Optional[int] = None
        self._cons_hop: Optional[int] = None
        self._cons_w: Optional[torch.Tensor] = None
        self._bind_weights()
        self._apply_cfg()
        self._apply_apg()

    def _weights_key(self):
        mods = (self.core, self.head, self.adapt_t, self.adapt_p)
        return tuple((p.data_ptr(), p._version) for m in mods for p in m.parameters())

    def _bind_weights(self) -> None:
        core, head = self.core, self.head
        prev = core.matmul, core.attn
        core.matmul, core.attn = self.matmul, self.attn
        try:
            self._core_tab, self._keep_core = core.weight_table()
        finally:
            core.matmul, core.attn = prev
        hb = hn = None
        if self.matmul == "f16x2":
            fn_ = core.final_norm
            bias = getattr(fn_, "bias", None)
            g = fn_.weight if bias is not None else fn_.scale
            bd = Fn.weight_bounds([g] + ([bias] if bias is not None else []))
            gmax = bd[0][0] * core.cfg.d_model ** 0.5
            hb = gmax + (bd[1][0] if bias is not None else 0.0)
            hn = gmax + (bd[1][1] if bias is not None else 0.0)
        self._head_tab, self._keep_head = head.weight_table(self.target, matmul=self.matmul, in_bound=hb, in_norm=hn)
        self._aw = L.dev_f32(self.adapt_t.proj.weight.detach(), "adapter weight")
        self._ab = L.dev_f32(self.adapt_t.proj.bias.detach(), "adapter bias")
        if self._aw.device != self.device:
            raise L.AvdError("engine modules moved to another device after the engine was built")
        s = L.StepDesc()
        s.embed = self.embed
        s.core = C.pointer(self._core_tab)
        s.head = C.pointer(self._head_tab)
        s.adapt_w, s.adapt_b = self._aw.data_ptr(), self._ab.data_ptr()
        s.alpha_bar, s.T_train = self.alpha_bar.data_ptr(), self.alpha_bar.numel()
        s.guidance, s.eta = self.guidance, self.eta
        s.split_streams = 1 if self._split_streams else 0
        self.desc = s
        need = L.lib().avd_step_workspace_bytes(C.byref(s))
        if need < 0:
            raise ValueError(L.lib().avd_last_error().decode())
        if self.workspace is None or self.workspace.numel() < need:
            self.workspace = torch.empty(need, dtype=torch.uint8, device=self.device)
        self._ptrs = self._table_ptrs()
        self._scalars = self._table_scalars()
        self._wkey = self._weights_key()

    def _table_ptrs(self):
        return tuple(t.data_ptr() for t in self._keep_core[1]) + tuple(t.data_ptr() for t in self._keep_head[1]) + \
            (self._aw.data_ptr(), self._ab.data_ptr(), self.workspace.data_ptr(), self.alpha_bar.data_ptr())

    def _table_scalars(self):
        cw, hw = self._core_tab, self._head_tab
        blocks = self._keep_core[0]
        out = [cw.d, cw.n_layers, cw.n_heads, cw.mlp_hidden, cw.norm_eps, cw.norm_kind, cw.split_terms, cw.attn_mode,
               hw.d_in, hw.hidden, hw.d_out, hw.n_shared, hw.ln_eps, hw.act, hw.split_terms, self.guidance, self.eta]
        if cw.split_terms == 3:
            for i in range(cw.n_layers):
                out += list(blocks[i].f16x2_scale)
        if hw.split_terms == 3 and hw.f16x2_scale:
            out += [hw.f16x2_scale[i] for i in range(2 * (hw.n_shared + 2))]
        return tuple(float(v) for v in out)

    def _sync_weights(self) -> None:
        if self._weights_key() == self._wkey:
            return
        old, old_sc = self._ptrs, self._scalars
        self._bind_weights()
        if self._ptrs != old:
            self._generation += 1
            self._stale_reason = "a parameter or the workspace was re-allocated"
        elif self._scalars != old_sc:
            self._generation += 1
            self._stale_reason = ("an in-place parameter update changed a scale that a captured HIP graph holds by value (f16x2 image "
                                  "scales follow max|w| and the norm gains)")
        if self._prompt_latent is not None:
            self.set_prompt(self._prompt_latent)

    def set_prompt(self, prompt_latent: torch.Tensor) -> torch.Tensor:
        z = L.dev_f32(prompt_latent, "prompt latent")
        self._prompt_latent = z
        B = self.embed.B
        if z.shape[0] != B:
            raise ValueError("prompt batch size must match the engine's")
        tok = self._prompt_tokens(z)
        if tok.shape[1] != self.embed.Np:
            raise ValueError(f"prompt yields {tok.shape[1]} tokens, engine was built for {self.embed.Np}")
        d = self.d
        Xp = self.Xp
        if Xp is None or tuple(Xp.shape) != (B, tok.shape[1], d) or Xp.device != self.device:
            Xp = torch.empty(B, tok.shape[1], d, device=self.device, dtype=torch.float32)
            self._generation += 1
            self._stale_reason = "the prompt rows were (re-)allocated by set_prompt()"
        self._prompt_rows(tok, Xp)
        self.Xp = Xp
        return Xp

    def _prompt_tokens(self, z: torch.Tensor) -> torch.Tensor:
        return latents_to_tokens_audio(z, *self.chunk) if self.target == "video" else ops.tube_patch_video(z, *self.tube)

    def _prompt_rows(self, tok: torch.Tensor, Xp: torch.Tensor, temb: bool = True) -> None:
        B, d, td = self.embed.B, self.d, self.tdim
        w, b = self.adapt_p.proj.weight.detach(), self.adapt_p.proj.bias.detach()
        t0 = su.timestep_embedding(torch.zeros(B, dtype=torch.long, device=self.device), td) if td and temb else None
        if self.temb_mode == "add":
            res = t0[:, None, :].expand(B, tok.shape[1], d).contiguous()
            L.check(L.lib().avd_gemm_bias_act_f32(tok.data_ptr(), tok.shape[2], L.dev_f32(w).data_ptr(), L.dev_f32(b).data_ptr(),
                                                  res.data_ptr(), d, Xp.data_ptr(), d, B * tok.shape[1], d, tok.shape[2],
                                                  L.ACT_NONE, L.stream_ptr(self.device)))
        else:
            L.check(L.lib().avd_gemm_bias_act_f32(tok.data_ptr(), tok.shape[2], L.dev_f32(w).data_ptr(), L.dev_f32(b).data_ptr(),
                                                  None, 0, Xp.data_ptr(), d, B * tok.shape[1], d - td, tok.shape[2],
                                                  L.ACT_NONE, L.stream_ptr(self.device)))
            if t0 is not None:
                Xp[..., d - td:] = t0[:, None, :]

    def set_known(self, known: torch.Tensor, mask: Optional[torch.Tensor] = None, *, guide_seed: int = 0, keying: str = "sample",
                  hop: Optional[int] = None, sample_offset: Optional[int] = None) -> None:
        if keying not in self.GUIDE_KEYINGS:
            raise ValueError(f"keying must be one of {self.GUIDE_KEYINGS}, got {keying!r}")
        offset = self.sample_offset if sample_offset is None else sample_offset
        Fn.noise_key(guide_seed, offset)
        if keying == "canvas":
            if hop is None:
                raise ValueError("keying='canvas' needs hop: the latent positions from one window of the batch to the next")
            hop = Fn.check_canvas_keying(self.latent_shape, hop, offset)
            if self.canvas_hop is not None and hop != self.canvas_hop:
                raise ValueError(f"a canvas-keyed guide needs hop == canvas_hop (the engine's noise is keyed for windows {self.canvas_hop} "
                                 f"positions apart), got hop {hop}")
            if self._cons_hop is not None and hop != self._cons_hop:
                raise ValueError(f"a canvas-keyed guide needs hop == the window consensus hop {self._cons_hop}, got hop {hop}")
            if self.eta > 0 and self.canvas_hop is None:
                raise ValueError("a canvas-keyed guide at eta > 0 needs the step's noise keyed by canvas position as well: build the "
                                 "engine with noise_keying='canvas', canvas_hop=hop (per-sample step noise is refused)")
        elif hop is not None:
            raise ValueError("hop belongs to keying='canvas'")
        elif offset + self.latent_shape[0] > 2 ** 32:
            raise ValueError(f"sample_offset {offset} + batch {self.latent_shape[0]} exceeds the stream's 2**32 sample indices")
        known = L.dev_f32(known, "known")
        if tuple(known.shape) != self.latent_shape:
            raise ValueError(f"known latent shape {tuple(known.shape)} != engine shape {self.latent_shape}")
        m = None
        if mask is not None:
            m = torch.as_tensor(mask).to(self.device, torch.float32)
            shape = self.latent_shape[1:] if m.dim() < len(self.latent_shape) else self.latent_shape
            try:
                m = m.expand(shape)
            except RuntimeError:
                raise ValueError(f"mask shape {tuple(m.shape)} does not broadcast to {self.latent_shape[1:]} or "
                                 f"{self.latent_shape}") from None
            if not bool(((m >= 0) & (m <= 1)).all()):
                raise ValueError("mask values must lie in [0, 1]")
        if self._known is None:
            self._known = torch.empty(self.latent_shape, device=self.device, dtype=torch.float32)
        self._known.copy_(known)
        if m is not None:
            if self._mask is None or tuple(self._mask.shape) != tuple(m.shape):
                self._mask = torch.empty(tuple(m.shape), device=self.device, dtype=torch.float32)
            self._mask.copy_(m)
        self._guide = Fn.latent_guide_desc(self._known, self._mask if m is not None else None, guide_seed, offset)
        self._guide_hop = hop
        self._touch_guide()

    def clear_known(self) -> None:
        self._guide = None
        self._touch_guide()

    def _touch_guide(self) -> None:
        g = self._guide
        sig = None if g is None else (g.known, g.mask, g.mask_batch_stride, g.key.seed, g.key.sample_offset, self._guide_hop)
        if sig != self._guide_sig:
            self._generation += 1
            self._stale_reason = "the latent guide's buffers, mask presence, seed, sample offset, keying or hop changed (set_known / " \
                                 "clear_known)"
        self._guide_sig = sig

    def set_cfg(self, guidance=None, rescale=None) -> None:
        B = self.embed.B
# ... 595 lines not shown
```

Before: 121.6 steps/s.

## Compose head input projection with first shared linear; fuse final norm into head image

The head's input projection and its first shared linear layer are algebraically merged into one precomposed weight and bias (W1·W0, W1·b0+b1). This removes one GEMM per head forward, and that merge is on by default through AVD_HEAD_COMPOSE. A second option lets the core's final RMSNorm write the bf16x3 split image straight into the head workspace, skipping a separate split pass. That option is gated by AVD_HEAD_FUSE, which defaults to off. Composing the weights changes rounding slightly and adds a cached composed weight image.

Result: no change. 122.6 steps/s (median of 6 runs) (+0.8%).

```diff
diff --git a/include/avdiff_hip.h b/include/avdiff_hip.h
--- a/include/avdiff_hip.h
+++ b/include/avdiff_hip.h
@@ -29,9 +29,16 @@
 int         avd_device_arch(char* buf, int buflen);
 int         avd_tune_set(const char* key, int64_t value);
 int         avd_cfg_dedup_set(int on);
+int         avd_head_fuse_set(int on);
 
 int avd_rmsnorm_f32(const float* x, const float* scale, float* y, int64_t rows, int d, float eps,
                     avd_stream_t stream);
+int avd_rmsnorm_image_f32(const float* x, const float* scale, void* out, int64_t rows, int d, float eps,
+                          avd_stream_t stream);
+
+int avd_linear_compose_f32(const float* W1 , const float* b1 , const float* W0 ,
+                           const float* b0 , float* W , float* b , int n, int h, int k,
+                           avd_stream_t stream);
 
 int avd_gemm_bias_act_f32(const float* A, int64_t lda, const float* W, const float* bias,
                           const float* residual, int64_t ldr, float* C, int64_t ldc,
diff --git a/multimodal_diffusion_amd/_lib.py b/multimodal_diffusion_amd/_lib.py
--- a/multimodal_diffusion_amd/_lib.py
+++ b/multimodal_diffusion_amd/_lib.py
@@ -113,6 +113,9 @@
     "avd_gemm_rmsfold_f32": (_I, [_P, _P, _P, _P, _P, _L, _I, _I, _I, _P, _I, _F, _P, _P]),
     "avd_tune_set": (_I, [C.c_char_p, _L]),
     "avd_cfg_dedup_set": (_I, [_I]),
+    "avd_head_fuse_set": (_I, [_I]),
+    "avd_rmsnorm_image_f32": (_I, [_P, _P, _P, _L, _I, _F, _P]),
+    "avd_linear_compose_f32": (_I, [_P, _P, _P, _P, _P, _P, _I, _I, _I, _P]),
     "avd_attn_fwd_f32": (_I, [_P, _P, _I, _I, _I, _I, _F, _I, _P, _P]),
     "avd_layernorm_act_f32": (_I, [_P, _P, _P, _P, _L, _I, _F, _I, _P]),
     "avd_timestep_embedding_f32": (_I, [_P, _P, _P, _I, _I, _F, _P]),
diff --git a/multimodal_diffusion_amd/csrc/avd_common.h b/multimodal_diffusion_amd/csrc/avd_common.h
--- a/multimodal_diffusion_amd/csrc/avd_common.h
+++ b/multimodal_diffusion_amd/csrc/avd_common.h
@@ -242,6 +242,7 @@
                 hipStream_t st);
 int layernorm_act_f32(const float* x, const float* gamma, const float* beta, float* y, int64_t rows, int d, float eps,
                       int act, hipStream_t st);
+int rmsnorm_image_f32(const float* x, RowMap xm, const float* scale, void* out, int64_t rows, int d, float eps, hipStream_t st);
 int weight_bounds_f32(const float* x, int64_t rows, int d, float* out2, hipStream_t st);
 
 int64_t split3_bytes(int64_t rows, int K);
diff --git a/multimodal_diffusion_amd/csrc/composite.hip b/multimodal_diffusion_amd/csrc/composite.hip
--- a/multimodal_diffusion_amd/csrc/composite.hip
+++ b/multimodal_diffusion_amd/csrc/composite.hip
@@ -180,6 +180,12 @@
     return true;
 }();
 
+static int g_head_fuse = 0;
+[[maybe_unused]] static const bool g_head_fuse_env_applied = [] {
+    if (const char* e = getenv("AVD_HEAD_FUSE")) g_head_fuse = atoll(e) != 0;
+    return true;
+}();
+
 static int64_t core_split_wide_bytes(const avd_core_weights* w, int B, int N) {
     const int64_t qkv3 = qkv3_bytes(B, N, w->n_heads), fc1 = split3_bytes((int64_t)B * N, w->mlp_hidden);
     return qkv3 > fc1 ? qkv3 : fc1;
@@ -234,10 +240,18 @@
            !g_mlp_fused && gemm_bf16x3_resmap_supported(terms) && core_use_split(w, (int64_t)B2 * N) && core_use_split_fold(w);
 }
 
+static bool core_head_image_ok(const avd_core_weights* w, int B, int N, int out_row0, int n_out_rows) {
+    const int terms = w->split_terms;
+    return (terms == 0 || terms == 6 || terms == 9) && core_use_split(w, (int64_t)B * N) && core_use_split_fold(w) && g_core_trim &&
+           out_row0 == 0 && n_out_rows < N && w->attn_mode == 0 && gemm_bf16x3_resmap_supported(terms);
+}
+
 static int core_forward(const avd_core_weights* w, const float* x, float* y, int B, int N, int out_row0,
                         int n_out_rows, const unsigned char* kpm, void* ws, int64_t ws_bytes, hipStream_t st,
-                        const float* ss_first = nullptr, const RowSegs* segs = nullptr) {
+                        const float* ss_first = nullptr, const RowSegs* segs = nullptr, void* head_img = nullptr) {
     if (int rc = check_core(w)) return rc;
+    AVD_REQUIRE(!head_img || (!kpm && core_head_image_ok(w, B, N, out_row0, n_out_rows)), AVD_EUNSUPPORTED,
+                "core: the head image output needs the folded split path with the trimmed last block");
     AVD_REQUIRE(x && y && B > 0 && N > 0, AVD_EINVAL, "core: bad input");
     AVD_REQUIRE(out_row0 >= 0 && n_out_rows > 0 && out_row0 + n_out_rows <= N, AVD_EINVAL, "core: bad output row window");
     const int64_t M = (int64_t)B * N;
@@ -309,6 +323,7 @@
                             if (int rc = gemm_bf16x3(wide3, b.fc2_weight3, b.fc2_bias, yc, yc, nullptr, Mc, d, hid, AVD_ACT_NONE, terms, st)) return rc;
                         }
                     }
+                    if (head_img) return rmsnorm_image_f32(yc, rd, w->final_norm_scale, head_img, Mc, d, w->norm_eps, st);
                     return rmsnorm_f32(yc, rd, w->final_norm_scale, y, null_from ? rd : RowMap{d, nq, (int64_t)N * d}, Mc, d, w->norm_eps, st);
                 }
                 if (int rc = in_proj(b)) return rc;
@@ -435,10 +450,13 @@
     return core_norm(w, y, w->final_norm_scale, w->final_norm_bias, y, M, st);
 }
 
+static bool head_composed(const avd_head_weights* w) {
+    return w->n_shared >= 1 && w->shared_lin_weight && !w->shared_lin_weight[0];
+}
 static bool head_split_capable(const avd_head_weights* w, int64_t rows) {
     if (w->split_terms == 0) return false;
     if (!w->input_proj_weight3 || !w->out_proj_weight3 || (w->n_shared > 0 && !w->shared_lin_weight3)) return false;
-    for (int j = 0; j < w->n_shared; ++j)
+    for (int j = head_composed(w) ? 1 : 0; j < w->n_shared; ++j)
         if (!w->shared_lin_weight3[j]) return false;
     if (w->split_terms == 3 && !w->f16x2_scale) return false;
     return gemm_bf16x3_supported(rows, w->hidden, w->d_in) && gemm_bf16x3_supported(rows, w->hidden, w->hidden) &&
@@ -448,6 +466,11 @@
 static bool head_use_split(const avd_head_weights* w, int64_t rows) {
     return (t_step_head_rows > rows ? t_step_head_rows : rows) >= split_min_rows() && head_split_capable(w, rows);
 }
+
+static bool head_takes_image(const avd_head_weights* w, int64_t rows) {
+    return (w->split_terms == 6 || w->split_terms == 9) && head_use_split(w, rows);
+}
+static void* head_input_image(void* head_ws) { return head_ws; }
 
 static int64_t head_ws_bytes(const avd_head_weights* w, int64_t rows) {
     const int64_t fp32_path = 2 * align_up(rows * w->hidden * 4);
@@ -458,7 +481,7 @@
 }
 
 static int head_forward(const avd_head_weights* w, const float* h, RowMap hm, int64_t rows, float* out, void* ws,
-                        int64_t ws_bytes, hipStream_t st) {
+                        int64_t ws_bytes, hipStream_t st, const void* in_img = nullptr) {
     AVD_REQUIRE(w && h && out, AVD_EINVAL, "head: null pointer");
     AVD_REQUIRE(w->d_in > 0 && w->hidden > 0 && w->d_out > 0 && w->n_shared >= 0, AVD_EINVAL, "head: bad dims");
     AVD_REQUIRE(w->input_proj_weight && w->out_proj_weight, AVD_EINVAL, "head: null weights");
@@ -467,6 +490,17 @@
     AVD_REQUIRE(w->split_terms == 0 || w->split_terms == 6 || w->split_terms == 9 || w->split_terms == 1 || w->split_terms == 3, AVD_EINVAL,
                 "head: split_terms must be 0 (fp32), 6, 9, 1 or 3, got %d", w->split_terms);
     AVD_REQUIRE(ws && ws_bytes >= head_ws_bytes(w, rows), AVD_EWORKSPACE, "head: workspace too small");
+    const bool composed = head_composed(w);
+    for (int j = 1; j < w->n_shared; ++j)
+        AVD_REQUIRE(w->shared_lin_weight[j], AVD_EINVAL, "head: shared_lin_weight[%d] is NULL (only block 0 may be composed away)", j);
+    if (composed) {
+        AVD_REQUIRE(!w->shared_lin_bias[0] && (w->split_terms == 0 || !w->shared_lin_weight3 || !w->shared_lin_weight3[0]), AVD_EINVAL,
+                    "head: a composed block 0 has neither weight, bias nor weight image (half-NULL entry)");
+        AVD_REQUIRE(w->split_terms == 0 || w->split_terms == 6 || w->split_terms == 9, AVD_EUNSUPPORTED,
+                    "head: a composed table takes split_terms 0, 6 or 9 (got %d: the f16x2 scales and the one-plane mode are defined on "
+                    "the uncomposed chain)", w->split_terms);
+    }
+    AVD_REQUIRE(!in_img || (in_img == ws && head_takes_image(w, rows)), AVD_EINVAL, "head: input image without the split path to read it");
     Carver cv{static_cast<char*>(ws), 0, ws_bytes};
     const RowMap rh{w->hidden, 0, 0}, ro{w->d_out, 0, 0};
     if (head_use_split(w, rows)) {
@@ -482,12 +516,20 @@
         void* imgA = cv.take((split3_bytes(rows, wide) + 3) / 4);
         void* imgB = cv.take((split3_bytes(rows, wide) + 3) / 4);
         float* t2 = cv.take(rows * w->hidden);
-        if (int rc = split3_rows_f32(h, hm, imgA, rows, w->d_in, st, asc(0))) return rc;
-        if (int rc = gemm_bf16x3(imgA, w->input_proj_weight3, w->input_proj_bias, nullptr, nullptr, imgB, rows, w->hidden, w->d_in, AVD_ACT_NONE,
-                                 terms, st, h2 ? asc(0) * wsc(0) : 1.f, h2 ? asc(1) : 1.f)) return rc;
+        if (!in_img)
+            if (int rc = split3_rows_f32(h, hm, imgA, rows, w->d_in, st, asc(0))) return rc;
         void* cur = imgB;
         void* nxt = imgA;
-        for (int j = 0; j < n; ++j) {
+        if (composed) {
+            if (int rc = gemm_bf16x3(imgA, w->input_proj_weight3, w->input_proj_bias, nullptr, t2, nullptr, rows, w->hidden, w->d_in, AVD_ACT_NONE,
+                                     terms, st, 1.f, 1.f)) return rc;
+            if (int rc = layernorm_act_split3_f32(t2, w->shared_ln_weight[0], w->shared_ln_bias[0], imgB, rows, w->hidden, w->ln_eps, w->act, st,
+                                                  0.f)) return rc;
+        } else {
+            if (int rc = gemm_bf16x3(imgA, w->input_proj_weight3, w->input_proj_bias, nullptr, nullptr, imgB, rows, w->hidden, w->d_in, AVD_ACT_NONE,
+                                     terms, st, h2 ? asc(0) * wsc(0) : 1.f, h2 ? asc(1) : 1.f)) return rc;
+        }
+        for (int j = composed ? 1 : 0; j < n; ++j) {
             if (int rc = gemm_bf16x3(cur, w->shared_lin_weight3[j], w->shared_lin_bias[j], nullptr, t2, nullptr, rows, w->hidden, w->hidden,
                                      AVD_ACT_NONE, terms, st, h2 ? asc(1 + j) * wsc(1 + j) : 1.f, 1.f)) return rc;
             if (int rc = layernorm_act_split3_f32(t2, w->shared_ln_weight[j], w->shared_ln_bias[j], nxt, rows, w->hidden, w->ln_eps, w->act, st,
@@ -499,8 +541,13 @@
     }
     float* t1 = cv.take(rows * w->hidden);
     float* t2 = cv.take(rows * w->hidden);
-    if (int rc = gemm_f32(h, hm, w->input_proj_weight, w->input_proj_bias, nullptr, rh, t1, rh, rows, w->hidden, w->d_in, AVD_ACT_NONE, st)) return rc;
-    for (int j = 0; j < w->n_shared; ++j) {
+    if (composed) {
+        if (int rc = gemm_f32(h, hm, w->input_proj_weight, w->input_proj_bias, nullptr, rh, t2, rh, rows, w->hidden, w->d_in, AVD_ACT_NONE, st)) return rc;
+        if (int rc = layernorm_act_f32(t2, w->shared_ln_weight[0], w->shared_ln_bias[0], t1, rows, w->hidden, w->ln_eps, w->act, st)) return rc;
+    } else {
+        if (int rc = gemm_f32(h, hm, w->input_proj_weight, w->input_proj_bias, nullptr, rh, t1, rh, rows, w->hidden, w->d_in, AVD_ACT_NONE, st)) return rc;
+    }
+    for (int j = composed ? 1 : 0; j < w->n_shared; ++j) {
         if (int rc = gemm_f32(t1, rh, w->shared_lin_weight[j], w->shared_lin_bias[j], nullptr, rh, t2, rh, rows, w->hidden, w->hidden, AVD_ACT_NONE, st)) return rc;
         if (int rc = layernorm_act_f32(t2, w->shared_ln_weight[j], w->shared_ln_bias[j], t1, rows, w->hidden, w->ln_eps, w->act, st)) return rc;
     }
@@ -727,6 +774,12 @@
     return prev;
 }
 
+extern "C" int avd_head_fuse_set(int on) {
+    const int prev = g_head_fuse;
+    g_head_fuse = on != 0;
+    return prev;
+}
+
 extern "C" int avd_device_arch(char* buf, int buflen) {
     AVD_REQUIRE(buf && buflen > 0, AVD_EINVAL, "device_arch: bad buffer");
     hipDeviceProp_t prop;
@@ -790,6 +843,12 @@
     return p.total;
 }
 
+static bool step_head_image_ok(const avd_step_desc* s, int Bc, int N, int row0, int64_t head_rows) {
+    const avd_embed_desc& e = s->embed;
+    return g_head_fuse && s->head && s->core && s->head->d_in == s->core->d && head_rows == (int64_t)Bc * e.Nt &&
+           core_head_image_ok(s->core, Bc, N, row0, e.Nt) && head_takes_image(s->head, head_rows);
+}
+
 static int denoise_step(const avd_step_desc* s, const avd_noise_key* key, const float* z, const float* Xp, const int64_t* t_now,
                         const int64_t* t_prev, const float* noise, float* z_out, void* workspace, int64_t workspace_bytes,
                         avd_stream_t stream, const int64_t* t_last = nullptr, float* x0_hist = nullptr,
@@ -807,12 +866,14 @@
     if (int rc = embed_cfg_pair(&e, z, s->adapt_w, s->adapt_b, t_now, Xp, tok, X2, st, ssx, false, dedup ? &seg : nullptr, slots)) return rc;
     const int row0 = e.target_first ? 0 : e.Np;
     const RowMap hm{e.d, e.Nt, (int64_t)p.N * e.d};
+    void* himg = !s->split_streams && step_head_image_ok(s, 2 * e.B, p.N, row0, p.rows) ? head_input_image(head_ws) : nullptr;
     if (dedup) {
-        if (int rc = core_forward(s->core, X2, X2, 2 * e.B, p.N, 0, e.Nt, nullptr, core_ws, p.core, st, nullptr, &seg)) return rc;
-        if (int rc = head_forward(s->head, X2, RowMap{e.d, 0, 0}, p.rows, eps2, head_ws, p.head, st)) return rc;
+        if (int rc = core_forward(s->core, X2, X2, 2 * e.B, p.N, 0, e.Nt, nullptr, core_ws, p.core, st, nullptr, &seg, himg)) return rc;
+        if (int rc = head_forward(s->head, X2, RowMap{e.d, 0, 0}, p.rows, eps2, head_ws, p.head, st, himg)) return rc;
     } else if (!s->split_streams) {
-        if (int rc = core_forward(s->core, X2, X2, 2 * e.B, p.N, row0, e.Nt, nullptr, core_ws, p.core, st, have_ss ? ssx : nullptr)) return rc;
-        if (int rc = head_forward(s->head, X2 + (int64_t)row0 * e.d, hm, p.rows, eps2, head_ws, p.head, st)) return rc;
+        if (int rc = core_forward(s->core, X2, X2, 2 * e.B, p.N, row0, e.Nt, nullptr, core_ws, p.core, st, have_ss ? ssx : nullptr, nullptr,
+                                  himg)) return rc;
+        if (int rc = head_forward(s->head, X2 + (int64_t)row0 * e.d, hm, p.rows, eps2, head_ws, p.head, st, himg)) return rc;
     } else {
         AuxState ax;
         if (int rc = ensure_aux(st, ax)) return rc;
@@ -859,8 +920,10 @@
     if (int rc = embed_cfg_pair(&e, z, s->adapt_w, s->adapt_b, t_now, Xp, tok, X1, st, ssx, true)) return rc;
     const int row0 = e.target_first ? 0 : e.Np;
     const RowMap hm{e.d, e.Nt, (int64_t)p.N * e.d};
-    if (int rc = core_forward(s->core, X1, X1, e.B, p.N, row0, e.Nt, nullptr, core_ws, p.core / 2, st, have_ss ? ssx : nullptr)) return rc;
-    if (int rc = head_forward(s->head, X1 + (int64_t)row0 * e.d, hm, p.rows / 2, eps1, head_ws, p.head / 2, st)) return rc;
+    void* himg = step_head_image_ok(s, e.B, p.N, row0, p.rows / 2) ? head_input_image(head_ws) : nullptr;
+    if (int rc = core_forward(s->core, X1, X1, e.B, p.N, row0, e.Nt, nullptr, core_ws, p.core / 2, st, have_ss ? ssx : nullptr, nullptr,
+                              himg)) return rc;
+    if (int rc = head_forward(s->head, X1 + (int64_t)row0 * e.d, hm, p.rows / 2, eps1, head_ws, p.head / 2, st, himg)) return rc;
     if (e.target_kind == 0)
         return eps_unpatch_ddim_f32(eps1, z, t_now, t_prev, s->alpha_bar, s->T_train, s->eta, noise, z_out, e.B, e.C, e.T, e.H, e.W, e.p0,
                                     e.p1, e.p2, st, key, t_last, x0_hist, guide, canvas_hop, guide_hop);
diff --git a/multimodal_diffusion_amd/csrc/rowops.hip b/multimodal_diffusion_amd/csrc/rowops.hip
--- a/multimodal_diffusion_amd/csrc/rowops.hip
+++ b/multimodal_diffusion_amd/csrc/rowops.hip
@@ -88,6 +88,57 @@
                 o[e] = t;
             }
             *reinterpret_cast<f32x4*>(yr + c) = o;
+        }
+    }
+}
+
+template <int NV>
+__global__ __launch_bounds__(256) void rmsnorm_image_kernel(const float* __restrict__ x, RowMap xm, const float* __restrict__ scale,
+                                                            unsigned char* __restrict__ out, int64_t rows, int64_t rows_pad, int d,
+                                                            float eps, float sqrt_d) {
+    const int lane = threadIdx.x & 63;
+    const int64_t row = (int64_t)blockIdx.x * 4 + (threadIdx.x >> 6);
+    if (row >= rows_pad) return;
+    const bool live = row < rows;
+    f32x4 v[NV];
+    float ss = 0.f;
+    if (live) {
+        const float* xr = x + xm.off(row);
+#pragma unroll
+        for (int i = 0; i < NV; ++i) {
+            const int c = (lane + 64 * i) * 4;
+            if (c < d) {
+                v[i] = *reinterpret_cast<const f32x4*>(xr + c);
+                ss += v[i][0] * v[i][0] + v[i][1] * v[i][1] + v[i][2] * v[i][2] + v[i][3] * v[i][3];
+            }
+        }
+    }
+    ss = wave_sum(ss);
+    const float den = sqrtf(ss) / sqrt_d + eps;
+    f32x4 o[NV];
+#pragma unroll
+    for (int i = 0; i < NV; ++i) {
+        const int c = (lane + 64 * i) * 4;
+        o[i] = f32x4{0.f, 0.f, 0.f, 0.f};
+        if (live && c < d) {
+            const f32x4 s = *reinterpret_cast<const f32x4*>(scale + c);
+            o[i] = f32x4{s[0] * v[i][0] / den, s[1] * v[i][1] / den, s[2] * v[i][2] / den, s[3] * v[i][3] / den};
+        }
+    }
+    const bool odd = lane & 1;
+#pragma unroll
+    for (int q = 0; q < (NV + 1) / 2; ++q) {
+        const int ie = 2 * q, io = 2 * q + 1 < NV ? 2 * q + 1 : 2 * q;
+        const f32x4 give = odd ? o[ie] : o[io];
+        f32x4 got;
+#pragma unroll
+        for (int e = 0; e < 4; ++e) got[e] = __shfl_xor(give[e], 1, 64);
+        if (odd && io == ie) continue;
+        const f32x4 lo = odd ? got : o[ie], hi = odd ? o[io] : got;
+        const int c = ((lane & ~1) + 64 * (odd ? io : ie)) * 4;
+        if (c < d) {
+            const float w8[8] = {lo[0], lo[1], lo[2], lo[3], hi[0], hi[1], hi[2], hi[3]};
+            store_split8(out, row, c, d, w8);
         }
     }
 }
@@ -194,6 +245,69 @@
     return AVD_OK;
 }
 
+int rmsnorm_image_f32(const float* x, RowMap xm, const float* scale, void* out, int64_t rows, int d, float eps, hipStream_t st) {
+    AVD_REQUIRE(x && scale && out, AVD_EINVAL, "rmsnorm_image: null pointer");
+    AVD_REQUIRE(rows > 0 && d > 0 && d % 16 == 0 && d <= 256 * ROW_MAXV, AVD_EUNSUPPORTED,
+                "rmsnorm_image: d=%d must be a multiple of 16, <= %d", d, 256 * ROW_MAXV);
+    AVD_REQUIRE(xm.ld % 4 == 0 && xm.stride % 4 == 0 && aligned16(x) && aligned16(out) && aligned16(scale), AVD_EUNSUPPORTED,
+                "rmsnorm_image: rows must be 16-byte aligned");
+    const int64_t rows_pad = (rows + 255) / 256 * 256;
+    AVD_REQUIRE(rows_pad / 4 < (1ll << 31), AVD_EUNSUPPORTED, "rmsnorm_image: grid too large");
+    const int tag = prof_tag_id("rmsnorm_image_kernel<%d>", nv_for(d));
+    ProfScope prof(tag, 10.0 * (double)rows * d, st);
+    const unsigned grid = (unsigned)(rows_pad / 4);
+    const float isd = (float)sqrt((double)d);
+    unsigned char* o = static_cast<unsigned char*>(out);
+    switch (nv_for(d)) {
+#define AVD_CASE(NV) case NV: hipLaunchKernelGGL(rmsnorm_image_kernel<NV>, dim3(grid), dim3(256), 0, st, x, xm, scale, o, rows, rows_pad, d, eps, isd); break;
+        AVD_CASE(1) AVD_CASE(2) AVD_CASE(3) AVD_CASE(4) AVD_CASE(5) AVD_CASE(6) AVD_CASE(7) AVD_CASE(8)
+#undef AVD_CASE
+    }
+    AVD_CHECK_LAUNCH("rmsnorm_image");
+    return AVD_OK;
+}
+
+__global__ __launch_bounds__(256) void linear_compose_kernel(const float* __restrict__ W1, const float* __restrict__ b1,
+                                                             const float* __restrict__ W0, const float* __restrict__ b0,
+                                                             float* __restrict__ W, float* __restrict__ b, int n, int h, int k) {
+    const int64_t idx = (int64_t)blockIdx.x * 256 + threadIdx.x;
+    if (idx >= (int64_t)n * (k + 1)) return;
+    const int i = (int)(idx / (k + 1)), c = (int)(idx % (k + 1));
+    const float* w1 = W1 + (int64_t)i * h;
+    double acc = 0.0;
+    if (c < k) {
+        for (int j = 0; j < h; ++j) acc += (double)w1[j] * (double)W0[(int64_t)j * k + c];
+        W[(int64_t)i * k + c] = (float)acc;
+    } else {
+        if (b0)
+            for (int j = 0; j < h; ++j) acc += (double)w1[j] * (double)b0[j];
+        if (b1) acc += (double)b1[i];
+        b[i] = (float)acc;
+    }
+}
+
+static bool ranges_overlap(const float* a, int64_t na, const float* b, int64_t nb) { return a && b && a < b + nb && b < a + na; }
+
+int linear_compose_f32(const float* W1, const float* b1, const float* W0, const float* b0, float* W, float* b, int n, int h, int k,
+                       hipStream_t st) {
+    AVD_REQUIRE(W1 && W0 && W && b, AVD_EINVAL, "linear_compose: null pointer");
+    AVD_REQUIRE(n > 0 && h > 0 && k > 0, AVD_EINVAL, "linear_compose: bad dims (n=%d h=%d k=%d)", n, h, k);
+    const int64_t nw1 = (int64_t)n * h, nw0 = (int64_t)h * k, nw = (int64_t)n * k;
+    const float* ins[4] = {W1, b1, W0, b0};
+    const int64_t in_n[4] = {nw1, n, nw0, h};
+    for (int i = 0; i < 4; ++i)
+        AVD_REQUIRE(!ranges_overlap(W, nw, ins[i], in_n[i]) && !ranges_overlap(b, n, ins[i], in_n[i]), AVD_EINVAL,
+                    "linear_compose: the outputs must not alias an input");
+    AVD_REQUIRE(!ranges_overlap(W, nw, b, n), AVD_EINVAL, "linear_compose: W and b must not overlap");
+    const int64_t total = (int64_t)n * (k + 1);
+    AVD_REQUIRE((total + 255) / 256 < (1ll << 31), AVD_EUNSUPPORTED, "linear_compose: grid too large");
+    static const int tag = prof_tag_id("linear_compose_kernel");
+    ProfScope prof(tag, 4.0 * (double)(nw1 + nw0 + nw), st);
+    hipLaunchKernelGGL(linear_compose_kernel, dim3((unsigned)((total + 255) / 256)), dim3(256), 0, st, W1, b1, W0, b0, W, b, n, h, k);
+    AVD_CHECK_LAUNCH("linear_compose");
+    return AVD_OK;
+}
+
 }
 
 extern "C" int avd_rmsnorm_f32(const float* x, const float* scale, float* y, int64_t rows, int d, float eps,
@@ -210,3 +324,13 @@
                                      int d, float eps, int act, avd_stream_t stream) {
     return avd::layernorm_act_f32(x, gamma, beta, y, rows, d, eps, act, static_cast<hipStream_t>(stream));
 }
+
+extern "C" int avd_linear_compose_f32(const float* W1, const float* b1, const float* W0, const float* b0, float* W, float* b, int n,
+                                      int h, int k, avd_stream_t stream) {
+    return avd::linear_compose_f32(W1, b1, W0, b0, W, b, n, h, k, static_cast<hipStream_t>(stream));
+}
+
+extern "C" int avd_rmsnorm_image_f32(const float* x, const float* scale, void* out, int64_t rows, int d, float eps,
+                                     avd_stream_t stream) {
+    return avd::rmsnorm_image_f32(x, avd::RowMap{d, 0, 0}, scale, out, rows, d, eps, static_cast<hipStream_t>(stream));
+}
diff --git a/multimodal_diffusion_amd/functional.py b/multimodal_diffusion_amd/functional.py
--- a/multimodal_diffusion_amd/functional.py
+++ b/multimodal_diffusion_amd/functional.py
@@ -3,7 +3,7 @@
 import ctypes as C
 import math
 import numbers
-from typing import Optional
+from typing import Optional, Tuple
 
 import torch
 
@@ -748,6 +748,38 @@
     return out
 
 
+def rmsnorm_image(x: Tensor, scale: Tensor, eps: float = 1e-6) -> Tensor:
+    x = L.dev_f32(x, "x")
+    scale = L.dev_f32(scale, "scale")
+    d = x.shape[-1]
+    rows = x.numel() // d
+    nbytes = L.lib().avd_split3_bytes(rows, d)
+    if nbytes < 0:
+        raise L.AvdError(f"rmsnorm_image: d={d} must be a multiple of 16")
+    out = torch.empty(nbytes, dtype=torch.uint8, device=x.device)
+    L.check(L.lib().avd_rmsnorm_image_f32(x.data_ptr(), scale.data_ptr(), out.data_ptr(), rows, d, eps, _st(x)))
+    return out
+
+
+def linear_compose(w1: Tensor, b1: Optional[Tensor], w0: Tensor, b0: Optional[Tensor],
+                   out: Optional[Tuple[Tensor, Tensor]] = None) -> Tuple[Tensor, Tensor]:
+    w1, w0 = L.dev_f32(w1, "w1"), L.dev_f32(w0, "w0")
+    b1 = None if b1 is None else L.dev_f32(b1, "b1")
+    b0 = None if b0 is None else L.dev_f32(b0, "b0")
+    n, h = w1.shape
+    if w0.shape[0] != h:
+        raise ValueError(f"linear_compose: w1 {tuple(w1.shape)} does not chain with w0 {tuple(w0.shape)}")
+    k = w0.shape[1]
+    if out is not None and tuple(out[0].shape) == (n, k) and tuple(out[1].shape) == (n,) and out[0].device == w1.device:
+        w, b = out
+    else:
+        w = torch.empty(n, k, dtype=torch.float32, device=w1.device)
+        b = torch.empty(n, dtype=torch.float32, device=w1.device)
+    L.check(L.lib().avd_linear_compose_f32(w1.data_ptr(), L.ptr(b1), w0.data_ptr(), L.ptr(b0), w.data_ptr(), b.data_ptr(), n, h, k,
+                                           _st(w1)))
+    return w, b
+
+
 def rmsnorm_split3(x: Tensor, scale: Tensor, eps: float = 1e-6) -> Tensor:
     x = L.dev_f32(x, "x")
     scale = L.dev_f32(scale, "scale")
diff --git a/multimodal_diffusion_amd/noise_heads.py b/multimodal_diffusion_amd/noise_heads.py
--- a/multimodal_diffusion_amd/noise_heads.py
+++ b/multimodal_diffusion_amd/noise_heads.py
@@ -1,6 +1,7 @@
 from __future__ import annotations
 
 import ctypes as C
+import os
 from typing import Dict, List, Optional, Union
 
 import torch
@@ -36,6 +37,8 @@
 
 
 class MultiModalNoiseHead(nn.Module):
+    compose_input: bool = os.environ.get("AVD_HEAD_COMPOSE", "1").strip() not in ("0", "")
+
     def __init__(self, input_dims: Dict[str, int], output_dims: Dict[str, int], hidden_dim: int = 512,
                  num_shared_layers: int = 2, num_modality_specific_layers: int = 1, dropout: float = 0.1,
                  activation: str = "gelu", share_parameters: bool = False):
@@ -109,13 +112,30 @@
             self._images[f"{m}.f16x2"] = hit
         return hit[1]
 
-    def weight_table(self, m: str, matmul: Optional[str] = None, in_bound: Optional[float] = None, in_norm: Optional[float] = None):
+    def _composed(self, m: str, blk0: nn.Sequential):
+        from . import functional as Fn
+        ps = (blk0[0].weight, blk0[0].bias, self.input_proj[m].weight, self.input_proj[m].bias)
+        key = tuple((p.data_ptr(), p._version, tuple(p.shape)) for p in ps)
+        name = f"{m}.composed"
+        hit = self._images.get(name)
+        if hit is None or hit[0] != key:
+            old = hit[1] if hit is not None and hit[1][0].device == ps[0].device else None
+            hit = (key, Fn.linear_compose(*(p.detach() for p in ps), out=old))
+            self._images[name] = hit
+        return hit[1]
+
+    def weight_table(self, m: str, matmul: Optional[str] = None, in_bound: Optional[float] = None, in_norm: Optional[float] = None,
+                     compose: Optional[bool] = None):
         matmul = self.matmul if matmul is None else matmul
         if matmul not in L.MATMUL_TERMS:
             raise ValueError(f"matmul must be one of {sorted(L.MATMUL_TERMS)}, got {matmul!r}")
         blocks = self._trunk(m)
         n = len(blocks)
         keep = []
+        terms = L.MATMUL_TERMS[matmul]
+        shapes_ok = self.input_dims[m] % 16 == 0 and self.hidden_dim % 256 == 0 and self.output_dims[m] % 256 == 0
+        compose = self.compose_input if compose is None else bool(compose)
+        compose = compose and n >= 1 and not (terms in (1, 3) and shapes_ok)
 
         def dp(p):
             t = L.dev_f32(p.detach(), "head parameter")
@@ -124,16 +144,16 @@
 
         arrs = [(C.c_void_p * max(n, 1))() for _ in range(5)]
         for j, blk in enumerate(blocks):
-            arrs[0][j], arrs[1][j] = dp(blk[0].weight), dp(blk[0].bias)
+            if not (compose and j == 0):
+                arrs[0][j], arrs[1][j] = dp(blk[0].weight), dp(blk[0].bias)
             arrs[2][j], arrs[3][j] = dp(blk[1].weight), dp(blk[1].bias)
         eps = blocks[0][1].eps if n else 1e-5
+        w_in, b_in = self._composed(m, blocks[0]) if compose else (self.input_proj[m].weight, self.input_proj[m].bias)
         hw = L.HeadWeights(self.input_dims[m], self.hidden_dim, self.output_dims[m], n, eps, self._act,
-                           dp(self.input_proj[m].weight), dp(self.input_proj[m].bias),
+                           dp(w_in), dp(b_in),
                            C.cast(arrs[0], C.POINTER(C.c_void_p)), C.cast(arrs[1], C.POINTER(C.c_void_p)),
                            C.cast(arrs[2], C.POINTER(C.c_void_p)), C.cast(arrs[3], C.POINTER(C.c_void_p)),
                            dp(self.out_proj[m].weight), dp(self.out_proj[m].bias))
-        terms = L.MATMUL_TERMS[matmul]
-        shapes_ok = self.input_dims[m] % 16 == 0 and self.hidden_dim % 256 == 0 and self.output_dims[m] % 256 == 0
         if terms and shapes_ok:
             sc = None
             if matmul == "f16x2":
@@ -143,13 +163,25 @@
                 scales = (C.c_float * len(sc))(*sc)
                 arrs.append(scales)
                 hw.f16x2_scale = C.cast(scales, C.POINTER(C.c_float))
-            ws = [self.input_proj[m].weight] + [b[0].weight for b in blocks] + [self.out_proj[m].weight]
-            imgs = [self._image(f"{m}.{i}", w, sc[i] if sc else 0.0) for i, w in enumerate(ws)]
-            keep += imgs
+            if compose:
+                key = self._images[f"{m}.composed"][0]
+                hit = self._images.get(f"{m}.composed3")
+                if hit is None or hit[0] != key:
+                    from . import functional as Fn
+                    old = hit[1] if hit is not None and hit[1].device == w_in.device else None
+                    hit = (key, Fn.split3(w_in, out=old))
+                    self._images[f"{m}.composed3"] = hit
+                imgs = [hit[1], None] + [self._image(f"{m}.{1 + j}", blocks[j][0].weight, 0.0) for j in range(1, n)] + \
+                    [self._image(f"{m}.{n + 1}", self.out_proj[m].weight, 0.0)]
+            else:
+                ws = [self.input_proj[m].weight] + [b[0].weight for b in blocks] + [self.out_proj[m].weight]
+                imgs = [self._image(f"{m}.{i}", w, sc[i] if sc else 0.0) for i, w in enumerate(ws)]
+            keep += [i for i in imgs if i is not None]
             hw.split_terms = terms
             hw.input_proj_weight3 = imgs[0].data_ptr()
             for j in range(n):
-                arrs[4][j] = imgs[1 + j].data_ptr()
+                if imgs[1 + j] is not None:
+                    arrs[4][j] = imgs[1 + j].data_ptr()
             hw.shared_lin_weight3 = C.cast(arrs[4], C.POINTER(C.c_void_p))
             hw.out_proj_weight3 = imgs[-1].data_ptr()
         return hw, (arrs, keep)
diff --git a/multimodal_diffusion_amd/sampler.py b/multimodal_diffusion_amd/sampler.py
--- a/multimodal_diffusion_amd/sampler.py
+++ b/multimodal_diffusion_amd/sampler.py
@@ -108,7 +108,8 @@
                  guidance: float, eta: float = 0.0, tube=(2, 4, 4), chunk=(4, 4), split_streams: Optional[bool] = None,
                  temb_mode: str = "concat", matmul: Optional[str] = None, attn: Optional[str] = None,
                  noise_seed: Optional[int] = None, sample_offset: int = 0, solver: str = "ddim", guidance_rescale=0.0,
-                 guidance_interval=None, noise_keying: str = "sample", canvas_hop: Optional[int] = None, apg=None):
+                 guidance_interval=None, noise_keying: str = "sample", canvas_hop: Optional[int] = None, apg=None,
+                 head_compose: Optional[bool] = None):
         if target not in ("video", "audio"):
             raise ValueError("target must be 'video' or 'audio'")
         if eta < 0:
@@ -126,6 +127,7 @@
         self.temb_mode = temb_mode
         self.target = target
         self.core, self.head = core, head
+        self.head_compose = head_compose
         self.adapt_t = adapt_v if target == "video" else adapt_a
         self.adapt_p = adapt_a if target == "video" else adapt_v
         self.d = core.cfg.d_model
@@ -240,7 +242,7 @@
             gmax = bd[0][0] * core.cfg.d_model ** 0.5
             hb = gmax + (bd[1][0] if bias is not None else 0.0)
             hn = gmax + (bd[1][1] if bias is not None else 0.0)
-        self._head_tab, self._keep_head = head.weight_table(self.target, matmul=self.matmul, in_bound=hb, in_norm=hn)
+        self._head_tab, self._keep_head = head.weight_table(self.target, matmul=self.matmul, in_bound=hb, in_norm=hn, compose=self.head_compose)
         self._aw = L.dev_f32(self.adapt_t.proj.weight.detach(), "adapter weight")
         self._ab = L.dev_f32(self.adapt_t.proj.bias.detach(), "adapter bias")
         if self._aw.device != self.device:
```
